# microsoft/fadtk

Measured on AMD Instinct MI355X. Metric: FAD scores/sec + cov-GEMM TFLOP/s (% MFMA peak), N=100k D=512, higher is better.
Workload: dtype f16 in, f16 MFMA with f32 accumulate over <= 8192-row runs, f64 across runs (moments); split-f16 MFMA iterations (f32 accumulate) + exact int8-MFMA products (int32 accumulate) + f64 correction (Frechet)

## Files before the change

fadtk_amd/csrc/frechet.hip:

```cpp
#include "frechet_internal.h"
#include "ns_mean.h"
#include "ns_fast.h"
#include "ns_fast_big.h"
#include "ns_fast_res.h"

#include <algorithm>
#include <atomic>
#include <cmath>
#include <type_traits>

namespace fad {

Pool& thread_pool(int device) {
    static thread_local PerThreadDevice<Pool> set;
    return set.get(device);
}
Workspace* free_slot(int device) {
    Pool& p = thread_pool(device);
    for (Workspace& w : p.slot)
        if (!w.busy) { w.pool = &p; return &w; }
    return nullptr;
}

SongKnobs SongKnobs::from_env() {
    SongKnobs k;
    auto off = [](const char* name) { const char* e = getenv(name); return e && e[0] == '0'; };
    if (const char* e = getenv("FAD_SONG_BIG")) k.big_min = atol(e);
    if (const char* e = getenv("FAD_SONG_RES")) k.res = (e[0] == '0') ? 0 : (e[0] == '1' ? 1 : 2);
    if (const char* e = getenv("FAD_SONG_FAST")) k.fast = (e[0] == '0') ? 0 : (e[0] == '2' ? 2 : 1);
    if (const char* e = getenv("FAD_FAST_TRACE")) k.trace = e[0] == '1';
    k.scaled = !off("FAD_SONG_SCALED");
    if (const char* e = getenv("FAD_SONG_L0_SCALE")) { const double v = atof(e); if (v > 0.0) k.l0_scale = v; }
    return k;
}


struct MixedResult {
    int status;
    int iters, decided_at, nonfinite, too_few0, too_few1;
    double tr_scaled, c, tr1, tr2, mean_term, res, est;
    int prepared;
    int pad;
};

__global__ __launch_bounds__(256) void ns32_finish(const double* __restrict__ stats, int d, int nb,
                                                   const NsState* __restrict__ st, Ns32State* __restrict__ s32,
                                                   MixedResult* __restrict__ out, int max_low) {
    __shared__ double red[4];
    __shared__ double red3[12];
    const int tid = threadIdx.x;
    const bool live = s32->ok != 0;
    double mr = 0.0, mc = 0.0, corr = 0.0, r2 = 0.0, tr = 0.0;
    if (live) {
        const double* rowabs = stats;
        const double* colabs = stats + (int64_t)nb * d;
        const double* scal = stats + 2 * (int64_t)nb * d;
        for (int i = tid; i < d; i += 256) {
            double rs, cs;
            sum_partials(rowabs, colabs, nb, d, i, rs, cs);
            mr = fmax(mr, rs); mc = fmax(mc, cs);
        }
        for (int k = tid; k < nb * nb; k += 256) {
            const double* sc = scal + (int64_t)kStatScal * k;
            corr += sc[0]; r2 += sc[1]; tr += sc[2];
        }
    }
    const double zinf = block_max(mr, red), zone = block_max(mc, red);
    double v3[3] = {corr, r2, tr};
    block_sum_n<3>(v3, red3);
    corr = v3[0]; r2 = v3[1]; tr = v3[2];
    if (tid != 0) return;
    MixedResult o;
    o.status = 0; o.iters = s32->final_iter; o.decided_at = s32->decided_at; o.nonfinite = st->nonfinite;
    o.too_few0 = st->too_few[0]; o.too_few1 = st->too_few[1];
    o.c = st->c; o.tr1 = st->tr1; o.tr2 = st->tr2; o.mean_term = st->mean_term;
    o.tr_scaled = 0.0; o.res = 0.0; o.est = 0.0; o.prepared = 1; o.pad = 0;
    if (st->done || s32->failed) {
        o.status = 2;
    } else if (live) {
        const int f = s32->final_iter;
        const int fm = f < 16 ? f : 15;
        double res = s32->res[fm];
        if (s32->decided_at == f - 1) { const double rp = s32->res[f - 1 < 16 ? f - 1 : 15]; res = 0.75 * rp * rp + 0.25 * rp * rp * rp; if (res < 2e-6) res = 2e-6; }
        const double zn = sqrt(zinf * zone), rn = sqrt(r2);
        const double trs = tr + 0.5 * corr;
        const double est = zn * zn * zn * rn * rn / 8.0 + zn * res * rn / 2.0;
        const bool finite = (trs == trs) && !isinf(trs) && (est == est) && !isinf(est);
        o.tr_scaled = trs; o.res = res; o.est = est;
        o.status = (finite && est <= 1e-9 * fabs(trs)) ? 1 : 2;
        if (o.status == 2 && finite && !s32->strict && s32->decided_at == f - 1 && f + 1 < max_low) {
            o.status = 4;
            s32->done = 0; s32->finished = 0; s32->ok = 0; s32->skip_corr = 1; s32->upd_skip[0] = 0; s32->upd_skip[1] = 0;
            s32->strict = 1;
        }
    }
    *out = o;
}

constexpr int kMaxLow = 14;
constexpr int kMaxLowWide = 22;
constexpr double kWideL0Scale = 3.0, kWideL0Min = 9e-4;
static bool wide_enabled(Pool* p) {
    if (p && p->lp_wide < 0) { const char* e = getenv("FAD_FRECHET_WIDE"); p->lp_wide = (e && e[0] == '0') ? 0 : 1; }
    return !p || p->lp_wide != 0;
}
static int max_low_of(const Workspace& ws) { return (ws.job.fast && wide_enabled(ws.pool)) ? kMaxLowWide : kMaxLow; }

static double pred_threshold(Pool* p, int d) {
    if (p && p->pred_thr == 0.0) { const char* e = getenv("FAD_FRECHET_PRED_THR"); p->pred_thr = (e && atof(e) > 0.0) ? atof(e) : -1.0; }
    if (p && p->pred_thr > 0.0) return p->pred_thr;
    return 2.5e-3 * (double)d / 512.0;
}

struct MixedBufs {
    double* A; float *Y[2], *Z[2], *T;
    NsState* dstate; double* partials; double* tilestats; Ns32State* s32; MixedResult* hres;
    unsigned nb;
};
static MixedBufs mixed_bufs(Workspace& ws, int d) {
    const int64_t dd = (int64_t)d * d;
    MixedBufs m;
    m.A = static_cast<double*>(ws.mats.p);
    m.Y[0] = static_cast<float*>(ws.mats32.p); m.Y[1] = m.Y[0] + dd;
    m.Z[0] = m.Y[1] + dd; m.Z[1] = m.Y[1] + 2 * dd;
    m.T = m.Y[1] + 3 * dd;
    m.dstate = static_cast<NsState*>(ws.small.p);
    m.partials = reinterpret_cast<double*>(m.dstate + 1);
    m.tilestats = m.partials + ns_pstride(d);
    m.s32 = reinterpret_cast<Ns32State*>(m.tilestats + stat_doubles(d));
    m.hres = reinterpret_cast<MixedResult*>(static_cast<char*>(ws.pinned) + sizeof(NsState));
    m.nb = (unsigned)stat_blocks(d);
    return m;
}

static int mixed_enqueue(Workspace& ws, int upto) {
    const int d = ws.job.d;
    hipStream_t stream = ws.job.stream;
    MixedBufs m = mixed_bufs(ws, d);
    int rc;
    for (int& k = ws.job.k; k < upto; ++k) {
        const int cur = k & 1;
        Gemm32Args g;
        memset(&g, 0, sizeof(g));
        if (k == 0) {
            g.C[0] = m.Y[1]; g.C[1] = m.Z[1]; g.alpha[0] = 1.0f; g.ntypes = 1; g.A64 = m.A; g.st64 = m.dstate;
            g.skip = &m.s32->done;
            FAD_TRY(gemm_f32_first_launch(d, g, stream));
            continue;
        }
        g.A[0] = m.Z[cur]; g.B[0] = m.Y[cur]; g.C[0] = m.T; g.alpha[0] = -0.5f; g.beta_eye[0] = 1.5f; g.gamma[0] = 1.0f;
        g.partials[0] = m.partials; g.skip = &m.s32->done; g.ntypes = 1;
        const int nslots = gemm_f32_launch(d, g, stream);
        if (nslots < 0) return nslots;
        memset(&g, 0, sizeof(g));
        g.A[0] = m.Y[cur]; g.B[0] = m.T; g.C[0] = m.Y[cur ^ 1]; g.alpha[0] = 1.0f;
        g.A[1] = m.T; g.B[1] = m.Z[cur]; g.C[1] = m.Z[cur ^ 1]; g.alpha[1] = 1.0f;
        g.ntypes = 2;
        g.skip = &m.s32->upd_skip[k & 1];
        g.check = 1; g.k = k; g.max_low = kMaxLow; g.nslots = nslots; g.chk_partials = m.partials; g.st = m.s32; g.st64 = m.dstate;
        g.thr_pred = pred_threshold(ws.pool, d);
        rc = gemm_f32_launch(d, g, stream);
        if (rc < 0) return rc;
    }
    NsProductExt ext;
    memset(&ext, 0, sizeof(ext));
    ext.stats = m.tilestats; ext.st = m.dstate; ext.A64 = m.A; ext.Z32 = m.Z[0]; ext.Z32_alt = m.Z[1];
    FAD_TRY(gemm_f64_correction_launch(d, m.Y[0], m.Y[1], &m.s32->final_iter, &m.s32->skip_corr, ext, stream));
    hipLaunchKernelGGL(ns32_finish, dim3(1), dim3(256), 0, stream, m.tilestats, d, (int)m.nb, m.dstate, m.s32, m.hres, kMaxLow);
    FAD_HIP_TRY(hipGetLastError());
    if (!ws.done_ev) FAD_HIP_TRY(hipEventCreateWithFlags(&ws.done_ev, hipEventDisableTiming));
    FAD_HIP_TRY(hipEventRecord(ws.done_ev, stream));
    return FAD_OK;
}

static bool mixed_eligible(Workspace& ws, int d, int max_iter, double tol);
static bool fast_dim(int d) { return d == 256 || d == 384 || d == 512 || d == 768 || d == 1024; }
static bool fast_eligible(Workspace& ws, int d, int max_iter, double tol) {
    Pool* p = ws.pool;
    if (p && p->fast < 0) { const char* e = getenv("FAD_FRECHET_FAST"); p->fast = (e && e[0] == '0') ? 0 : 1; }
    return (!p || p->fast) && fast_dim(d) && mixed_eligible(ws, d, max_iter, tol);
}

struct FastBufs {
    nsf::MatHdr* hdr;
    uint4* digC[2];
    nsf::SplitMat P, Y[2], Z[2], T;
    uint4 *digY[2], *digYt[2];
    nsf::SplitMat Rv, Pv, Ev;
    int* host_words; double* host_vals; double* host_stats; double* host_vstats;
};
static size_t fast_bytes(int d) {
    const size_t dd = (size_t)d * d;
    return 256 + 2 * 6 * dd + 6 * 8 * dd + 4 * 6 * dd + 3 * 8 * dd + 256;
}
static size_t fast_pinned_bytes(int d) {
    const size_t nb = (size_t)d / 32;
    return sizeof(NsState) + sizeof(MixedResult) + 64 + nsf::kHostWords * sizeof(int) + nsf::kHostVals * sizeof(double) +
           (nsf::kTileStats + 2 + nsf::kVerStats) * nb * nb * sizeof(double) + 128;
}
static FastBufs fast_bufs(Workspace& ws, int d) {
    const size_t dd = (size_t)d * d;
    char* p = static_cast<char*>(ws.fast.p);
    FastBufs f;
    f.hdr = reinterpret_cast<nsf::MatHdr*>(p); p += 256;
    for (int i = 0; i < 2; ++i) { f.digC[i] = reinterpret_cast<uint4*>(p); p += 6 * dd; }
    nsf::SplitMat* mats[6] = {&f.P, &f.Y[0], &f.Y[1], &f.Z[0], &f.Z[1], &f.T};
    for (nsf::SplitMat* m : mats) {
        m->a = reinterpret_cast<uint4*>(p); p += 4 * dd;
        m->at = reinterpret_cast<uint4*>(p); p += 4 * dd;
    }
    for (int i = 0; i < 2; ++i) { f.digY[i] = reinterpret_cast<uint4*>(p); p += 6 * dd; f.digYt[i] = reinterpret_cast<uint4*>(p); p += 6 * dd; }
    nsf::SplitMat* vmats[3] = {&f.Rv, &f.Pv, &f.Ev};
    for (nsf::SplitMat* m : vmats) {
        m->a = reinterpret_cast<uint4*>(p); p += 4 * dd;
        m->at = reinterpret_cast<uint4*>(p); p += 4 * dd;
    }
    char* h = static_cast<char*>(ws.pinned);
    f.host_words = nullptr; f.host_vals = nullptr; f.host_stats = nullptr; f.host_vstats = nullptr;
    if (h && ws.pinned_cap >= fast_pinned_bytes(d)) {
        const size_t nb2 = ((size_t)d / 32) * ((size_t)d / 32);
        h += ((sizeof(NsState) + sizeof(MixedResult) + 63) / 64) * 64;
        f.host_vals = reinterpret_cast<double*>(h); h += nsf::kHostVals * sizeof(double);
        f.host_stats = reinterpret_cast<double*>(h); h += (nsf::kTileStats + 2) * nb2 * sizeof(double);
        f.host_vstats = reinterpret_cast<double*>(h); h += nsf::kVerStats * nb2 * sizeof(double);
        f.host_words = reinterpret_cast<int*>(h);
    }
    return f;
}

static int fast_prepare(Workspace& ws, int d, int ddof, const double* acc1, const double* acc2, const double* cov1, const double* cov2,
                        const double* mu1, const double* mu2, int mean_dtype, double* mus, double* covs, hipStream_t st,
                        const float* run1 = nullptr, const float* run2 = nullptr) {
    void* const before = ws.fast.p;
    FAD_TRY(ws.fast.reserve(fast_bytes(d)));
    FAD_TRY(ws.small.reserve(ns_small_bytes(d, 1)));
    FastBufs f = fast_bufs(ws, d);
    if (ws.fast.p != before) FAD_HIP_TRY(hipMemsetAsync(f.hdr, 0, 256, st));
    ws.job.gen = ++ws.fast_gen;
    if (ws.fast_gen > (1 << 30)) ws.fast_gen = 1;
    nsf::PrepArgs a;
    memset(&a, 0, sizeof(a));
    a.acc[0] = acc1; a.acc[1] = acc2; a.cov_in[0] = cov1; a.cov_in[1] = cov2; a.mu_in[0] = mu1; a.mu_in[1] = mu2;
    a.run[0] = run1; a.run[1] = run2;
    a.d = d; a.ddof = ddof; a.gen = ws.job.gen; a.mean_dtype = mean_dtype;
    a.mus = mus; a.covs = covs;
    a.dig[0] = f.digC[0]; a.dig[1] = f.digC[1];
    a.st = static_cast<NsState*>(ws.small.p);
    a.hdr[0] = f.hdr; a.hdr[1] = f.hdr + 1;
    hipLaunchKernelGGL(nsf::nsf_prepare, dim3((unsigned)((int64_t)d * d / 2048 + 1), 2), dim3(512), 0, st, a);
    FAD_HIP_TRY(hipGetLastError());
    return FAD_OK;
}

template <int NS> static void fast_launch_split(int mode, unsigned t, unsigned B, const nsf::SplitArgs& g, hipStream_t st) {
    if (mode == nsf::SP_FIRST) hipLaunchKernelGGL((nsf::nsf_split<NS, nsf::SP_FIRST>), dim3(t, t, B), dim3(512), 0, st, g);
    else if (mode == nsf::SP_T) hipLaunchKernelGGL((nsf::nsf_split<NS, nsf::SP_T>), dim3(t, t, B), dim3(512), 0, st, g);
    else if (mode == nsf::SP_V2) hipLaunchKernelGGL((nsf::nsf_split<NS, nsf::SP_V2>), dim3(t, t, 2 * B), dim3(512), 0, st, g);
    else if (mode == nsf::SP_V3) hipLaunchKernelGGL((nsf::nsf_split<NS, nsf::SP_V3>), dim3(t, t, B), dim3(512), 0, st, g);
    else hipLaunchKernelGGL((nsf::nsf_split<NS, nsf::SP_U>), dim3(t, t, 3 * B), dim3(512), 0, st, g);
}
static void fast_split(int d, int mode, const nsf::SplitArgs& g, hipStream_t st, unsigned B);
static void fast_verify_launch(int d, unsigned B, nsf::SplitArgs g, const nsf::SplitMat (&Y)[2], const nsf::SplitMat (&Z)[2], const nsf::SplitMat& Rv,
                               const nsf::SplitMat& Pv, const nsf::SplitMat& Ev, const Ns32State* s32, double* vstats, int* vwords, int64_t hstride,
                               hipStream_t st) {
    g.sel = &s32->final_iter; g.skip = &s32->skip_corr;
    g.Zf[0] = Z[0]; g.Zf[1] = Z[1]; g.Yf[0] = Y[0]; g.Yf[1] = Y[1];
    g.vstats = vstats; g.vwords = vwords; g.hstride = hstride;
    g.B[0] = Rv; g.C[0] = Pv; g.C[1] = Ev;
    fast_split(d, nsf::SP_V2, g, st, B);
    g.B[0] = Pv; g.A[1] = Ev; g.C[0] = nsf::SplitMat{nullptr, nullptr}; g.C[1] = nsf::SplitMat{nullptr, nullptr};
    fast_split(d, nsf::SP_V3, g, st, B);
}
static void fast_split(int d, int mode, const nsf::SplitArgs& g, hipStream_t st, unsigned B) {
    const unsigned t = (unsigned)(d / 32);
    switch (d) {
        case 128: fast_launch_split<1>(mode, t, B, g, st); break;
        case 256: fast_launch_split<2>(mode, t, B, g, st); break;
        case 384: fast_launch_split<3>(mode, t, B, g, st); break;
        case 512: fast_launch_split<4>(mode, t, B, g, st); break;
        case 768: fast_launch_split<6>(mode, t, B, g, st); break;
        default: fast_launch_split<8>(mode, t, B, g, st); break;
    }
}
template <int NJ> static void fast_big_attrs() {
    (void)hipFuncSetAttribute(reinterpret_cast<const void*>(&nsf::nsf_big<nsf::SP_T, NJ>), hipFuncAttributeMaxDynamicSharedMemorySize, (int)nsf::kBigLds);
    (void)hipFuncSetAttribute(reinterpret_cast<const void*>(&nsf::nsf_big<nsf::SP_U, NJ>), hipFuncAttributeMaxDynamicSharedMemorySize, (int)nsf::kBigLds);
    (void)hipFuncSetAttribute(reinterpret_cast<const void*>(&nsf::nsf_big<nsf::SP_FIRST, NJ>), hipFuncAttributeMaxDynamicSharedMemorySize, (int)nsf::kBigLds);
}
template <int NJ> static void fast_big_launch(int d, int mode, const nsf::SplitArgs& g, hipStream_t st, unsigned B) {
    const int tt = nsf::big_tiles(d, NJ);
    const unsigned one = (unsigned)nsf::big_grid((int)B, tt), two = (unsigned)nsf::big_grid((int)B, 2 * tt);
    if (mode == nsf::SP_FIRST) hipLaunchKernelGGL((nsf::nsf_big<nsf::SP_FIRST, NJ>), dim3(one), dim3(256), nsf::kBigLds, st, g);
    else if (mode == nsf::SP_T) hipLaunchKernelGGL((nsf::nsf_big<nsf::SP_T, NJ>), dim3(one), dim3(256), nsf::kBigLds, st, g);
    else hipLaunchKernelGGL((nsf::nsf_big<nsf::SP_U, NJ>), dim3(two + B), dim3(256), nsf::kBigLds, st, g);
}
static int fast_big_t_slots(int d, unsigned B) { return nsf::big_tiles(d, nsf::big_nj(d, 1, (int)B)); }
static int fast_split_big(int d, int mode, nsf::SplitArgs g, hipStream_t st, unsigned B, int device) {
    static std::atomic<unsigned> ready{0};
    if (device >= 0 && device < 32 && !(ready.load(std::memory_order_acquire) & (1u << device))) {
        fast_big_attrs<1>(); fast_big_attrs<2>();
        FAD_HIP_TRY(hipGetLastError());
        ready.fetch_or(1u << device, std::memory_order_release);
    }
    g.nprob = (int)B;
    if (nsf::big_nj(d, mode == nsf::SP_U ? 2 : 1, (int)B) == 1) fast_big_launch<1>(d, mode, g, st, B);
    else fast_big_launch<2>(d, mode, g, st, B);
    return FAD_OK;
}
static int fast_i8_big(int d, int mode, const nsf::I8Args& g, hipStream_t st, unsigned B, int device) {
    static std::atomic<unsigned> ready{0};
    if (device >= 0 && device < 32 && !(ready.load(std::memory_order_acquire) & (1u << device))) {
        FAD_HIP_TRY(hipFuncSetAttribute(reinterpret_cast<const void*>(&nsf::nsf_i8_big<nsf::I8_A>), hipFuncAttributeMaxDynamicSharedMemorySize, (int)nsf::kI8BigLds));
        FAD_HIP_TRY(hipFuncSetAttribute(reinterpret_cast<const void*>(&nsf::nsf_i8_big<nsf::I8_G>), hipFuncAttributeMaxDynamicSharedMemorySize, (int)nsf::kI8BigLds));
        FAD_HIP_TRY(hipFuncSetAttribute(reinterpret_cast<const void*>(&nsf::nsf_i8_big<nsf::I8_G, true>), hipFuncAttributeMaxDynamicSharedMemorySize, (int)nsf::kI8BigLds));
        ready.fetch_or(1u << device, std::memory_order_release);
    }
    const unsigned grid = (unsigned)nsf::big_grid((int)B, (d / 128) * (d / 64));
    if (mode == nsf::I8_A) hipLaunchKernelGGL((nsf::nsf_i8_big<nsf::I8_A>), dim3(grid), dim3(512), nsf::kI8BigLds, st, g, (int)B);
    else if (g.Rv.a) hipLaunchKernelGGL((nsf::nsf_i8_big<nsf::I8_G, true>), dim3(grid), dim3(512), nsf::kI8BigLds, st, g, (int)B);
    else hipLaunchKernelGGL((nsf::nsf_i8_big<nsf::I8_G>), dim3(grid), dim3(512), nsf::kI8BigLds, st, g, (int)B);
    return FAD_OK;
}
template <int NS8> static void fast_launch_i8(int mode, unsigned t, unsigned B, const nsf::I8Args& g, hipStream_t st) {
    if (mode == nsf::I8_A) hipLaunchKernelGGL((nsf::nsf_i8<NS8, nsf::I8_A>), dim3(t, t, B), dim3(512), 0, st, g);
    else hipLaunchKernelGGL((nsf::nsf_i8<NS8, nsf::I8_G>), dim3(t, t, B), dim3(512), 0, st, g);
}
static void fast_i8(int d, int mode, const nsf::I8Args& g, hipStream_t st, unsigned B = 1) {
    const unsigned t = (unsigned)(d / 32);
    switch (d) {
        case 128: case 256: fast_launch_i8<1>(mode, t, B, g, st); break;
        case 384: case 512: fast_launch_i8<2>(mode, t, B, g, st); break;
        case 768: fast_launch_i8<3>(mode, t, B, g, st); break;
        default: fast_launch_i8<4>(mode, t, B, g, st); break;
    }
}

static nsf::SplitArgs fast_split_args(Workspace& ws, const MixedBufs& m, const FastBufs& f, int d) {
    nsf::SplitArgs g;
    memset(&g, 0, sizeof(g));
    g.d = d; g.gen = ws.job.gen; g.hA = f.hdr; g.hB = f.hdr + 1; g.st = m.dstate; g.s32 = m.s32;
    if (wide_enabled(ws.pool)) { g.scaled = 1; g.lp_wide = 1; g.l0_scale = kWideL0Scale; g.l0_min = kWideL0Min; }
    return g;
}
static int fast_verify_enqueue(Workspace& ws) {
    const int d = ws.job.d;
    MixedBufs m = mixed_bufs(ws, d);
    FastBufs f = fast_bufs(ws, d);
    f.host_words[13] = 0;
    fast_verify_launch(d, 1, fast_split_args(ws, m, f, d), f.Y, f.Z, f.Rv, f.Pv, f.Ev, m.s32, f.host_vstats, f.host_words, 0, ws.job.stream);
    FAD_HIP_TRY(hipGetLastError());
    FAD_HIP_TRY(hipEventRecord(ws.done_ev, ws.job.stream));
    return FAD_OK;
}
static int fast_enqueue(Workspace& ws, int upto) {
    const int d = ws.job.d;
    hipStream_t stream = ws.job.stream;
    MixedBufs m = mixed_bufs(ws, d);
    FastBufs f = fast_bufs(ws, d);
    if (!f.host_words) return set_error(FAD_ERR_ALLOC, "pinned result area of the fast Frechet chain is missing");
    const int nslots = (d / 32) * (d / 32);
    const int max_low = max_low_of(ws);
    for (int& k = ws.job.k; k < upto; ++k) {
        nsf::SplitArgs g = fast_split_args(ws, m, f, d);
        if (k == 0) {
            nsf::I8Args a;
            memset(&a, 0, sizeof(a));
            a.Adig = f.digC[0]; a.Bdig = f.digC[1]; a.d = d; a.gen = ws.job.gen; a.hA = f.hdr; a.hB = f.hdr + 1; a.stats = m.tilestats;
            a.A64 = m.A; a.P = f.P; a.st = m.dstate;
            fast_i8(d, nsf::I8_A, a, stream);
            g.A[0] = f.P; g.B[0] = f.P; g.C[0] = f.Y[1]; g.C[1] = f.Z[1]; g.Cdig[0] = f.digY[1]; g.Cdig_t[0] = f.digYt[1];
            g.A64 = m.A; g.statsA = m.tilestats;
            fast_split(d, nsf::SP_FIRST, g, stream, 1);
            continue;
        }
        const int cur = k & 1;
        g.A[0] = f.Z[cur]; g.B[0] = f.Y[cur]; g.C[0] = f.T; g.alpha = -0.5f; g.beta_eye = 1.5f; g.gamma = 1.0f;
        g.partials = m.partials; g.skip = &m.s32->done; g.k = k;
        fast_split(d, nsf::SP_T, g, stream, 1);
        g = fast_split_args(ws, m, f, d);
        g.A[0] = f.Y[cur]; g.B[0] = f.T; g.C[0] = f.Y[cur ^ 1];
        g.A[1] = f.T; g.B[1] = f.Z[cur]; g.C[1] = f.Z[cur ^ 1];
        g.Cdig[0] = f.digY[cur ^ 1]; g.Cdig_t[0] = f.digYt[cur ^ 1];
        g.skip = &m.s32->upd_skip[k & 1];
        g.k = k; g.max_low = max_low; g.nslots = nslots; g.chk_partials = m.partials;
        g.thr_pred = pred_threshold(ws.pool, d);
        fast_split(d, nsf::SP_U, g, stream, 1);
    }
    nsf::I8Args a;
    memset(&a, 0, sizeof(a));
    a.Adig = f.digY[0]; a.Bdig = f.digYt[0]; a.Adig_alt = f.digY[1]; a.Bdig_alt = f.digYt[1]; a.sel = &m.s32->final_iter;
    a.d = d; a.gen = ws.job.gen; a.hA = f.hdr; a.hB = f.hdr + 1; a.skip = &m.s32->skip_corr; a.stats = f.host_stats; a.st = m.dstate; a.A64in = m.A;
    a.Y[0] = f.Y[0]; a.Y[1] = f.Y[1]; a.Z[0] = f.Z[0]; a.Z[1] = f.Z[1];
    a.s32 = m.s32; a.host_words = f.host_words; a.host_vals = f.host_vals;
    const bool wide = wide_enabled(ws.pool);
    if (wide) { a.Rv = f.Rv; a.scaled = 1; }
    f.host_words[12] = 0;
    f.host_words[13] = 0;
    fast_i8(d, nsf::I8_G, a, stream);
    FAD_HIP_TRY(hipGetLastError());
    if (!ws.done_ev) FAD_HIP_TRY(hipEventCreateWithFlags(&ws.done_ev, hipEventDisableTiming));
    if (wide && ws.pool && ws.pool->lp_verify) return fast_verify_enqueue(ws);
    FAD_HIP_TRY(hipEventRecord(ws.done_ev, stream));
    return FAD_OK;
}

static void fast_decide_one(const int* hw, const double* hv, const double* hsx, int nb, MixedResult* out, const double* hvx = nullptr,
                            int gen = 0, int max_low = kMaxLow) {
    MixedResult o;
    memset(&o, 0, sizeof(o));
    const bool bad = hw[0] != 0;
    o.status = 0; o.iters = hw[7]; o.decided_at = hw[8]; o.nonfinite = hw[2]; o.too_few0 = hw[3]; o.too_few1 = hw[4];
    o.c = hv[0]; o.tr1 = hv[1]; o.tr2 = hv[2]; o.mean_term = hv[3];
    o.prepared = 0;
    const bool ok = hw[5] != 0, failed = hw[6] != 0, strict = hw[9] != 0;
    if (bad || hw[1] || failed) {
        o.status = 2;
    } else if (ok && !hw[11]) {
        double corr = 0.0, r2 = 0.0, tr = 0.0, zinf = 0.0, zone = 0.0;
        for (int t = 0; t < nb * nb; ++t) { corr += hsx[nsf::kTileStats * t]; r2 += hsx[nsf::kTileStats * t + 1]; tr += hsx[nsf::kTileStats * t + 2]; }
        const double* zmax = hsx + (size_t)nsf::kTileStats * nb * nb;
        for (int x = 0; x < nb; ++x) {
            double rs = 0.0, cs = 0.0;
            for (int y = 0; y < nb; ++y) { rs += zmax[2 * (y * nb + x)]; cs += zmax[2 * (x * nb + y) + 1]; }
            if (rs > zinf) zinf = rs;
            if (cs > zone) zone = cs;
        }
        const int fi = hw[7];
        double res = hv[4 + ns32_slot(fi)];
        if (hw[8] == fi - 1) { const double rp = hv[4 + ns32_slot(fi - 1)]; res = 0.75 * rp * rp + 0.25 * rp * rp * rp; if (res < 2e-6) res = 2e-6; }
        const double zn = std::sqrt(zinf * zone), rn = std::sqrt(r2);
        double trs = tr + 0.5 * corr;
        double est = zn * zn * zn * rn * rn / 8.0 + zn * res * rn / 2.0;
        bool finite = std::isfinite(trs) && std::isfinite(est);
        double fad = o.mean_term + o.tr1 + o.tr2 - 2.0 * std::sqrt(o.c) * trs;
        bool accept = finite && (est <= 1e-9 * std::fabs(trs) || 2.0 * std::sqrt(o.c) * est <= 1e-5 * std::fabs(fad));
        const bool scaled = hvx && hw[14] != 0;
        const bool predicted = hw[8] == fi - 1 && fi >= 1;
        const double r_pred = predicted ? hv[4 + ns32_slot(fi - 1)] : 0.0;
        const bool can_go_on = predicted && !strict && fi + 1 < max_low && (!scaled || r_pred > 0.1);
        bool need_verify = false;
        if (!accept && finite && hvx && !can_go_on) {
            if (hw[13] == gen) {
                const double inv = 1.0 / ((double)nsf::kVerScale * (double)nsf::kVerScale);
                double qp = 0.0, ep = 0.0, pp = 0.0, ee = 0.0;
                for (int t = 0; t < nb * nb; ++t) { qp += hvx[nsf::kVerStats * t]; ep += hvx[nsf::kVerStats * t + 1]; pp += hvx[nsf::kVerStats * t + 2]; ee += hvx[nsf::kVerStats * t + 3]; }
                qp *= inv; ep *= inv; pp *= inv; ee *= inv;
                const double trs_v = trs + 0.5 * ep;
                const double est_v = 4.0 * std::fabs(qp) / 8.0 + ee * std::sqrt(pp);
                const double fad_v = o.mean_term + o.tr1 + o.tr2 - 2.0 * std::sqrt(o.c) * trs_v;
                const bool fin_v = std::isfinite(trs_v) && std::isfinite(est_v);
                if (fin_v && (est_v <= 1e-9 * std::fabs(trs_v) || 2.0 * std::sqrt(o.c) * est_v <= 4e-6 * std::fabs(fad_v))) {
                    accept = true; trs = trs_v; est = est_v; fad = fad_v; o.pad = 1;
                }
            } else {
                need_verify = true;
            }
        }
        o.tr_scaled = trs; o.res = res; o.est = est;
        o.status = accept ? 1 : 2;
        if (!accept && finite && can_go_on) o.status = 4;
        else if (!accept && need_verify) o.status = 5;
    }
    *out = o;
}

static int fast_decide(Workspace& ws) {
    const int d = ws.job.d, nb = d / 32;
    MixedBufs m = mixed_bufs(ws, d);
    FastBufs f = fast_bufs(ws, d);
    if (f.host_words[12] != ws.job.gen) return set_error(FAD_ERR_HIP, "the correction kernel of the fast Frechet chain left no result");
    const bool wide = wide_enabled(ws.pool);
    fast_decide_one(f.host_words, f.host_vals, f.host_stats, nb, m.hres, wide ? f.host_vstats : nullptr, ws.job.gen, max_low_of(ws));
    if (m.hres->status == 4) {
        hipLaunchKernelGGL(nsf::nsf_rearm, dim3(1), dim3(64), 0, ws.job.stream, m.s32);
        FAD_HIP_TRY(hipGetLastError());
    }
    return FAD_OK;
}

bool fast_song_dim(int d) { return d == 128 || d == 256 || d == 384 || d == 512 || d == 768 || d == 1024; }

struct SongBlock {
    size_t hdr, st, s32, partials, stats, A64, P, Y[2], Z[2], T, digS, digY[2], digYt[2], stride;
};
static SongBlock song_block(int d) {
    const size_t dd = (size_t)d * d, nb = (size_t)d / 32;
    SongBlock b; size_t o = 0;
    auto take = [&](size_t bytes) { const size_t at = o; o += (bytes + 255) & ~(size_t)255; return at; };
    b.hdr = take(sizeof(nsf::MatHdr)); b.st = take(sizeof(NsState)); b.s32 = take(sizeof(Ns32State));
    b.partials = take(nb * nb * sizeof(double)); b.stats = take(nsf::kTileStats * nb * nb * sizeof(double));
    b.A64 = take(8 * dd); b.P = take(8 * dd);
    b.Y[0] = take(8 * dd); b.Y[1] = take(8 * dd); b.Z[0] = take(8 * dd); b.Z[1] = take(8 * dd); b.T = take(8 * dd);
    b.digS = take(6 * dd);
    b.digY[0] = take(6 * dd); b.digYt[0] = take(6 * dd); b.digY[1] = take(6 * dd); b.digYt[1] = take(6 * dd);
    b.stride = o;
    return b;
}
static size_t host_vstats_off(int d) {
    const size_t nb = (size_t)d / 32;
    return (nsf::kHostVals + (nsf::kTileStats + 2) * nb * nb) * sizeof(double) + ((nsf::kHostWords * sizeof(int) + 7) & ~(size_t)7);
}
static size_t song_host_stride(int d) {
    const size_t nb = (size_t)d / 32;
    return (host_vstats_off(d) + nsf::kVerStats * nb * nb * sizeof(double) + 63) & ~(size_t)63;
}
int64_t fast_songs_capacity(int d, size_t budget_bytes) {
    const int64_t n = (int64_t)(budget_bytes / song_block(d).stride);
    return n < 1 ? 1 : (n > 16384 ? 16384 : n);
}

int fast_songs(int d, int64_t B, const double* dcov_b, const double* covs, hipStream_t st, Workspace& ws,
               std::vector<double>& tr_sqrt, std::vector<char>& ok, int device, const SongKnobs& knobs) {
    const bool big = knobs.big_min > 0 && B >= knobs.big_min;
    const bool resident = d == 128 && knobs.res != 0;
    const bool res_full = resident && knobs.res != 1;
    const bool scaled_steps = knobs.scaled && big && d >= 256;
    const bool scaled_res = knobs.scaled && resident;
    const size_t dd = (size_t)d * d;
    const int nb = d / 32;
    const SongBlock L = song_block(d);
    const size_t hs = song_host_stride(d);
    FAD_TRY(ws.fast_songs.reserve(512 + 6 * dd + (size_t)B * L.stride));
    if (!ws.fast_songs_pin || ws.fast_songs_pin_cap < (size_t)B * hs) {
        if (ws.fast_songs_pin) (void)hipHostFree(ws.fast_songs_pin);
        ws.fast_songs_pin = nullptr; ws.fast_songs_pin_cap = 0;
        FAD_HIP_TRY(hipHostMalloc(&ws.fast_songs_pin, (size_t)B * hs + 4096, hipHostMallocDefault));
        ws.fast_songs_pin_cap = (size_t)B * hs + 4096;
    }
    char* base = static_cast<char*>(ws.fast_songs.p);
    nsf::MatHdr* hdr_b = reinterpret_cast<nsf::MatHdr*>(base);
    uint4* dig_b = reinterpret_cast<uint4*>(base + 512);
    char* blk = base + 512 + ((6 * dd + 255) & ~(size_t)255);
    char* hpin = static_cast<char*>(ws.fast_songs_pin);
    double* h_vals = reinterpret_cast<double*>(hpin);
    double* h_stats = h_vals + nsf::kHostVals;
    int* h_words = reinterpret_cast<int*>(h_stats + (size_t)(nsf::kTileStats + 2) * nb * nb);
    auto at = [&](size_t off) { return blk + off; };
    auto mat = [&](size_t off) { nsf::SplitMat m; m.a = reinterpret_cast<uint4*>(at(off)); m.at = reinterpret_cast<uint4*>(at(off + 4 * dd)); return m; };
    const int gen = ++ws.fast_gen;
    if (ws.fast_gen > (1 << 30)) ws.fast_gen = 1;
    FAD_HIP_TRY(hipMemsetAsync(hdr_b, 0, sizeof(nsf::MatHdr), st));
    FAD_HIP_TRY(hipMemset2DAsync(at(L.hdr), L.stride, 0, sizeof(nsf::MatHdr), (size_t)B, st));

    nsf::PrepArgs pa;
    memset(&pa, 0, sizeof(pa));
    pa.cov_in[0] = dcov_b; pa.cov_in[1] = covs; pa.d = d; pa.ddof = 1; pa.gen = gen; pa.mean_dtype = -1;
    pa.dig[0] = dig_b; pa.dig[1] = reinterpret_cast<uint4*>(at(L.digS));
    pa.st = reinterpret_cast<NsState*>(at(L.st)); pa.hdr[0] = hdr_b; pa.hdr[1] = reinterpret_cast<nsf::MatHdr*>(at(L.hdr));
    pa.batch = 1; pa.pstride = (int64_t)L.stride;
    hipLaunchKernelGGL(nsf::nsf_prepare, dim3((unsigned)(dd / 2048), (unsigned)(1 + B)), dim3(512), 0, st, pa);

    NsState* st0 = reinterpret_cast<NsState*>(at(L.st));
    Ns32State* s32_0 = reinterpret_cast<Ns32State*>(at(L.s32));
    double* partials = reinterpret_cast<double*>(at(L.partials));
    double* stats = reinterpret_cast<double*>(at(L.stats));
    double* A64 = reinterpret_cast<double*>(at(L.A64));
    const nsf::SplitMat P = mat(L.P), Y[2] = {mat(L.Y[0]), mat(L.Y[1])}, Z[2] = {mat(L.Z[0]), mat(L.Z[1])}, T = mat(L.T);
    uint4* digY[2] = {reinterpret_cast<uint4*>(at(L.digY[0])), reinterpret_cast<uint4*>(at(L.digY[1]))};
    uint4* digYt[2] = {reinterpret_cast<uint4*>(at(L.digYt[0])), reinterpret_cast<uint4*>(at(L.digYt[1]))};
    auto split_args = [&]() {
        nsf::SplitArgs g;
        memset(&g, 0, sizeof(g));
        g.d = d; g.gen = gen; g.hA = hdr_b; g.hB = reinterpret_cast<nsf::MatHdr*>(at(L.hdr)); g.pstride = (int64_t)L.stride;
        g.st = st0; g.s32 = s32_0;
        g.scaled = scaled_steps ? 1 : 0; g.l0_scale = knobs.l0_scale;
        return g;
    };
    {
        nsf::I8Args a;
        memset(&a, 0, sizeof(a));
        a.Adig = dig_b; a.Bdig = reinterpret_cast<uint4*>(at(L.digS)); a.d = d; a.gen = gen; a.hA = hdr_b;
        a.hB = reinterpret_cast<nsf::MatHdr*>(at(L.hdr)); a.pstride = (int64_t)L.stride; a.stats = stats; a.A64 = A64; a.P = P; a.st = st0;
        if (res_full) {  }
        else if (big && d >= 256) FAD_TRY(fast_i8_big(d, nsf::I8_A, a, st, (unsigned)B, device));
        else fast_i8(d, nsf::I8_A, a, st, (unsigned)B);
        if (resident) {
            static std::atomic<unsigned> ready{0};
            if (device >= 0 && device < 32 && !(ready.load(std::memory_order_acquire) & (1u << device))) {
                FAD_HIP_TRY(hipFuncSetAttribute(reinterpret_cast<const void*>(&nsf::nsf_res128<false>), hipFuncAttributeMaxDynamicSharedMemorySize, (int)nsf::kResLds));
                FAD_HIP_TRY(hipFuncSetAttribute(reinterpret_cast<const void*>(&nsf::nsf_res128<true>), hipFuncAttributeMaxDynamicSharedMemorySize, (int)nsf::kResLdsFull));
                ready.fetch_or(1u << device, std::memory_order_release);
            }
            nsf::ResArgs r;
            memset(&r, 0, sizeof(r));
            r.gen = gen; r.max_low = kMaxLow; r.thr_pred = pred_threshold(ws.pool, d); r.hA = hdr_b; r.hB = reinterpret_cast<nsf::MatHdr*>(at(L.hdr));
            r.pstride = (int64_t)L.stride; r.A64 = A64; r.statsA = stats; r.st = st0; r.s32 = s32_0;
            r.Y[0] = Y[0]; r.Y[1] = Y[1]; r.Z[0] = Z[0]; r.Z[1] = Z[1];
            r.scaled = scaled_res ? 1 : 0; r.l0_scale = 2.0 * knobs.l0_scale;
            if (res_full) {
                r.Adig = dig_b; r.Bdig = reinterpret_cast<uint4*>(at(L.digS)); r.hstride = (int64_t)hs;
                r.stats = h_stats; r.host_words = h_words; r.host_vals = h_vals;
                for (int64_t b = 0; b < B; ++b) reinterpret_cast<int*>(reinterpret_cast<char*>(h_words) + b * hs)[12] = 0;
                hipLaunchKernelGGL(nsf::nsf_res128<true>, dim3((unsigned)B), dim3(256), nsf::kResLdsFull, st, r);
            } else {
                hipLaunchKernelGGL(nsf::nsf_res128<false>, dim3((unsigned)B), dim3(256), nsf::kResLds, st, r);
            }
        } else {
            nsf::SplitArgs g = split_args();
            g.A[0] = P; g.B[0] = P; g.C[0] = Y[1]; g.C[1] = Z[1]; g.A64 = A64; g.statsA = stats;
            if (big && d >= 256) FAD_TRY(fast_split_big(d, nsf::SP_FIRST, g, st, (unsigned)B, device));
            else fast_split(d, nsf::SP_FIRST, g, st, (unsigned)B);
        }
    }
    tr_sqrt.assign((size_t)B, 0.0); ok.assign((size_t)B, 0);
    std::vector<char> settled((size_t)B, 0);
    const bool trace = knobs.trace;
    int k = 1, upto = resident ? 1 : 9;
    for (;;) {
        for (; k < upto; ++k) {
            const int cur = k & 1;
            nsf::SplitArgs g = split_args();
            g.A[0] = Z[cur]; g.B[0] = Y[cur]; g.C[0] = T; g.alpha = -0.5f; g.beta_eye = 1.5f; g.gamma = 1.0f;
            g.partials = partials; g.skip = &s32_0->done; g.k = k;
            if (big) FAD_TRY(fast_split_big(d, nsf::SP_T, g, st, (unsigned)B, device));
            else fast_split(d, nsf::SP_T, g, st, (unsigned)B);
            g = split_args();
            g.A[0] = Y[cur]; g.B[0] = T; g.C[0] = Y[cur ^ 1]; g.A[1] = T; g.B[1] = Z[cur]; g.C[1] = Z[cur ^ 1];
            g.skip = &s32_0->upd_skip[k & 1];
            g.k = k; g.max_low = kMaxLow; g.nslots = big ? fast_big_t_slots(d, (unsigned)B) : nb * nb; g.chk_partials = partials; g.thr_pred = pred_threshold(ws.pool, d);
            if (big) FAD_TRY(fast_split_big(d, nsf::SP_U, g, st, (unsigned)B, device));
            else fast_split(d, nsf::SP_U, g, st, (unsigned)B);
        }
        if (!res_full) {
            nsf::DigArgs dg;
            memset(&dg, 0, sizeof(dg));
            dg.d = d; dg.gen = gen; dg.hA = hdr_b; dg.hB = reinterpret_cast<nsf::MatHdr*>(at(L.hdr)); dg.pstride = (int64_t)L.stride; dg.s32 = s32_0;
            dg.Y[0] = Y[0]; dg.Y[1] = Y[1]; dg.dig[0] = digY[0]; dg.dig[1] = digY[1]; dg.dig_t[0] = digYt[0]; dg.dig_t[1] = digYt[1];
            hipLaunchKernelGGL(nsf::nsf_digitize, dim3((unsigned)((dd / 16 + 255) / 256), 2, (unsigned)B), dim3(256), 0, st, dg);
        }
        if (!res_full) {
            nsf::I8Args a;
            memset(&a, 0, sizeof(a));
            a.Adig = digY[0]; a.Bdig = digYt[0]; a.Adig_alt = digY[1]; a.Bdig_alt = digYt[1]; a.sel = &s32_0->final_iter;
            a.d = d; a.gen = gen; a.hA = hdr_b; a.hB = reinterpret_cast<nsf::MatHdr*>(at(L.hdr)); a.pstride = (int64_t)L.stride; a.hstride = (int64_t)hs;
            a.skip = &s32_0->skip_corr; a.stats = h_stats; a.st = st0; a.A64in = A64;
            a.Y[0] = Y[0]; a.Y[1] = Y[1]; a.Z[0] = Z[0]; a.Z[1] = Z[1]; a.s32 = s32_0; a.host_words = h_words; a.host_vals = h_vals;
            for (int64_t b = 0; b < B; ++b) reinterpret_cast<int*>(reinterpret_cast<char*>(h_words) + b * hs)[12] = 0;
            if (big && d >= 256) FAD_TRY(fast_i8_big(d, nsf::I8_G, a, st, (unsigned)B, device));
            else fast_i8(d, nsf::I8_G, a, st, (unsigned)B);
        }
        FAD_HIP_TRY(hipGetLastError());
        FAD_HIP_TRY(hipStreamSynchronize(st));
        bool pending = false;
        for (int64_t b = 0; b < B; ++b) {
            if (settled[b]) continue;
            const int* hw = reinterpret_cast<const int*>(reinterpret_cast<const char*>(h_words) + b * hs);
            const double* hv = reinterpret_cast<const double*>(reinterpret_cast<const char*>(h_vals) + b * hs);
            const double* hx = reinterpret_cast<const double*>(reinterpret_cast<const char*>(h_stats) + b * hs);
            if (hw[12] != gen) return set_error(FAD_ERR_HIP, "the correction kernel of the batched fast chain left no result for song %lld", (long long)b);
            MixedResult r;
            fast_decide_one(hw, hv, hx, nb, &r);
            if (r.status == 0 && k < kMaxLow && !resident) { pending = true; continue; }
            settled[b] = 1;
            if (r.status == 1) { ok[b] = 1; tr_sqrt[b] = std::sqrt(r.c) * r.tr_scaled; }
            if (trace)
                fprintf(stderr, "[fad fast songs] song %lld: status %d iters %d decided_at %d res %.3e est %.3e tr %.6e c %.3e (words bad %d done %d ok %d failed %d skipped %d)\n",
                        (long long)b, r.status, r.iters, r.decided_at, r.res, r.est, r.tr_scaled, r.c, hw[0], hw[1], hw[5], hw[6], hw[11]);
            if (trace && b == 0) {
                fprintf(stderr, "[fad fast songs] song 0 residuals:");
                for (int q = 1; q < 16 && q <= r.iters; ++q) fprintf(stderr, " %.3e", hv[4 + q]);
                fprintf(stderr, "\n");
            }
        }
        if (!pending) break;
        upto = kMaxLow;
    }
    return FAD_OK;
}


struct PairBlock {
    size_t hdrA, hdrB, st, s32, partials, stats, A64, P, Y[2], Z[2], T, digA, digB, digY[2], digYt[2], mus, covs, Rv, Pv, Ev, stride;
};
static PairBlock pair_block(int d) {
    const size_t dd = (size_t)d * d, nb = (size_t)d / 32;
    PairBlock b; size_t o = 0;
    auto take = [&](size_t bytes) { const size_t at = o; o += (bytes + 255) & ~(size_t)255; return at; };
    b.hdrA = take(sizeof(nsf::MatHdr)); b.hdrB = take(sizeof(nsf::MatHdr)); b.st = take(sizeof(NsState)); b.s32 = take(sizeof(Ns32State));
    b.partials = take(nb * nb * sizeof(double)); b.stats = take(nsf::kTileStats * nb * nb * sizeof(double));
    b.A64 = take(8 * dd); b.P = take(8 * dd);
    b.Y[0] = take(8 * dd); b.Y[1] = take(8 * dd); b.Z[0] = take(8 * dd); b.Z[1] = take(8 * dd); b.T = take(8 * dd);
    b.digA = take(6 * dd); b.digB = take(6 * dd);
    b.digY[0] = take(6 * dd); b.digYt[0] = take(6 * dd); b.digY[1] = take(6 * dd); b.digYt[1] = take(6 * dd);
    b.mus = take(2 * (size_t)d * sizeof(double)); b.covs = take(2 * dd * sizeof(double));
    b.Rv = take(8 * dd); b.Pv = take(8 * dd); b.Ev = take(8 * dd);
    b.stride = o;
    return b;
}

static int pairs_verify_enqueue(Workspace& ws, int d, int B, hipStream_t st) {
    const size_t dd = (size_t)d * d;
    const PairBlock L = pair_block(d);
    const size_t hs = song_host_stride(d);
    char* blk = static_cast<char*>(ws.fast_pairs.p);
    char* hpin = static_cast<char*>(ws.fast_pairs_pin);
    auto at = [&](size_t off) { return blk + off; };
    auto mat = [&](size_t off) { nsf::SplitMat m; m.a = reinterpret_cast<uint4*>(at(off)); m.at = reinterpret_cast<uint4*>(at(off + 4 * dd)); return m; };
    nsf::SplitArgs g;
    memset(&g, 0, sizeof(g));
    g.d = d; g.gen = ws.multi.gen; g.hA = reinterpret_cast<nsf::MatHdr*>(at(L.hdrA)); g.hB = reinterpret_cast<nsf::MatHdr*>(at(L.hdrB));
    g.pstride = (int64_t)L.stride; g.astride = (int64_t)L.stride;
    g.st = reinterpret_cast<NsState*>(at(L.st)); g.s32 = reinterpret_cast<Ns32State*>(at(L.s32));
    const nsf::SplitMat Y[2] = {mat(L.Y[0]), mat(L.Y[1])}, Z[2] = {mat(L.Z[0]), mat(L.Z[1])};
    const int nb = d / 32;
    int* h_words = reinterpret_cast<int*>(hpin + (nsf::kHostVals + (size_t)(nsf::kTileStats + 2) * nb * nb) * sizeof(double));
    double* h_vstats = reinterpret_cast<double*>(hpin + host_vstats_off(d));
    for (int b = 0; b < B; ++b) reinterpret_cast<int*>(reinterpret_cast<char*>(h_words) + (size_t)b * hs)[13] = 0;
    fast_verify_launch(d, (unsigned)B, g, Y, Z, mat(L.Rv), mat(L.Pv), mat(L.Ev), g.s32, h_vstats, h_words, (int64_t)hs, st);
    FAD_HIP_TRY(hipGetLastError());
    FAD_HIP_TRY(hipEventRecord(ws.done_ev, st));
    return FAD_OK;
}

static int pairs_enqueue(Workspace& ws, int d, int B, const fad_moments_t* const* h1, const fad_moments_t* const* h2, int ddof,
                         int mean_dtype, hipStream_t st) {
    const size_t dd = (size_t)d * d;
    const int nb = d / 32;
    constexpr int kPairsBigMin = 3;
    const bool big = B >= kPairsBigMin && d >= 256;
    const bool wide = wide_enabled(ws.pool);
    const int max_low = wide ? kMaxLowWide : kMaxLow;
    const int device = ws.job.device;
    const PairBlock L = pair_block(d);
    const size_t hs = song_host_stride(d);
    void* const before = ws.fast_pairs.p;
    FAD_TRY(ws.fast_pairs.reserve((size_t)(B > 16 ? kMaxMultiPairs : B > 8 ? 16 : B > 4 ? 8 : 4) * L.stride + 256));
    if (!ws.fast_pairs_pin || ws.fast_pairs_pin_cap < (size_t)B * hs) {
        if (ws.fast_pairs_pin) (void)hipHostFree(ws.fast_pairs_pin);
        ws.fast_pairs_pin = nullptr; ws.fast_pairs_pin_cap = 0;
        FAD_HIP_TRY(hipHostMalloc(&ws.fast_pairs_pin, (size_t)kMaxMultiPairs * hs + 4096, hipHostMallocDefault));
        ws.fast_pairs_pin_cap = (size_t)kMaxMultiPairs * hs + 4096;
    }
    char* blk = static_cast<char*>(ws.fast_pairs.p);
    char* hpin = static_cast<char*>(ws.fast_pairs_pin);
    double* h_vals = reinterpret_cast<double*>(hpin);
    double* h_stats = h_vals + nsf::kHostVals;
    int* h_words = reinterpret_cast<int*>(h_stats + (size_t)(nsf::kTileStats + 2) * nb * nb);
    auto at = [&](size_t off) { return blk + off; };
    auto mat = [&](size_t off) { nsf::SplitMat m; m.a = reinterpret_cast<uint4*>(at(off)); m.at = reinterpret_cast<uint4*>(at(off + 4 * dd)); return m; };
    const int gen = ++ws.fast_gen;
    if (ws.fast_gen > (1 << 30)) ws.fast_gen = 1;
    ws.multi.gen = gen;
    if (ws.fast_pairs.p != before) {
        FAD_HIP_TRY(hipMemset2DAsync(at(L.hdrA), L.stride, 0, sizeof(nsf::MatHdr), (size_t)B, st));
        FAD_HIP_TRY(hipMemset2DAsync(at(L.hdrB), L.stride, 0, sizeof(nsf::MatHdr), (size_t)B, st));
    }
    nsf::MatHdr* hA = reinterpret_cast<nsf::MatHdr*>(at(L.hdrA));
    nsf::MatHdr* hB = reinterpret_cast<nsf::MatHdr*>(at(L.hdrB));
    NsState* st0 = reinterpret_cast<NsState*>(at(L.st));
    Ns32State* s32_0 = reinterpret_cast<Ns32State*>(at(L.s32));
    double* partials = reinterpret_cast<double*>(at(L.partials));
    double* stats = reinterpret_cast<double*>(at(L.stats));
    double* A64 = reinterpret_cast<double*>(at(L.A64));
    const nsf::SplitMat P = mat(L.P), Y[2] = {mat(L.Y[0]), mat(L.Y[1])}, Z[2] = {mat(L.Z[0]), mat(L.Z[1])}, T = mat(L.T);
    uint4* digY[2] = {reinterpret_cast<uint4*>(at(L.digY[0])), reinterpret_cast<uint4*>(at(L.digY[1]))};
    uint4* digYt[2] = {reinterpret_cast<uint4*>(at(L.digYt[0])), reinterpret_cast<uint4*>(at(L.digYt[1]))};

    static_assert(2 * kMaxMultiPairs <= nsf::kPrepMaxSets, "PrepArgs holds two sets per pair of a batch");
    nsf::PrepArgs pa;
    memset(&pa, 0, sizeof(pa));
    for (int b = 0; b < B; ++b) {
        pa.accs[2 * b] = moments_packed(h1[b]); pa.accs[2 * b + 1] = moments_packed(h2[b]);
        pa.runs[2 * b] = moments_runsum(h1[b]); pa.runs[2 * b + 1] = moments_runsum(h2[b]);
    }
    pa.acc[0] = pa.accs[0]; pa.acc[1] = pa.accs[1];
    pa.d = d; pa.ddof = ddof; pa.gen = gen; pa.mean_dtype = mean_dtype;
    pa.mus = reinterpret_cast<double*>(at(L.mus)); pa.covs = reinterpret_cast<double*>(at(L.covs));
    pa.dig[0] = reinterpret_cast<uint4*>(at(L.digA)); pa.dig[1] = reinterpret_cast<uint4*>(at(L.digB));
    pa.st = st0; pa.hdr[0] = hA; pa.hdr[1] = hB;
    pa.batch = 2; pa.pstride = (int64_t)L.stride; pa.no_covs = 1;
    pa.per = ((dd / 2048) % 4 == 0) ? 4 : 2;
    hipLaunchKernelGGL(nsf::nsf_prepare, dim3((unsigned)(dd / 2048 / pa.per + 1), (unsigned)(2 * B)), dim3(512), 0, st, pa);

    auto split_args = [&]() {
        nsf::SplitArgs g;
        memset(&g, 0, sizeof(g));
        g.d = d; g.gen = gen; g.hA = hA; g.hB = hB; g.pstride = (int64_t)L.stride; g.astride = (int64_t)L.stride;
        g.st = st0; g.s32 = s32_0;
        if (wide) { g.scaled = 1; g.lp_wide = 1; g.l0_scale = kWideL0Scale; g.l0_min = kWideL0Min; }
        return g;
    };
    {
        nsf::I8Args a;
        memset(&a, 0, sizeof(a));
        a.Adig = reinterpret_cast<uint4*>(at(L.digA)); a.Bdig = reinterpret_cast<uint4*>(at(L.digB)); a.d = d; a.gen = gen; a.hA = hA; a.hB = hB;
        a.pstride = (int64_t)L.stride; a.astride = (int64_t)L.stride; a.stats = stats; a.A64 = A64; a.P = P; a.st = st0;
        if (big) FAD_TRY(fast_i8_big(d, nsf::I8_A, a, st, (unsigned)B, device));
        else fast_i8(d, nsf::I8_A, a, st, (unsigned)B);
        nsf::SplitArgs g = split_args();
        g.A[0] = P; g.B[0] = P; g.C[0] = Y[1]; g.C[1] = Z[1]; g.A64 = A64; g.statsA = stats;
        if (big) FAD_TRY(fast_split_big(d, nsf::SP_FIRST, g, st, (unsigned)B, device));
        else { g.Cdig[0] = digY[1]; g.Cdig_t[0] = digYt[1]; fast_split(d, nsf::SP_FIRST, g, st, (unsigned)B); }
    }
    int want = ws.pool ? ws.pool->lp_iters : 5;
    if (want < 2) want = 2;
    if (want > max_low) want = max_low;
    for (int k = 1; k < want; ++k) {
        const int cur = k & 1;
        nsf::SplitArgs g = split_args();
        g.A[0] = Z[cur]; g.B[0] = Y[cur]; g.C[0] = T; g.alpha = -0.5f; g.beta_eye = 1.5f; g.gamma = 1.0f;
        g.partials = partials; g.skip = &s32_0->done; g.k = k;
        if (big) FAD_TRY(fast_split_big(d, nsf::SP_T, g, st, (unsigned)B, device));
        else fast_split(d, nsf::SP_T, g, st, (unsigned)B);
        g = split_args();
        g.A[0] = Y[cur]; g.B[0] = T; g.C[0] = Y[cur ^ 1]; g.A[1] = T; g.B[1] = Z[cur]; g.C[1] = Z[cur ^ 1];
        if (!big) { g.Cdig[0] = digY[cur ^ 1]; g.Cdig_t[0] = digYt[cur ^ 1]; }
        g.skip = &s32_0->upd_skip[k & 1];
        g.k = k; g.max_low = max_low; g.nslots = big ? fast_big_t_slots(d, (unsigned)B) : nb * nb; g.chk_partials = partials; g.thr_pred = pred_threshold(ws.pool, d);
        if (big) FAD_TRY(fast_split_big(d, nsf::SP_U, g, st, (unsigned)B, device));
        else fast_split(d, nsf::SP_U, g, st, (unsigned)B);
    }
    if (big) {
        nsf::DigArgs dg;
        memset(&dg, 0, sizeof(dg));
        dg.d = d; dg.gen = gen; dg.hA = hA; dg.hB = hB; dg.pstride = (int64_t)L.stride; dg.astride = (int64_t)L.stride; dg.s32 = s32_0;
        dg.Y[0] = Y[0]; dg.Y[1] = Y[1]; dg.dig[0] = digY[0]; dg.dig[1] = digY[1]; dg.dig_t[0] = digYt[0]; dg.dig_t[1] = digYt[1];
        hipLaunchKernelGGL(nsf::nsf_digitize, dim3((unsigned)((dd / 16 + 255) / 256), 2, (unsigned)B), dim3(256), 0, st, dg);
    }
    {
        nsf::I8Args a;
        memset(&a, 0, sizeof(a));
        a.Adig = digY[0]; a.Bdig = digYt[0]; a.Adig_alt = digY[1]; a.Bdig_alt = digYt[1]; a.sel = &s32_0->final_iter;
        a.d = d; a.gen = gen; a.hA = hA; a.hB = hB; a.pstride = (int64_t)L.stride; a.astride = (int64_t)L.stride; a.hstride = (int64_t)hs;
        a.skip = &s32_0->skip_corr; a.stats = h_stats; a.st = st0; a.A64in = A64;
        a.Y[0] = Y[0]; a.Y[1] = Y[1]; a.Z[0] = Z[0]; a.Z[1] = Z[1]; a.s32 = s32_0; a.host_words = h_words; a.host_vals = h_vals;
        if (wide) { a.Rv = mat(L.Rv); a.scaled = 1; }
        for (int b = 0; b < B; ++b) { int* w = reinterpret_cast<int*>(reinterpret_cast<char*>(h_words) + (size_t)b * hs); w[12] = 0; w[13] = 0; }
        if (big) FAD_TRY(fast_i8_big(d, nsf::I8_G, a, st, (unsigned)B, device));
        else fast_i8(d, nsf::I8_G, a, st, (unsigned)B);
    }
    FAD_HIP_TRY(hipGetLastError());
    if (!ws.done_ev) FAD_HIP_TRY(hipEventCreateWithFlags(&ws.done_ev, hipEventDisableTiming));
    if (wide && ws.pool && ws.pool->lp_verify) return pairs_verify_enqueue(ws, d, B, st);
    FAD_HIP_TRY(hipEventRecord(ws.done_ev, st));
    return FAD_OK;
}

static int mixed_begin(const NsProblem& pb, int device, hipStream_t stream, Workspace& ws) {
    const int d = pb.d;
    const int64_t dd = (int64_t)d * d;
    FAD_TRY(ws.mats.reserve((size_t)(6 * dd) * sizeof(double)));
    FAD_TRY(ws.mats32.reserve((size_t)(5 * dd) * sizeof(float)));
    const size_t hbytes = ws.job.fast ? fast_pinned_bytes(d) : sizeof(NsState) + sizeof(MixedResult);
    if (!ws.pinned || ws.pinned_cap < hbytes) {
        if (ws.pinned) (void)hipHostFree(ws.pinned);
        ws.pinned = nullptr; ws.pinned_cap = 0;
        FAD_HIP_TRY(hipHostMalloc(&ws.pinned, hbytes + 4096, hipHostMallocDefault));
        ws.pinned_cap = hbytes + 4096;
    }
    MixedBufs m = mixed_bufs(ws, d);
    m.hres->status = -1;
    ws.job.d = d; ws.job.device = device; ws.job.stream = stream; ws.job.k = 0;
    if (ws.job.fast) {
        ws.job.mu1 = pb.mu1; ws.job.mu2 = pb.mu2; ws.job.mean_dtype = pb.mean_dtype;
        int want = ws.pool ? ws.pool->lp_iters : 5;
        if (want < 2) want = 2;
        if (want > max_low_of(ws)) want = max_low_of(ws);
        if (ws.pool && ws.pool->lp_hopeless) want = 1;
        return fast_enqueue(ws, want);
    }
    NsProductExt ext;
    memset(&ext, 0, sizeof(ext));
    ext.stats = m.tilestats; ext.mu1 = pb.mu1; ext.mu2 = pb.mu2; ext.mean_dtype = pb.mean_dtype; ext.st = m.dstate;
    FAD_TRY(gemm_f64_product_stats_launch(d, pb.cov1, pb.cov2, m.A, &m.dstate->done, ext, stream));
    enqueue_ns_prepare(m.tilestats, d, (int)m.nb, pb.mu1, 0, pb.mu2, 0, pb.mean_dtype, m.dstate, 1, m.s32, 1, stream);
    int want = ws.pool ? ws.pool->lp_iters : 5;
    if (want < 2) want = 2;
    if (want > kMaxLow) want = kMaxLow;
    return mixed_enqueue(ws, want);
}

static int mixed_finish(Workspace& ws, MixedResult* res) {
    MixedBufs m = mixed_bufs(ws, ws.job.d);
    const int max_low = max_low_of(ws);
    bool asked = false;
    for (;;) {
        FAD_HIP_TRY(hipEventSynchronize(ws.done_ev));
        if (ws.job.fast) FAD_TRY(fast_decide(ws));
        if (m.hres->status == 5) {
            if (asked) { m.hres->status = 2; break; }
            asked = true;
            FAD_TRY(fast_verify_enqueue(ws));
            continue;
        }
        if (m.hres->status == 4) {
            ws.job.k = m.hres->iters;
            m.hres->status = 0;
        } else if (m.hres->status != 0 || ws.job.k >= max_low) {
            break;
        }
        if (ws.job.k >= max_low) break;
        const int step = (ws.job.fast && max_low > kMaxLow) ? 4 : 2;
        const int upto = (ws.job.k + step < max_low) ? ws.job.k + step : max_low;
        FAD_TRY(ws.job.fast ? fast_enqueue(ws, upto) : mixed_enqueue(ws, upto));
    }
    *res = *m.hres;
    if (res->status == 0) res->status = 2;
    if (res->status == 1 && res->decided_at >= 0 && ws.pool) ws.pool->lp_iters = res->decided_at + 1;
    if (ws.pool && ws.job.fast) {
        ws.pool->lp_hopeless = res->status == 2 && res->iters < 0;
        ws.pool->lp_verify = res->status == 1 && res->pad == 1;
    }
    return FAD_OK;
}

static bool mixed_eligible(Workspace& ws, int d, int max_iter, double tol) {
    Pool* p = ws.pool;
    if (p && p->mixed < 0) { const char* e = getenv("FAD_FRECHET_MIXED"); p->mixed = (e && e[0] == '0') ? 0 : 1; }
    return (!p || p->mixed) && d % 64 == 0 && max_iter <= 0 && tol <= 0.0;
}

static int frechet_single(int d, const double* cov1, const double* cov2, const double* mu1, const double* mu2,
                          double eps, int max_iter, double tol, int mean_dtype, int device, hipStream_t stream,
                          Workspace& ws, double* out_fad, fad_diag_t* diag, bool check_few) {
    const int64_t dd = (int64_t)d * d;
    NsState* hs = nullptr;
    bool reuse = false;
    NsProblem pb{d, 1, cov1, 0, cov2, 0, mu1, 0, mu2, 0, mean_dtype};
    if (mixed_eligible(ws, d, max_iter, tol)) {
        MixedResult r;
        if (!ws.job.mixed) FAD_TRY(mixed_begin(pb, device, stream, ws));
        ws.job.mixed = false;
        FAD_TRY(mixed_finish(ws, &r));
        if (check_few && (r.too_few0 || r.too_few1))
            return set_error(FAD_ERR_TOO_FEW_ROWS, "FAD requires at least two embedding window frames in each set");
        if (r.status == 1) {
            const double tr_sqrt = sqrt(r.c) * r.tr_scaled;
            if (out_fad) *out_fad = r.mean_term + r.tr1 + r.tr2 - 2.0 * tr_sqrt;
            if (diag) {
                diag->iters = r.iters + 1; diag->converged = 3; diag->used_eps = 0; diag->route = ws.job.fast ? 2 : 1;
                diag->residual = r.res; diag->scale = r.c; diag->mean_term = r.mean_term; diag->tr1 = r.tr1; diag->tr2 = r.tr2;
                diag->tr_sqrt = tr_sqrt; diag->verified = (ws.job.fast && r.pad == 1) ? 1 : 0; diag->reserved = 0;
            }
            return FAD_OK;
        }
        reuse = r.prepared != 0;
    }
    FAD_TRY(run_ns(pb, max_iter, tol, device, stream, ws, &hs, reuse));
    if (check_few && (hs->too_few[0] || hs->too_few[1]))
        return set_error(FAD_ERR_TOO_FEW_ROWS, "FAD requires at least two embedding window frames in each set");
    bool used_eps = false;
    if (hs->nonfinite && eps > 0.0) {
        FAD_TRY(ws.stage.reserve((size_t)(4 * dd + 2 * d) * sizeof(double)));
        double* E1 = static_cast<double*>(ws.stage.p) + 2 * dd + 2 * d;
        double* E2 = E1 + dd;
        FAD_HIP_TRY(hipMemcpyAsync(E1, cov1, dd * sizeof(double), hipMemcpyDeviceToDevice, stream));
        FAD_HIP_TRY(hipMemcpyAsync(E2, cov2, dd * sizeof(double), hipMemcpyDeviceToDevice, stream));
        enqueue_add_diag(E1, d, eps, stream);
        enqueue_add_diag(E2, d, eps, stream);
        enqueue_clear_states(static_cast<NsState*>(ws.small.p), 1, stream);
        NsProblem pe{d, 1, E1, 0, E2, 0, mu1, 0, mu2, 0, mean_dtype};
        FAD_TRY(run_ns(pe, max_iter, tol, device, stream, ws, &hs));
        used_eps = true;
    }
    if (hs->nonfinite) {
        if (diag) { memset(diag, 0, sizeof(*diag)); diag->used_eps = used_eps; diag->residual = hs->res_last; }
        return set_error(FAD_ERR_NOT_FINITE,
                         "sqrt(C1 C2) did not stay finite (NaN/Inf input or a product with negative eigenvalues)");
    }
    const double tr_sqrt = sqrt(hs->c) * hs->tr_last;
    double tr1 = hs->tr1, tr2 = hs->tr2;
    if (used_eps) { tr1 -= eps * d; tr2 -= eps * d; }
    if (out_fad) *out_fad = hs->mean_term + tr1 + tr2 - 2.0 * tr_sqrt;
    if (diag) {
        diag->iters = hs->final_iter + 1; diag->converged = hs->conv; diag->used_eps = used_eps ? 1 : 0;
        diag->route = 0; diag->residual = hs->res_last; diag->scale = hs->c;
        diag->mean_term = hs->mean_term; diag->tr1 = tr1; diag->tr2 = tr2; diag->tr_sqrt = tr_sqrt; diag->verified = 0; diag->reserved = 0;
    }
    if (hs->conv == 0)
        return set_error(FAD_ERR_NOT_CONVERGED, "Newton-Schulz stopped at max_iter with residual %.3e", hs->res_last);
    return FAD_OK;
}

const void* code_object_anchor_frechet() { return reinterpret_cast<const void*>(&ns32_finish); }
}

using namespace fad;

extern "C" {

int fad_frechet(int d, const double* mu1, const double* cov1, const double* mu2, const double* cov2,
                double eps, int max_iter, double tol, int on_device, int device, void* stream,
                double* out_fad, fad_diag_t* diag) {
    if (d < 1 || d > 16384) return set_error(FAD_ERR_INVALID, "d=%d out of range", d);
    if (!mu1 || !mu2 || !cov1 || !cov2 || !out_fad) return set_error(FAD_ERR_INVALID, "NULL argument");
    FAD_TRY(check_device(device));
    DeviceGuard g(device);
    if (!g.ok) return set_error(FAD_ERR_HIP, "cannot select device %d", device);
    hipStream_t st = static_cast<hipStream_t>(stream);
    Workspace* wsp = free_slot(device);
    if (!wsp) return set_error(FAD_ERR_INVALID, "all %d Frechet slots of this thread are in flight: collect one with fad_frechet_end", Pool::kSlots);
    Workspace& ws = *wsp;
    ws.job = Workspace::Job();
    FAD_TRY(ws.small.reserve(ns_small_bytes(d, 1)));
    const bool fast = fast_eligible(ws, d, max_iter, tol);
    if (!fast) enqueue_clear_states(static_cast<NsState*>(ws.small.p), 1, st);
    const int64_t dd = (int64_t)d * d;
    const double *dc1 = cov1, *dc2 = cov2, *dm1 = mu1, *dm2 = mu2;
    if (!on_device) {
        FAD_TRY(ws.stage.reserve((size_t)(4 * dd + 2 * d) * sizeof(double)));
        double* s = static_cast<double*>(ws.stage.p);
        FAD_HIP_TRY(hipMemcpyAsync(s, cov1, dd * sizeof(double), hipMemcpyHostToDevice, st));
        FAD_HIP_TRY(hipMemcpyAsync(s + dd, cov2, dd * sizeof(double), hipMemcpyHostToDevice, st));
        FAD_HIP_TRY(hipMemcpyAsync(s + 2 * dd, mu1, d * sizeof(double), hipMemcpyHostToDevice, st));
        FAD_HIP_TRY(hipMemcpyAsync(s + 2 * dd + d, mu2, d * sizeof(double), hipMemcpyHostToDevice, st));
        dc1 = s; dc2 = s + dd; dm1 = s + 2 * dd; dm2 = s + 2 * dd + d;
    }
    if (fast) {
        ws.job.fast = true;
        FAD_TRY(fast_prepare(ws, d, 1, nullptr, nullptr, dc1, dc2, dm1, dm2, -1, nullptr, nullptr, st));
    }
    return frechet_single(d, dc1, dc2, dm1, dm2, eps, max_iter, tol, -1, device, st, ws, out_fad, diag, false);
}

static int stage_from_moments(const fad_moments_t* h1, const fad_moments_t* h2, int ddof, double eps, int mean_dtype,
                              hipStream_t st, Workspace& ws, int max_iter = 0, double tol = 0.0) {
    if (!h1 || !h2) return set_error(FAD_ERR_INVALID, "NULL argument");
    const int d = moments_dim(h1), device = moments_device(h1);
    if (moments_dim(h2) != d)
        return set_error(FAD_ERR_SHAPE, "Training and test covariances have different dimensions (%d vs %d)", d, moments_dim(h2));
    if (moments_device(h2) != device) return set_error(FAD_ERR_INVALID, "handles live on different devices");
    FAD_TRY(moments_settle(h1, st));
    FAD_TRY(moments_settle(h2, st));
    FAD_TRY(ws.small.reserve(ns_small_bytes(d, 1)));
    const int64_t dd = (int64_t)d * d;
    FAD_TRY(ws.stage.reserve((size_t)(4 * dd + 2 * d) * sizeof(double)));
    double* s = static_cast<double*>(ws.stage.p);
    ws.job = Workspace::Job();
    ws.job.d = d; ws.job.device = device; ws.job.stream = st; ws.job.eps = eps; ws.job.mean_dtype = mean_dtype; ws.job.ddof = ddof;
    ws.job.cov1 = s; ws.job.cov2 = s + dd; ws.job.mu1 = s + 2 * dd; ws.job.mu2 = s + 2 * dd + d;
    if (fast_eligible(ws, d, max_iter, tol)) {
        ws.job.fast = true;
        FAD_TRY(fast_prepare(ws, d, ddof, moments_packed(h1), moments_packed(h2), nullptr, nullptr, nullptr, nullptr, mean_dtype, s + 2 * dd, s, st,
                             moments_runsum(h1), moments_runsum(h2)));
        FAD_TRY(moments_mark_read(h1, st));
        return moments_mark_read(h2, st);
    }
    enqueue_finalize_for_frechet(moments_packed(h1), moments_packed(h2), d, ddof, s + 2 * dd, s, static_cast<NsState*>(ws.small.p), st,
                                 moments_runsum(h1), moments_runsum(h2));
    FAD_HIP_TRY(hipGetLastError());
    FAD_TRY(moments_mark_read(h1, st));
    return moments_mark_read(h2, st);
}

int fad_frechet_from_moments(const fad_moments_t* h1, const fad_moments_t* h2, int ddof, double eps,
                             int max_iter, double tol, int mean_dtype, void* stream, double* out_fad, fad_diag_t* diag) {
    if (!h1 || !h2 || !out_fad) return set_error(FAD_ERR_INVALID, "NULL argument");
    const int device = moments_device(h1);
    DeviceGuard g(device);
    hipStream_t st = static_cast<hipStream_t>(stream);
    Workspace* wsp = free_slot(device);
    if (!wsp) return set_error(FAD_ERR_INVALID, "all %d Frechet slots of this thread are in flight: collect one with fad_frechet_end", Pool::kSlots);
    Workspace& ws = *wsp;
    ws.pool = &thread_pool(device);
    FAD_TRY(stage_from_moments(h1, h2, ddof, eps, mean_dtype, st, ws, max_iter, tol));
    const Workspace::Job j = ws.job;
    return frechet_single(j.d, j.cov1, j.cov2, j.mu1, j.mu2, eps, max_iter, tol, mean_dtype, device, st, ws, out_fad, diag, true);
}

int fad_frechet_from_moments_begin(const fad_moments_t* h1, const fad_moments_t* h2, int ddof, double eps, int mean_dtype,
                                   void* stream, fad_frechet_job_t** job) {
    if (!h1 || !h2 || !job) return set_error(FAD_ERR_INVALID, "NULL argument");
    *job = nullptr;
    const int device = moments_device(h1);
    DeviceGuard g(device);
    hipStream_t st = static_cast<hipStream_t>(stream);
    Workspace* wsp = free_slot(device);
    if (!wsp) return set_error(FAD_ERR_INVALID, "all %d Frechet slots of this thread are in flight: collect one with fad_frechet_end", Pool::kSlots);
    Workspace& ws = *wsp;
    ws.pool = &thread_pool(device);
    const bool mixed = mixed_eligible(ws, moments_dim(h1), 0, 0.0);
    FAD_TRY(stage_from_moments(h1, h2, ddof, eps, mean_dtype, st, ws));
    if (mixed) {
        const Workspace::Job& j = ws.job;
        NsProblem pb{j.d, 1, j.cov1, 0, j.cov2, 0, j.mu1, 0, j.mu2, 0, mean_dtype};
        FAD_TRY(mixed_begin(pb, device, st, ws));
        ws.job.mixed = true;
    }
    ws.busy = true;
    *job = reinterpret_cast<fad_frechet_job_t*>(wsp);
    return FAD_OK;
}

int fad_frechet_end(fad_frechet_job_t* job, double* out_fad, fad_diag_t* diag) {
    if (!job || !out_fad) return set_error(FAD_ERR_INVALID, "NULL argument");
    Workspace& ws = *reinterpret_cast<Workspace*>(job);
    if (!ws.busy) return set_error(FAD_ERR_INVALID, "this job was collected already");
    DeviceGuard g(ws.job.device);
    ws.busy = false;
    const Workspace::Job j = ws.job;
    return frechet_single(j.d, j.cov1, j.cov2, j.mu1, j.mu2, j.eps, 0, 0.0, j.mean_dtype, j.device, j.stream, ws, out_fad, diag, true);
}

int fad_frechet_from_moments_multi_begin(int count, const fad_moments_t* const* h1, const fad_moments_t* const* h2, int ddof, double eps,
                                         int mean_dtype, void* stream, fad_frechet_job_t** job) {
    if (!h1 || !h2 || !job) return set_error(FAD_ERR_INVALID, "NULL argument");
    *job = nullptr;
    if (count < 1 || count > kMaxMultiPairs) return set_error(FAD_ERR_INVALID, "count=%d out of range [1, %d]", count, kMaxMultiPairs);
    for (int b = 0; b < count; ++b) if (!h1[b] || !h2[b]) return set_error(FAD_ERR_INVALID, "pair %d: NULL handle", b);
    const int device = moments_device(h1[0]), d = moments_dim(h1[0]);
    for (int b = 0; b < count; ++b) {
        if (moments_dim(h1[b]) != d || moments_dim(h2[b]) != d)
            return set_error(FAD_ERR_SHAPE, "Training and test covariances have different dimensions (pair %d: %d vs %d, pair 0: %d)", b,
                             moments_dim(h1[b]), moments_dim(h2[b]), d);
        if (moments_device(h1[b]) != device || moments_device(h2[b]) != device) return set_error(FAD_ERR_INVALID, "handles live on different devices");
    }
    DeviceGuard g(device);
    hipStream_t st = static_cast<hipStream_t>(stream);
    Workspace* wsp = free_slot(device);
    if (!wsp) return set_error(FAD_ERR_INVALID, "all %d Frechet slots of this thread are in flight: collect one with fad_frechet_end", Pool::kSlots);
    Workspace& ws = *wsp;
    ws.pool = &thread_pool(device);
    ws.job = Workspace::Job();
    ws.job.d = d; ws.job.device = device; ws.job.stream = st; ws.job.eps = eps; ws.job.mean_dtype = mean_dtype; ws.job.ddof = ddof;
    ws.multi = Workspace::Multi();
    ws.multi.count = count;
    for (int b = 0; b < count; ++b) { ws.multi.h1[b] = h1[b]; ws.multi.h2[b] = h2[b]; }
    if (fast_eligible(ws, d, 0, 0.0)) {
        for (int b = 0; b < count; ++b) { FAD_TRY(moments_settle(h1[b], st)); FAD_TRY(moments_settle(h2[b], st)); }
        FAD_TRY(pairs_enqueue(ws, d, count, h1, h2, ddof, mean_dtype, st));
        for (int b = 0; b < count; ++b) { FAD_TRY(moments_mark_read(h1[b], st)); FAD_TRY(moments_mark_read(h2[b], st)); }
        ws.multi.enqueued = true;
    }
    ws.busy = true;
    *job = reinterpret_cast<fad_frechet_job_t*>(wsp);
    return FAD_OK;
}

int fad_frechet_multi_end(fad_frechet_job_t* job, int count, double* out_fad, fad_diag_t* diag) {
    if (!job || !out_fad) return set_error(FAD_ERR_INVALID, "NULL argument");
    Workspace& ws = *reinterpret_cast<Workspace*>(job);
    if (!ws.busy) return set_error(FAD_ERR_INVALID, "this job was collected already");
    if (count != ws.multi.count) return set_error(FAD_ERR_INVALID, "this job holds %d pairs, not %d", ws.multi.count, count);
    const Workspace::Job j = ws.job;
    const Workspace::Multi m = ws.multi;
    DeviceGuard g(j.device);
    const int d = j.d, nb = d / 32;
    bool done[kMaxMultiPairs] = {false};
    int chain_status[kMaxMultiPairs];
    for (int b = 0; b < kMaxMultiPairs; ++b) chain_status[b] = -1;
    int rc = FAD_OK;
    if (m.enqueued) {
        const hipError_t e = hipEventSynchronize(ws.done_ev);
        if (e != hipSuccess) { ws.busy = false; return set_error(FAD_ERR_HIP, "hipEventSynchronize failed: %s", hipGetErrorString(e)); }
        const size_t hs = song_host_stride(d);
        const char* hpin = static_cast<const char*>(ws.fast_pairs_pin);
        const size_t off_stats = nsf::kHostVals * sizeof(double), off_words = off_stats + (size_t)(nsf::kTileStats + 2) * nb * nb * sizeof(double);
        const size_t off_vstats = host_vstats_off(d);
        const bool wide = wide_enabled(ws.pool);
        int learnt = -1;
        bool any_verified = false;
        for (int round = 0; round < 2; ++round) {
            bool ask = false;
            for (int b = 0; b < count; ++b) {
                if (done[b]) continue;
                const double* hv = reinterpret_cast<const double*>(hpin + (size_t)b * hs);
                const double* hx = reinterpret_cast<const double*>(hpin + (size_t)b * hs + off_stats);
                const int* hw = reinterpret_cast<const int*>(hpin + (size_t)b * hs + off_words);
                const double* hvx = reinterpret_cast<const double*>(hpin + (size_t)b * hs + off_vstats);
                if (hw[12] != m.gen) continue;
                MixedResult r;
                fast_decide_one(hw, hv, hx, nb, &r, wide ? hvx : nullptr, m.gen, wide ? kMaxLowWide : kMaxLow);
                chain_status[b] = r.status;
                if (r.too_few0 || r.too_few1) {
                    if (rc == FAD_OK) rc = set_error(FAD_ERR_TOO_FEW_ROWS, "FAD requires at least two embedding window frames in each set");
                    out_fad[b] = NAN; done[b] = true;
                    continue;
                }
                if (r.status == 5 && round == 0) { ask = true; continue; }
                if (r.status != 1) continue;
                const double tr_sqrt = sqrt(r.c) * r.tr_scaled;
                out_fad[b] = r.mean_term + r.tr1 + r.tr2 - 2.0 * tr_sqrt;
                if (diag) {
                    fad_diag_t& q = diag[b];
                    memset(&q, 0, sizeof(q));
                    q.iters = r.iters + 1; q.converged = 3; q.used_eps = 0; q.route = 2;
                    q.residual = r.res; q.scale = r.c; q.mean_term = r.mean_term; q.tr1 = r.tr1; q.tr2 = r.tr2; q.tr_sqrt = tr_sqrt;
                    q.verified = r.pad == 1 ? 1 : 0;
                }
                if (r.decided_at + 1 > learnt) learnt = r.decided_at + 1;
                if (r.pad == 1) any_verified = true;
                done[b] = true;
            }
            if (!ask) break;
            const int rv = pairs_verify_enqueue(ws, d, count, j.stream);
            if (rv != FAD_OK) { if (rc == FAD_OK) rc = rv; break; }
            const hipError_t e2 = hipEventSynchronize(ws.done_ev);
            if (e2 != hipSuccess) { ws.busy = false; return set_error(FAD_ERR_HIP, "hipEventSynchronize failed: %s", hipGetErrorString(e2)); }
        }
        if (learnt > 0 && ws.pool) ws.pool->lp_iters = learnt;
        if (ws.pool && wide) ws.pool->lp_verify = any_verified;

        int declined = 0;
        for (int b = 0; b < count; ++b) if (!done[b] && chain_status[b] == 2) ++declined;
        if (rc == FAD_OK && declined >= 2) {
            const PairBlock L = pair_block(d);
            const size_t dd = (size_t)d * d;
            char* blk = static_cast<char*>(ws.fast_pairs.p);
            const int64_t stride = (int64_t)(L.stride / sizeof(double));
            const double* mus = reinterpret_cast<const double*>(blk + L.mus);
            const double* covs = reinterpret_cast<const double*>(blk + L.covs);
            int r2 = ws.small.reserve(ns_small_bytes(d, count));
            NsState* hst = nullptr;
            if (r2 == FAD_OK) {
                NsState* dstates = static_cast<NsState*>(ws.small.p);
                enqueue_clear_states(dstates, count, j.stream);
                uint32_t mask = 0;
                for (int b = 0; b < count; ++b) if (done[b] || chain_status[b] != 2) mask |= (1u << b);
                if (mask) enqueue_mark_states_done(dstates, mask, count, j.stream);
                nsf::PrepArgs pc;
                memset(&pc, 0, sizeof(pc));
                for (int b = 0; b < count; ++b) { pc.accs[2 * b] = moments_packed(m.h1[b]); pc.accs[2 * b + 1] = moments_packed(m.h2[b]); }
                pc.d = d; pc.ddof = j.ddof; pc.batch = 2; pc.pstride = (int64_t)L.stride;
                pc.covs = reinterpret_cast<double*>(blk + L.covs);
                hipLaunchKernelGGL(nsf::nsf_pairs_covs, dim3((unsigned)(dd / 2048), (unsigned)(2 * count)), dim3(512), 0, j.stream, pc);
                NsProblem pb{d, count, covs, stride, covs + dd, stride, mus, stride, mus + d, stride, j.mean_dtype};
                r2 = run_ns(pb, 0, 0.0, j.device, j.stream, ws, &hst, false, nullptr, (ws.pool && ws.pool->f64_iters_multi > 0) ? ws.pool->f64_iters_multi + 1 : 0);
            }
            if (r2 == FAD_OK && hst) {
                int most = 0;
                for (int b = 0; b < count; ++b) {
                    if (done[b] || chain_status[b] != 2) continue;
                    const NsState& q = hst[b];
                    if (q.nonfinite || q.conv == 0 || !q.finished || q.final_iter < 0) continue;
                    const double tr_sqrt = sqrt(q.c) * q.tr_last;
                    out_fad[b] = q.mean_term + q.tr1 + q.tr2 - 2.0 * tr_sqrt;
                    if (diag) {
                        fad_diag_t& g2 = diag[b];
                        memset(&g2, 0, sizeof(g2));
                        g2.iters = q.final_iter + 1; g2.converged = q.conv; g2.used_eps = 0; g2.route = 0; g2.residual = q.res_last;
                        g2.scale = q.c; g2.mean_term = q.mean_term; g2.tr1 = q.tr1; g2.tr2 = q.tr2; g2.tr_sqrt = tr_sqrt;
                    }
                    if (q.final_iter + 1 > most) most = q.final_iter + 1;
                    done[b] = true;
                }
                if (most > 0 && ws.pool) ws.pool->f64_iters_multi = most;
            }
        }
    }
    ws.busy = false;
    ws.multi = Workspace::Multi();
    for (int b = 0; b < count; ++b) {
        if (done[b]) continue;
        const int r1 = fad_frechet_from_moments(m.h1[b], m.h2[b], j.ddof, j.eps, 0, 0.0, j.mean_dtype, j.stream, &out_fad[b], diag ? &diag[b] : nullptr);
        if (r1 != FAD_OK && rc == FAD_OK) rc = r1;
    }
    return rc;
}

int fad_frechet_cancel(fad_frechet_job_t* job) {
    if (!job) return set_error(FAD_ERR_INVALID, "NULL argument");
    Workspace& ws = *reinterpret_cast<Workspace*>(job);
    if (!ws.busy) return FAD_OK;
    DeviceGuard g(ws.job.device);
    if ((ws.job.mixed || ws.multi.enqueued) && ws.done_ev) FAD_HIP_TRY(hipEventSynchronize(ws.done_ev));
    else FAD_HIP_TRY(hipStreamSynchronize(ws.job.stream));
    ws.busy = false;
    ws.job = Workspace::Job();
    ws.multi = Workspace::Multi();
    return FAD_OK;
}

}
```

fadtk_amd/csrc/ns_fast.h:

```cpp
#pragma once
#include "fad_common.h"
#include "ns_check.h"
#include "ns32.h"
#include "ns_mean.h"

namespace fad {
namespace nsf {

typedef int i32x4 __attribute__((ext_vector_type(4)));
typedef int i32x16 __attribute__((ext_vector_type(16)));
typedef _Float16 f16x8 __attribute__((ext_vector_type(8)));
typedef _Float16 f16x2 __attribute__((ext_vector_type(2)));

constexpr int kDigits = 6;
constexpr int kUminA = 3, kUminG = 4;
constexpr float kLoScale = 2048.f, kLoInv = 1.f / 2048.f;
constexpr int kTileStats = 4;

__device__ __host__ __forceinline__ size_t fa_idx(int rb, int ks, int plane, int lane, int d) {
    return (((size_t)rb * (size_t)(d >> 4) + (size_t)ks) * 2 + (size_t)plane) * 64 + (size_t)lane;
}
__device__ __host__ __forceinline__ size_t dg_idx(int rb, int ks, int p, int lane, int d) {
    return (((size_t)rb * (size_t)(d >> 5) + (size_t)ks) * kDigits + (size_t)p) * 64 + (size_t)lane;
}
__device__ __host__ __forceinline__ size_t fa_elem(int row, int k, int plane, int d, int& half) {
    half = k & 7;
    return fa_idx(row >> 5, k >> 4, plane, 32 * ((k >> 3) & 1) + (row & 31), d);
}
__device__ __host__ __forceinline__ size_t dg_elem(int row, int k, int p, int d, int& byte) {
    byte = k & 15;
    return dg_idx(row >> 5, k >> 5, p, 32 * ((k >> 4) & 1) + (row & 31), d);
}

template <typename F> __device__ __forceinline__ void digits_of(F v, int (&dg)[kDigits]) {
    F t = v * (F)32;
#pragma unroll
    for (int p = kDigits - 1; p >= 0; --p) {
        const F r = (sizeof(F) == 4) ? (F)__builtin_rintf((float)t) : (F)__builtin_rint((double)t);
        dg[p] = (int)r;
        t = (t - r) * (F)128;
    }
}

__device__ __forceinline__ void split16(float v, _Float16& hi, _Float16& lo) {
    hi = (_Float16)v;
    lo = (_Float16)((v - (float)hi) * kLoScale);
}
__device__ __forceinline__ float used16(_Float16 hi, _Float16 lo) { return (float)hi + (float)lo * kLoInv; }

template <int N, int NW = 8> __device__ __forceinline__ void wg8_sum(double (&v)[N], double* red) {
#pragma unroll
    for (int q = 0; q < N; ++q)
#pragma unroll
        for (int off = 32; off > 0; off >>= 1) v[q] += __shfl_xor(v[q], off);
    __syncthreads();
    if ((threadIdx.x & 63) == 0) {
#pragma unroll
        for (int q = 0; q < N; ++q) red[(threadIdx.x >> 6) * N + q] = v[q];
    }
    __syncthreads();
#pragma unroll
    for (int q = 0; q < N; ++q) {
        double t = 0.0;
#pragma unroll
        for (int w = 0; w < NW; ++w) t += red[w * N + q];
        v[q] = t;
    }
}
template <int NW = 8> __device__ __forceinline__ double wg8_max(double v, double* red) {
#pragma unroll
    for (int off = 32; off > 0; off >>= 1) v = fmax(v, __shfl_xor(v, off));
    __syncthreads();
    if ((threadIdx.x & 63) == 0) red[threadIdx.x >> 6] = v;
    __syncthreads();
    double t = red[0];
#pragma unroll
    for (int w = 1; w < NW; ++w) t = fmax(t, red[w]);
    return t;
}

__device__ __forceinline__ void tile_of_block(int& ty, int& tx) {
    ty = blockIdx.y; tx = blockIdx.x;
    const int t = gridDim.x;
    if ((t & 3) == 0) {
        const int b = blockIdx.y * t + blockIdx.x;
        const int xcd = b & 7, idx = b >> 3;
        const int R = t >> 1, Cc = t >> 2;
        ty = (xcd >> 2) * R + idx / Cc;
        tx = (xcd & 3) * Cc + idx % Cc;
    }
}

struct MatHdr {
    double s;
    double tr;
    int bad;
    int flag_gen;
    int pad[2];
};
__device__ __forceinline__ bool hdr_bad(const MatHdr* a, const MatHdr* b, int gen) {
    return (a->bad | b->bad) != 0 || a->flag_gen == gen || b->flag_gen == gen;
}
__device__ __forceinline__ double hdr_inv_s12(const MatHdr* a, const MatHdr* b) { return 1.0 / (a->s * b->s); }

template <class T> __device__ __forceinline__ T* adv(T* p, int64_t bytes) {
    return reinterpret_cast<T*>(reinterpret_cast<uintptr_t>(p) + (uintptr_t)bytes);
}

struct SplitMat { uint4* a; uint4* at; };
__device__ __forceinline__ SplitMat adv(const SplitMat& m, int64_t bytes) { return SplitMat{adv(m.a, bytes), adv(m.at, bytes)}; }

constexpr int kPrepMaxSets = 64;
struct PrepArgs {
    const double* acc[2];
    const double* cov_in[2];
    const double* mu_in[2];
    int d, ddof, gen, mean_dtype;
    double* mus;
    double* covs;
    uint4* dig[2];
    NsState* st; MatHdr* hdr[2];
    int batch; int64_t pstride;
    const double* accs[kPrepMaxSets];
    const float* run[2]; const float* runs[kPrepMaxSets];
    int no_covs;
    int per;
};

__device__ __forceinline__ double prep_cov(double m, double sr, double sk, double inv_n, double inv_nd) { return (m - (sr * sk) * inv_n) * inv_nd; }

__global__ __launch_bounds__(512) void nsf_prepare(PrepArgs a) {
    __shared__ double red[8 * 2];
    __shared__ double mu_lds[2 * 1024];
    __shared__ float gaps[1024];
    const int tid = threadIdx.x, d = a.d;
    const bool pairs = a.batch == 2, songs = a.batch == 1;
    const int set = songs ? (blockIdx.y ? 1 : 0) : (pairs ? (int)(blockIdx.y & 1) : (int)blockIdx.y);
    const int64_t po = songs ? (blockIdx.y ? (int64_t)(blockIdx.y - 1) * a.pstride : 0) : (pairs ? (int64_t)(blockIdx.y >> 1) * a.pstride : 0);
    if (!songs && blockIdx.x == gridDim.x - 1) {
        if (set != 0 || tid >= 256) return;
        double* mus = adv(a.mus, po);
        for (int q = 0; q < 2; ++q) {
            const double* acq = pairs ? a.accs[(blockIdx.y & ~1u) + q] : a.acc[q];
            const float* rq = pairs ? a.runs[(blockIdx.y & ~1u) + q] : a.run[q];
            for (int i = tid; i < d; i += 256) {
                const double m = acq ? ((rq ? numpy_mean_of_f32_sum(rq[i], acq[0]) : acq[1 + i] / acq[0])) : a.mu_in[q][i];
                mu_lds[q * 1024 + i] = m;
                if (acq) mus[(int64_t)q * d + i] = m;
            }
        }
        __syncthreads();
        const double mt = mean_term_block(mu_lds, mu_lds + 1024, d, a.mean_dtype, gaps, red);
        if (tid == 0) adv(a.st, po)->mean_term = mt;
        return;
    }
    const double* acc = pairs ? a.accs[blockIdx.y] : a.acc[set];
    const double n = acc ? acc[0] : 2.0;
    const double* sum = acc ? acc + 1 : nullptr;
    const double* M = acc ? acc + 1 + d : a.cov_in[set] + ((songs && blockIdx.y) ? (int64_t)(blockIdx.y - 1) * d * d : 0);
    MatHdr* hdr = adv(a.hdr[set], po);
    NsState* st = adv(a.st, po);
    const double inv_n = 1.0 / n, inv_nd = 1.0 / (n - (double)a.ddof);
    const int per = a.per > 1 ? a.per : 1;
    int T = blockIdx.x * per * 512 + tid;
    int qd = T & 3, piece = T >> 2;
    int r = piece & 31, g = (piece >> 5) & 1, ksrb = piece >> 6, ks = ksrb % (d >> 5), rb = ksrb / (d >> 5);
    int row = 32 * rb + r, k0 = 32 * ks + 16 * g + 4 * qd;
    double m[4], sk[4], sr = 0.0;
    const bool transposed = !acc && set == 1;
    auto fetch = [&]() {
        const double* Mrow = M + (int64_t)row * d + k0;
#pragma unroll
        for (int q = 0; q < 4; ++q) m[q] = transposed ? M[(int64_t)(k0 + q) * d + row] : Mrow[q];
        if (acc) {
            sr = sum[row];
#pragma unroll
            for (int q = 0; q < 4; ++q) sk[q] = sum[k0 + q];
        }
    };
    fetch();
    double tr1[1] = {0.0}, mx = 0.0;
    for (int i = tid; i < d; i += 512) {
        const double md = M[(int64_t)i * d + i];
        const double v = acc ? (md - (sum[i] * sum[i]) * inv_n) * inv_nd : md;
        tr1[0] += v; mx = fmax(mx, v);
    }
    mx = wg8_max(mx, red);
    wg8_sum<1>(tr1, red);
    const double tr = tr1[0];
    const bool few = acc && n < 2.0;
    const bool bad = few || !(tr == tr) || isinf(tr) || !(mx > 0.0) || isinf(mx);
    int ex = 0;
    if (!bad) (void)frexp(mx, &ex);
    const double s = bad ? 1.0 : ldexp(1.0, -ex);
    if (blockIdx.x == 0 && tid == 0) {
        hdr->s = s; hdr->tr = tr; hdr->bad = bad ? 1 : 0;
        if (!songs) st->too_few[set] = few ? 1 : 0;
        if (songs ? set == 1 : set == 0) {
            st->done = 0; st->finished = 0; st->nonfinite = 0; st->conv = 0; st->final_iter = -1;
            st->upd_skip[0] = 0; st->upd_skip[1] = 0;
            if (songs) { st->too_few[0] = 0; st->too_few[1] = 0; st->mean_term = 0.0; }
        }
    }
    bool off_grid = false;
    uint4* out = adv(a.dig[set], po);
    for (int it = 0; it < per; ++it) {
        if (it > 0) {
            T += 512;
            qd = T & 3; piece = T >> 2;
            r = piece & 31; g = (piece >> 5) & 1; ksrb = piece >> 6; ks = ksrb % (d >> 5); rb = ksrb / (d >> 5);
            row = 32 * rb + r; k0 = 32 * ks + 16 * g + 4 * qd;
            fetch();
        }
        uint32_t w[kDigits];
#pragma unroll
        for (int p = 0; p < kDigits; ++p) w[p] = 0u;
        double* cov_out = acc ? adv(a.covs, po) + (int64_t)set * d * d + (int64_t)row * d + k0 : nullptr;
#pragma unroll
        for (int q = 0; q < 4; ++q) {
            const double c0 = acc ? prep_cov(m[q], sr, sk[q], inv_n, inv_nd) : m[q];
            if (acc && !a.no_covs) cov_out[q] = c0;
            const double v = c0 * s;
            const bool fits = fabs(v) <= 1.9375;
            off_grid = off_grid || !fits;
            int dg[kDigits];
            digits_of<double>((bad || !fits) ? 0.0 : v, dg);
#pragma unroll
            for (int p = 0; p < kDigits; ++p) w[p] |= ((uint32_t)dg[p] & 0xffu) << (8 * q);
        }
#pragma unroll
        for (int p = 0; p < kDigits; ++p) reinterpret_cast<uint32_t*>(out + dg_idx(rb, ks, p, 32 * g + r, d))[qd] = w[p];
    }
    if (off_grid) hdr->flag_gen = a.gen;
}

__global__ __launch_bounds__(512) void nsf_pairs_covs(PrepArgs a) {
    const int d = a.d, set = (int)(blockIdx.y & 1);
    const int64_t po = (int64_t)(blockIdx.y >> 1) * a.pstride;
    const double* acc = a.accs[blockIdx.y];
    const double n = acc[0];
    const double* sum = acc + 1;
    const double* M = acc + 1 + d;
    const double inv_n = 1.0 / n, inv_nd = 1.0 / (n - (double)a.ddof);
    const int64_t e = ((int64_t)blockIdx.x * 512 + threadIdx.x) * 4;
    const int row = (int)(e / d), k0 = (int)(e - (int64_t)row * d);
    const double sr = sum[row];
    double* cov_out = adv(a.covs, po) + (int64_t)set * d * d + (int64_t)row * d + k0;
#pragma unroll
    for (int q = 0; q < 4; ++q) cov_out[q] = prep_cov(M[(int64_t)row * d + k0 + q], sr, sum[k0 + q], inv_n, inv_nd);
}

__device__ __forceinline__ void store_tile_planes(const float* fin, const SplitMat& X, int ty, int tx, int d, int tid) {
    {
        const bool tr = tid >= 128;
        const int ln = tid & 31, q = (tid >> 5) & 3;
        f16x8 hi, lo;
#pragma unroll
        for (int j = 0; j < 8; ++j) {
            const float v = tr ? fin[(8 * q + j) * 33 + ln] : fin[ln * 33 + 8 * q + j];
            _Float16 h, l; split16(v, h, l); hi[j] = h; lo[j] = l;
        }
        uint4* base = tr ? X.at : X.a;
        const int rb = tr ? tx : ty, ks = 2 * (tr ? ty : tx) + (q >> 1), lane = 32 * (q & 1) + ln;
        uint4 uh, ul; __builtin_memcpy(&uh, &hi, 16); __builtin_memcpy(&ul, &lo, 16);
        base[fa_idx(rb, ks, 0, lane, d)] = uh;
        base[fa_idx(rb, ks, 1, lane, d)] = ul;
    }
}
__device__ __forceinline__ void store_tile_digits(const float* fin, uint4* dig, uint4* dig_t, int ty, int tx, int d, int tid) {
    {
        const bool tr = tid < 256;
        const int u = tid & 255, ln = u & 31, q = u >> 5;
        uint32_t w[kDigits];
#pragma unroll
        for (int p = 0; p < kDigits; ++p) w[p] = 0u;
#pragma unroll
        for (int j = 0; j < 4; ++j) {
            const float v = tr ? fin[(4 * q + j) * 33 + ln] : fin[ln * 33 + 4 * q + j];
            _Float16 h, l; split16(v, h, l);
            int dg[kDigits];
            digits_of<float>(used16(h, l), dg);
#pragma unroll
            for (int p = 0; p < kDigits; ++p) w[p] |= ((uint32_t)dg[p] & 0xffu) << (8 * j);
        }
        uint4* base = tr ? dig_t : dig;
        const int rb = tr ? tx : ty, ks = tr ? ty : tx, lane = 32 * (q >> 2) + ln;
#pragma unroll
        for (int p = 0; p < kDigits; ++p)
            reinterpret_cast<uint32_t*>(base + dg_idx(rb, ks, p, lane, d))[q & 3] = w[p];
    }
}
__device__ __forceinline__ void store_tile(const float* fin, const SplitMat& X, uint4* dig, uint4* dig_t, int ty, int tx, int d, int tid) {
    if (tid < 256) store_tile_planes(fin, X, ty, tx, d, tid);
    if (dig) store_tile_digits(fin, dig, dig_t, ty, tx, d, tid);
}


enum { I8_A = 0, I8_G = 1 };
constexpr int kHostWords = 16, kHostVals = 24;
struct I8Args {
    const uint4* Adig; const uint4* Bdig;
    const uint4* Adig_alt; const uint4* Bdig_alt; const int* sel;
    int d, gen;
    const MatHdr* hA; const MatHdr* hB;
    int64_t pstride, hstride;
    int64_t astride;
    const int* skip;
    double* stats;
    double* A64; SplitMat P;
    NsState* st;
    const double* A64in;
    SplitMat Y[2], Z[2];
    const Ns32State* s32;
    int* host_words;
    double* host_vals;
    SplitMat Rv;
    int scaled;
};
constexpr float kVerScale = 4096.f;
constexpr int kVerStats = 4;

template <int NS8, int MODE>
__global__ __launch_bounds__(512) void nsf_i8(I8Args g) {
    __shared__ __attribute__((aligned(16))) double part[2 * 32 * 33];
    __shared__ float fin[32 * 33];
    __shared__ float finR[(MODE == I8_G) ? 32 * 33 : 1];
    __shared__ double red[8 * 4];
    constexpr int kUmin = (MODE == I8_A) ? kUminA : kUminG;
    constexpr int kGroups = 2 * (kDigits - 1) - kUmin + 1;
    const int d = g.d, tid = threadIdx.x, lane = tid & 63;
    const int64_t po = (int64_t)blockIdx.z * g.pstride, ho = (int64_t)blockIdx.z * g.hstride;
    const MatHdr* hB = adv(g.hB, po);
    const MatHdr* hA = adv(g.hA, (int64_t)blockIdx.z * g.astride);
    NsState* const st_p = adv(g.st, po);
    const bool bad = hdr_bad(hA, hB, g.gen);
    const bool skipped = bad || (g.skip && *adv(g.skip, po) != 0);
    if constexpr (MODE == I8_G) {
        if (blockIdx.x == 0 && blockIdx.y == 0 && tid == 0) {
            const NsState* st = st_p; const Ns32State* s = adv(g.s32, po);
            int* hw = adv(g.host_words, ho); double* hv = adv(g.host_vals, ho);
            hw[0] = bad ? 1 : 0; hw[1] = st->done; hw[2] = st->nonfinite; hw[3] = st->too_few[0]; hw[4] = st->too_few[1];
            hw[5] = s->ok; hw[6] = s->failed; hw[7] = s->final_iter; hw[8] = s->decided_at; hw[9] = s->strict; hw[10] = s->finished;
            hw[11] = skipped ? 1 : 0;
            hv[0] = st->c; hv[1] = st->tr1; hv[2] = st->tr2; hv[3] = st->mean_term;
#pragma unroll
            for (int q = 0; q < 16; ++q) hv[4 + q] = s->res[q];
            hw[14] = (g.scaled && st->mu[0] != 1.0) ? 1 : 0;
            hw[12] = g.gen;
        }
    }
    if (skipped) return;
    int ty, tx; tile_of_block(ty, tx);
    const int wave = __builtin_amdgcn_readfirstlane(tid >> 6);
    const int kg = lane >> 5, r = lane & 31;
    const int row0 = ty * 32, col0 = tx * 32;
    const bool alt = (MODE == I8_G) && g.sel && (*adv(g.sel, po) & 1);
    const uint4* Ad = (MODE == I8_A) ? adv(g.Adig, (int64_t)blockIdx.z * g.astride) : adv(alt ? g.Adig_alt : g.Adig, po);
    const uint4* Bd = adv(alt ? g.Bdig_alt : g.Bdig, po);
    const bool idle = wave * NS8 >= (d >> 5);

    constexpr int NBUF = (NS8 <= 2) ? NS8 : 2;
    i32x4 a[NBUF][kDigits], b[NBUF][kDigits];
    auto fetch = [&](int buf, int s) {
        const i32x4* pa = reinterpret_cast<const i32x4*>(Ad + dg_idx(ty, wave * NS8 + s, 0, lane, d));
        const i32x4* pb = reinterpret_cast<const i32x4*>(Bd + dg_idx(tx, wave * NS8 + s, 0, lane, d));
#pragma unroll
        for (int m = kDigits - 1; m >= 0; --m) { a[buf][m] = pa[64 * m]; b[buf][m] = pb[64 * m]; }
    };
    i32x16 acc[kGroups];
#pragma unroll
    for (int u = 0; u < kGroups; ++u)
#pragma unroll
        for (int q = 0; q < 16; ++q) acc[u][q] = 0;
    auto mma = [&](int buf) {
#pragma unroll
        for (int m = kDigits - 1; m >= 0; --m) {
#pragma unroll
            for (int q = kDigits - 1; q >= m; --q)
                if (m + q >= kUmin) acc[m + q - kUmin] = __builtin_amdgcn_mfma_i32_32x32x32_i8(a[buf][m], b[buf][q], acc[m + q - kUmin], 0, 0, 0);
#pragma unroll
            for (int p = kDigits - 1; p > m; --p)
                if (p + m >= kUmin) acc[p + m - kUmin] = __builtin_amdgcn_mfma_i32_32x32x32_i8(a[buf][p], b[buf][m], acc[p + m - kUmin], 0, 0, 0);
        }
    };
    if (idle) {
    } else if constexpr (NS8 <= 2) {
#pragma unroll
        for (int s = 0; s < NS8; ++s) fetch(s, s);
#pragma unroll
        for (int s = 0; s < NS8; ++s) mma(s);
    } else {
        fetch(0, 0);
#pragma unroll
        for (int s = 0; s < NS8; ++s) {
            if (s + 1 < NS8) fetch((s + 1) & 1, s + 1);
            mma(s & 1);
        }
    }
    double gp[16];
#pragma unroll
    for (int q = 0; q < 16; ++q) gp[q] = 0.0;
#pragma unroll
    for (int u = 0; u < kGroups; ++u) {
        const double wgt = __builtin_ldexp(1.0, 7 * (u + kUmin) - 80);
#pragma unroll
        for (int q = 0; q < 16; ++q) gp[q] = __builtin_fma((double)acc[u][q], wgt, gp[q]);
    }
    {
        auto put = [&](int slot) {
#pragma unroll
            for (int reg = 0; reg < 16; ++reg) part[slot * (32 * 33) + ((reg & 3) + 8 * (reg >> 2) + 4 * kg) * 33 + r] = gp[reg];
        };
        auto add = [&](int slot) {
#pragma unroll
            for (int reg = 0; reg < 16; ++reg) gp[reg] += part[slot * (32 * 33) + ((reg & 3) + 8 * (reg >> 2) + 4 * kg) * 33 + r];
        };
        if (wave >= 6) put(wave - 6);
        __syncthreads();
        if (wave == 4 || wave == 5) add(wave - 4);
        __syncthreads();
        if (wave == 4 || wave == 5) put(wave - 4);
        __syncthreads();
        if (wave == 2 || wave == 3) add(wave - 2);
        __syncthreads();
        if (wave == 2 || wave == 3) put(wave - 2);
        __syncthreads();
        if (wave < 2) add(wave);
        __syncthreads();
        if (wave < 2) put(wave);
        __syncthreads();
    }
    const int rr = tid >> 4, cp = tid & 15;
    double G2[2];
#pragma unroll
    for (int q = 0; q < 2; ++q) {
        const int o = rr * 33 + 2 * cp + q;
        G2[q] = part[o] + part[(32 * 33) + o];
    }
    const int nb = gridDim.x;
    const int gr = row0 + rr, gc = col0 + 2 * cp;
    double* const stats = adv(g.stats, (MODE == I8_A) ? po : ho);
    double* scal = stats + (size_t)kTileStats * (ty * nb + tx);
    double m = 0.0, v3[3] = {0.0, 0.0, 0.0};
    if constexpr (MODE == I8_A) {
        const double inv = hdr_inv_s12(hA, hB);
        *reinterpret_cast<double2*>(adv(g.A64, po) + (int64_t)gr * d + gc) = make_double2(G2[0] * inv, G2[1] * inv);
        fin[rr * 33 + 2 * cp] = (float)G2[0]; fin[rr * 33 + 2 * cp + 1] = (float)G2[1];
        v3[0] = G2[0] * G2[0] + G2[1] * G2[1];
        v3[1] = (gr == gc ? G2[0] : 0.0) + (gr == gc + 1 ? G2[1] : 0.0);
        __syncthreads();
        store_tile(fin, adv(g.P, po), nullptr, nullptr, ty, tx, d, tid);
        if (tid < 32) { for (int c = 0; c < 32; ++c) m += fabsf(fin[tid * 33 + c]); }
        else if (tid < 64) { for (int q = 0; q < 32; ++q) m += fabsf(fin[q * 33 + tid - 32]); }
    } else {
        const SplitMat Zm = adv(g.Z[alt ? 1 : 0], po);
        const SplitMat Ym = adv(g.Y[alt ? 1 : 0], po);
        const double inv_c = 1.0 / st_p->c;
        const double2 a2 = *reinterpret_cast<const double2*>(adv(g.A64in, po) + (int64_t)gr * d + gc);
        int half;
        const size_t zi0 = fa_elem(gr, gc, 0, d, half);
        const f16x2 zh = *reinterpret_cast<const f16x2*>(reinterpret_cast<const _Float16*>(Zm.at + zi0) + half);
        const f16x2 zl = *reinterpret_cast<const f16x2*>(reinterpret_cast<const _Float16*>(Zm.at + zi0 + 64) + half);
        const double z0 = (double)used16(zh[0], zl[0]), z1 = (double)used16(zh[1], zl[1]);
        const double R0 = a2.x * inv_c - G2[0], R1 = a2.y * inv_c - G2[1];
        v3[0] = z0 * R0 + z1 * R1; v3[1] = R0 * R0 + R1 * R1;
        if (gr == gc || gr == gc + 1) {
            int hy;
            const size_t yi = fa_elem(gr, gr, 0, d, hy);
            v3[2] = (double)used16(reinterpret_cast<const _Float16*>(Ym.a + yi)[hy], reinterpret_cast<const _Float16*>(Ym.a + yi + 64)[hy]);
        }
        fin[rr * 33 + 2 * cp] = fabsf((float)z0); fin[rr * 33 + 2 * cp + 1] = fabsf((float)z1);
        finR[rr * 33 + 2 * cp] = (float)(R0 * (double)kVerScale); finR[rr * 33 + 2 * cp + 1] = (float)(R1 * (double)kVerScale);
        __syncthreads();
        if (g.Rv.a && tid < 256) store_tile_planes(finR, adv(g.Rv, po), ty, tx, d, tid);
        if (tid < 32) { for (int q = 0; q < 32; ++q) m += fin[q * 33 + tid]; }
        else if (tid < 64) { for (int c = 0; c < 32; ++c) m += fin[(tid - 32) * 33 + c]; }
    }
    double mrow = (tid < 32) ? m : 0.0, mcol = (tid >= 32 && tid < 64) ? m : 0.0;
#pragma unroll
    for (int off = 32; off > 0; off >>= 1) { mrow = fmax(mrow, __shfl_xor(mrow, off)); mcol = fmax(mcol, __shfl_xor(mcol, off)); }
    wg8_sum<3>(v3, red);
    if (tid == 0) {
        if constexpr (MODE == I8_A) {
            scal[0] = v3[0]; scal[1] = v3[1]; scal[2] = mrow; scal[3] = mcol;
        } else {
            scal[0] = v3[0]; scal[1] = v3[1]; scal[2] = v3[2]; scal[3] = 0.0;
            double* zmax = stats + (size_t)kTileStats * nb * nb + 2 * (size_t)(ty * nb + tx);
            zmax[0] = mrow; zmax[1] = mcol;
        }
    }
}

enum { SP_FIRST = 0, SP_T = 1, SP_U = 2, SP_V2 = 3, SP_V3 = 4 };
struct SplitArgs {
    int d, gen;
    const MatHdr* hA; const MatHdr* hB;
    int64_t pstride;
    int64_t astride;
    const int* skip;
    SplitMat A[2], B[2], C[2];
    uint4* Cdig[2]; uint4* Cdig_t[2];
    float alpha, beta_eye, gamma;
    double* partials;
    const double* A64; const double* statsA;
    NsState* st; Ns32State* s32;
    int k, max_low, nslots;
    int nprob;
    double l0_scale;
    int scaled;
    double thr_pred;
    const double* chk_partials;
    int lp_wide; double l0_min;
    const int* sel; SplitMat Zf[2], Yf[2];
    double* vstats; int* vwords; int64_t hstride;
};

template <int NT = 512> __device__ __forceinline__ void nsf_check(const SplitArgs& g, int64_t po, double* red) {
    Ns32State* st = adv(g.s32, po);
    NsState* st64 = adv(g.st, po);
    const double* chk_partials = adv(g.chk_partials, po);
    const int k = g.k;
    if (st->finished || st64->done) {
        if (threadIdx.x == 0) { st->upd_skip[(k + 1) & 1] = 1; if (st64->done && !st->finished) { st->finished = 1; st->failed = 1; st->done = 1; } }
        return;
    }
    double s[1] = {0.0};
    for (int i = threadIdx.x; i < g.nslots; i += NT) s[0] += chk_partials[i];
    wg8_sum<1, NT / 64>(s, red);
    if (threadIdx.x != 0) return;
    const double mu_k = g.scaled ? st64->mu[k] : 1.0;
    const double res = 2.0 * sqrt(s[0]) / (mu_k * mu_k * mu_k);
    st->res[ns32_slot(k)] = res;
    if (g.scaled && k + 1 < kMaxIter) {
        double l = st64->l_cur;
        if (res == res && res < 1.0) { const double lr = sqrt(1.0 - res); if (lr > l) l = lr; }
        (void)ns_step_scale_with(mu_k, l);
        double ln = l, mn = ns_step_scale(ln);
        const double cap = ns_scale_cap(res, g.d);
        st64->mu[k + 1] = mn < cap ? mn : cap;
        st64->l_cur = l;
    }
    const double prev = (k > 0) ? st->res[ns32_slot(k - 1)] : 1e300;
    const bool finite = (res == res) && !isinf(res);
    const bool grows = k >= 4 && res > prev && res > 1e-3;
    const bool give_up = grows && (!g.scaled || st->grew);
    st->grew = grows ? 1 : 0;
    if (!finite || k + 1 >= g.max_low || give_up) {
        st->failed = 1; st->finished = 1; st->done = 1; st->final_iter = k; st->decided_at = k; st->upd_skip[(k + 1) & 1] = 1;
        return;
    }
    if (k >= 1 && res <= 1e-3 && (res > 0.3 * prev || res <= 1e-6)) {
        st->ok = 1; st->skip_corr = 0; st->finished = 1; st->done = 1; st->final_iter = k; st->decided_at = k; st->upd_skip[(k + 1) & 1] = 1;
        return;
    }
    const double bound = 0.75 * res * res + 0.25 * res * res * res;
    if (bound <= (st->strict ? 2e-6 : g.thr_pred) && mu_k == 1.0) {
        st->ok = 1; st->skip_corr = 0; st->finished = 1; st->done = 1; st->final_iter = k + 1; st->decided_at = k; st->upd_skip[(k + 1) & 1] = 1;
    }
}

template <int NS, int MODE>
__global__ __launch_bounds__(512) void nsf_split(SplitArgs g) {
    __shared__ __attribute__((aligned(16))) float part[4 * 32 * 33];
    __shared__ float fin[32 * 33];
    __shared__ float fin2[32 * 33];
    __shared__ double red[8 * 4];
    const int d = g.d, tid = threadIdx.x, lane = tid & 63;
    constexpr int ZPER = (MODE == SP_U) ? 3 : ((MODE == SP_V2) ? 2 : 1);
    const int64_t po = (int64_t)(blockIdx.z / ZPER) * g.pstride;
    const int zs = (int)(blockIdx.z % ZPER);
    if constexpr (MODE == SP_U) {
        if (zs == 2) {
            if (blockIdx.x == 0 && blockIdx.y == 0) nsf_check<512>(g, po, red);
            return;
        }
    }
    const MatHdr* hB = adv(g.hB, po);
    const MatHdr* hA = adv(g.hA, (int64_t)(blockIdx.z / ZPER) * g.astride);
    if (hdr_bad(hA, hB, g.gen)) return;
    const int zi = (MODE == SP_U || MODE == SP_V2) ? zs : 0;
    int ty, tx; tile_of_block(ty, tx);
    const int wave = __builtin_amdgcn_readfirstlane(tid >> 6);
    const int kg = lane >> 5, r = lane & 31;
    const int row0 = ty * 32, col0 = tx * 32;
    constexpr bool VER = (MODE == SP_V2 || MODE == SP_V3);
    if constexpr (VER) {
        if (g.skip && *adv(g.skip, po) != 0) return;
        if (MODE == SP_V3 && blockIdx.x == 0 && blockIdx.y == 0 && tid == 0)
            adv(g.vwords, (int64_t)blockIdx.z * g.hstride)[13] = g.gen;
    }
    const int par = VER ? (*adv(g.sel, po) & 1) : 0;

    f16x8 ah[NS], al[NS], bh[NS], bl[NS];
    {
        const SplitMat Am = adv(VER ? g.Zf[par] : g.A[zi], po);
        const SplitMat Bm = adv((MODE == SP_V2 && zs == 1) ? g.Yf[par] : g.B[VER ? 0 : zi], po);
        const f16x8* pa = reinterpret_cast<const f16x8*>(Am.a + fa_idx(ty, wave * NS, 0, lane, d));
        const f16x8* pb = reinterpret_cast<const f16x8*>(Bm.at + fa_idx(tx, wave * NS, 0, lane, d));
#pragma unroll
        for (int s = 0; s < NS; ++s) { ah[s] = pa[128 * s]; al[s] = pa[128 * s + 64]; bh[s] = pb[128 * s]; bl[s] = pb[128 * s + 64]; }
    }
    const int rr = tid >> 4, cp = tid & 15;
    double inv_c = 0.0, inv_cn = 0.0;
    float m1 = 1.5f, m3 = 0.5f;
    double2 a2 = make_double2(0.0, 0.0);
    if constexpr (MODE == SP_FIRST) {
        a2 = *reinterpret_cast<const double2*>(adv(g.A64, po) + (int64_t)(row0 + rr) * d + col0 + 2 * cp);
        const int nb = gridDim.x;
        const double* scal = adv(g.statsA, po);
        double* tmax = reinterpret_cast<double*>(part);
        double v2[2] = {0.0, 0.0};
        for (int k = tid; k < nb * nb; k += 512) {
            const double2 r0 = *reinterpret_cast<const double2*>(scal + kTileStats * k), r1 = *reinterpret_cast<const double2*>(scal + kTileStats * k + 2);
            v2[0] += r0.x; v2[1] += r0.y;
            tmax[k] = (r1.x == r1.x) ? r1.x : 1e300; tmax[nb * nb + k] = (r1.y == r1.y) ? r1.y : 1e300;
        }
        __syncthreads();
        double bnd = 0.0;
        if (tid < 2 * nb) {
            const int line = tid % nb; const bool col = tid >= nb;
            for (int q = 0; q < nb; ++q) bnd += col ? tmax[nb * nb + q * nb + line] : tmax[line * nb + q];
        }
        const double inf_b = wg8_max((tid < nb) ? bnd : 0.0, red);
        const double one_b = wg8_max((tid >= nb && tid < 2 * nb) ? bnd : 0.0, red);
        wg8_sum<2>(v2, red);
        const double fro2 = v2[0], trA = v2[1];
        double u = sqrt(fro2);
        if (inf_b < u) u = inf_b;
        if (one_b < u) u = one_b;
        double c = u / 2.9;
        const double wmean = (trA > 0.0) ? fro2 / trA : 0.0;
        if (wmean > c && wmean <= u) c = wmean;
        NsState* const st_p = adv(g.st, po);
        const double mean_term = st_p->mean_term, tr1 = hA->tr, tr2 = hB->tr;
        const bool bad = !(fro2 == fro2) || isinf(fro2) || !(trA == trA) || isinf(trA) || !(mean_term == mean_term) || isinf(mean_term);
        const bool zero = !bad && !(c > 0.0);
        const bool flat = trA * trA >= 0.25 * (double)d * fro2;
        const bool scaled = g.scaled && !bad && !zero && u > 0.0 && trA * trA < 0.8 * (double)d * fro2;
        double l0 = 1.0;
        if (scaled) { l0 = ns_l0_from_participation((float)(trA * trA / fro2), d) * g.l0_scale; if (l0 > 0.5) l0 = 0.5; }
        const bool hopeless = !bad && !zero && (c < 0.0078125 || (g.lp_wide ? (scaled && l0 < g.l0_min) || (!scaled && !flat) : !flat));
        double mu0 = 1.0;
        if (scaled && !hopeless) {
            c = u;
            double l = l0;
            mu0 = ns_step_scale(l);
            if (blockIdx.x == 0 && blockIdx.y == 0 && tid == 0) { double ln = l; st_p->mu[0] = mu0; st_p->mu[1] = ns_step_scale(ln); st_p->l_cur = l; }
        } else if (g.scaled && blockIdx.x == 0 && blockIdx.y == 0 && tid == 0) {
            st_p->mu[0] = 1.0; st_p->mu[1] = 1.0; st_p->l_cur = 1.0;
        }
        if (blockIdx.x == 0 && blockIdx.y == 0 && tid == 0) {
            NsState* st = st_p; Ns32State* s32 = adv(g.s32, po);
            st->c = zero ? 1.0 : c * hdr_inv_s12(hA, hB);
            st->tr1 = tr1; st->tr2 = tr2;
            st->res_last = 0.0; st->tr_last = 0.0; st->res_min = 1e300; st->tr_safe = 0.0; st->has_safe = 0;
            st->final_iter = zero ? 0 : -1; st->conv = zero ? 1 : 0;
            st->nonfinite = bad ? 1 : 0; st->done = (bad || zero) ? 1 : 0; st->finished = (bad || zero) ? 1 : 0;
            s32->done = 0; s32->finished = 0; s32->ok = 0; s32->final_iter = -1; s32->failed = 0;
            s32->upd_skip[0] = 0; s32->upd_skip[1] = 0; s32->skip_corr = 1; s32->decided_at = -1; s32->strict = 0; s32->grew = 0;
            s32->res[0] = 1e300;
            if (bad || zero || hopeless) { s32->done = 1; s32->finished = 1; s32->failed = 1; s32->upd_skip[0] = 1; s32->upd_skip[1] = 1; }
        }
        if (bad || zero || hopeless) return;
        inv_cn = 1.0 / c;
        inv_c = inv_cn / hdr_inv_s12(hA, hB);
        m1 = (float)(1.5 * mu0); m3 = (float)(0.5 * mu0 * mu0 * mu0);
    } else if constexpr (!VER) {
        if (g.skip && *adv(g.skip, po) != 0) return;
    }
    f32x16 acc0, acc1;
#pragma unroll
    for (int q = 0; q < 16; ++q) { acc0[q] = 0.f; acc1[q] = 0.f; }
#pragma unroll
    for (int s = 0; s < NS; ++s) {
        acc0 = __builtin_amdgcn_mfma_f32_32x32x16_f16(ah[s], bh[s], acc0, 0, 0, 0);
        acc1 = __builtin_amdgcn_mfma_f32_32x32x16_f16(ah[s], bl[s], acc1, 0, 0, 0);
        acc1 = __builtin_amdgcn_mfma_f32_32x32x16_f16(al[s], bh[s], acc1, 0, 0, 0);
    }
    if (wave >= 4) {
#pragma unroll
        for (int reg = 0; reg < 16; ++reg) part[(wave - 4) * (32 * 33) + ((reg & 3) + 8 * (reg >> 2) + 4 * kg) * 33 + r] = acc0[reg] + acc1[reg] * kLoInv;
    }
    __syncthreads();
    if (wave < 4) {
#pragma unroll
        for (int reg = 0; reg < 16; ++reg) part[wave * (32 * 33) + ((reg & 3) + 8 * (reg >> 2) + 4 * kg) * 33 + r] += acc0[reg] + acc1[reg] * kLoInv;
    }
    __syncthreads();
    float alpha = (MODE == SP_T) ? g.alpha : 1.f, beta = (MODE == SP_T) ? g.beta_eye : 0.f, gamma = g.gamma;
    if (MODE == SP_T && g.scaled) {
        const double m = adv(g.st, po)->mu[g.k];
        alpha = (float)(-0.5 * m * m * m); beta = (float)(1.5 * m); gamma = beta + alpha;
    }
    double ss = 0.0;
    double v4[4] = {0.0, 0.0, 0.0, 0.0};
#pragma unroll
    for (int q = 0; q < 2; ++q) {
        const int o = rr * 33 + 2 * cp + q;
        const float sum = (part[o] + part[(32 * 33) + o]) + (part[2 * (32 * 33) + o] + part[3 * (32 * 33) + o]);
        const bool dg = (row0 + rr) == (col0 + 2 * cp + q);
        if constexpr (MODE == SP_FIRST) {
            const float y0 = (float)((q ? a2.y : a2.x) * inv_c);
            const float y2 = (float)((double)sum * (inv_cn * inv_cn));
            fin[o] = m1 * y0 - m3 * y2;
            fin2[o] = (dg ? m1 : 0.f) - m3 * y0;
        } else if constexpr (MODE == SP_V2) {
            fin[o] = zs ? ((dg ? 1.f : 0.f) - sum) * kVerScale : sum;
        } else if constexpr (MODE == SP_V3) {
            const int gr = row0 + rr, gc = col0 + 2 * cp;
            int half;
            const size_t pi = fa_elem(gr, gc, 0, d, half);
            const SplitMat Pm = adv(g.B[0], po), Em = adv(g.A[1], po);
            const float pt = used16(reinterpret_cast<const _Float16*>(Pm.at + pi)[half + q], reinterpret_cast<const _Float16*>(Pm.at + pi + 64)[half + q]);
            const float pij = used16(reinterpret_cast<const _Float16*>(Pm.a + pi)[half + q], reinterpret_cast<const _Float16*>(Pm.a + pi + 64)[half + q]);
            const float eij = used16(reinterpret_cast<const _Float16*>(Em.a + pi)[half + q], reinterpret_cast<const _Float16*>(Em.a + pi + 64)[half + q]);
            v4[0] += (double)sum * (double)pt; v4[1] += (double)eij * (double)pt; v4[2] += (double)pij * (double)pij; v4[3] += (double)eij * (double)eij;
        } else {
            const float v = alpha * sum + (dg ? beta : 0.f);
            fin[o] = v;
            if constexpr (MODE == SP_T) { const double e = (double)v - (dg ? (double)gamma : 0.0); ss += e * e; }
        }
    }
    if constexpr (MODE == SP_V3) {
        wg8_sum<4>(v4, red);
        if (tid == 0) {
            double* o = adv(g.vstats, (int64_t)blockIdx.z * g.hstride) + (size_t)kVerStats * (ty * gridDim.x + tx);
            o[0] = v4[0]; o[1] = v4[1]; o[2] = v4[2]; o[3] = v4[3];
        }
        return;
    }
    __syncthreads();
    const bool with_digits = ((MODE == SP_FIRST) || (MODE == SP_U && zi == 0)) && g.Cdig[0] != nullptr;
    store_tile(fin, adv(g.C[zi], po), with_digits ? adv(g.Cdig[0], po) : nullptr, with_digits ? adv(g.Cdig_t[0], po) : nullptr, ty, tx, d, tid);
    if constexpr (MODE == SP_FIRST) store_tile(fin2, adv(g.C[1], po), nullptr, nullptr, ty, tx, d, tid);
    if constexpr (MODE == SP_T) {
        double s1[1] = {ss};
        wg8_sum<1>(s1, red);
        if (tid == 0) adv(g.partials, po)[ty * gridDim.x + tx] = s1[0];
    }
}

struct DigArgs {
    int d, gen;
    const MatHdr* hA; const MatHdr* hB; int64_t pstride;
    const Ns32State* s32;
    SplitMat Y[2]; uint4* dig[2]; uint4* dig_t[2];
    int64_t astride;
};
__global__ __launch_bounds__(256) void nsf_digitize(DigArgs g) {
    const int64_t po = (int64_t)blockIdx.z * g.pstride;
    if (hdr_bad(adv(g.hA, (int64_t)blockIdx.z * g.astride), adv(g.hB, po), g.gen)) return;
    const Ns32State* s = adv(g.s32, po);
    if (s->skip_corr) return;
    const int d = g.d, par = s->final_iter & 1;
    const int t = blockIdx.x * 256 + threadIdx.x;
    if (t >= (d * d) >> 4) return;
    const SplitMat Ym = adv(g.Y[par], po);
    const uint4* src = blockIdx.y ? Ym.at : Ym.a;
    uint4* dst = adv(blockIdx.y ? g.dig_t[par] : g.dig[par], po);
    const int lane = t & 63, ksrb = t >> 6, ks = ksrb % (d >> 5), rb = ksrb / (d >> 5);
    const int m = lane & 31, g2 = lane >> 5;
    uint32_t w[kDigits][4];
#pragma unroll
    for (int p = 0; p < kDigits; ++p) { w[p][0] = 0u; w[p][1] = 0u; w[p][2] = 0u; w[p][3] = 0u; }
#pragma unroll
    for (int h = 0; h < 2; ++h) {
        const uint4 uh = src[fa_idx(rb, 2 * ks + g2, 0, 32 * h + m, d)], ul = src[fa_idx(rb, 2 * ks + g2, 1, 32 * h + m, d)];
        f16x8 hi, lo; __builtin_memcpy(&hi, &uh, 16); __builtin_memcpy(&lo, &ul, 16);
#pragma unroll
        for (int j = 0; j < 8; ++j) {
            int dg[kDigits];
            digits_of<float>(used16(hi[j], lo[j]), dg);
            const int byte = 8 * h + j;
#pragma unroll
            for (int p = 0; p < kDigits; ++p) w[p][byte >> 2] |= ((uint32_t)dg[p] & 0xffu) << (8 * (byte & 3));
        }
    }
#pragma unroll
    for (int p = 0; p < kDigits; ++p) dst[dg_idx(rb, ks, p, lane, d)] = make_uint4(w[p][0], w[p][1], w[p][2], w[p][3]);
}

__global__ void nsf_rearm(Ns32State* s32) {
    if (threadIdx.x == 0 && blockIdx.x == 0) {
        s32->done = 0; s32->finished = 0; s32->ok = 0; s32->skip_corr = 1; s32->upd_skip[0] = 0; s32->upd_skip[1] = 0;
        s32->strict = 1;
    }
}

}
}
```

fadtk_amd/csrc/ns_fast_big.h:

```cpp
#pragma once
#include "ns_fast.h"
#include "big_slots.h"

namespace fad {
namespace nsf {

#ifndef FAD_BIG_STAGES
#define FAD_BIG_STAGES 3
#endif
constexpr int kBigStages = FAD_BIG_STAGES;
constexpr int kBigStage = 1024;
constexpr size_t kBigLds = (size_t)kBigStages * kBigStage * 16 + 256;

template <int MODE, int NJ = 2>
__global__ __launch_bounds__(256, (FAD_BIG_STAGES <= 3) ? 3 : ((FAD_BIG_STAGES <= 4) ? 2 : 1)) void nsf_big(SplitArgs g) {
    static_assert(MODE == SP_T || MODE == SP_U || MODE == SP_FIRST, "SP_FIRST: iteration 0 (scale from nsf_i8<A>'s statistics, Y1, Z1)");
    extern __shared__ __attribute__((aligned(16))) uint4 ring[];
    double* red = reinterpret_cast<double*>(ring + kBigStages * kBigStage);
    const int d = g.d, tid = threadIdx.x, lane = tid & 63;
    constexpr int ZP = (MODE == SP_U) ? 2 : 1;
    const int t = d >> 7, tx_n = (NJ == 2) ? t : 2 * t, tt = t * tx_n;
    const int L = blockIdx.x;
    const int nprod = big_grid(g.nprob, tt * ZP);
    if constexpr (MODE == SP_U) {
        if (L >= nprod) { nsf_check<256>(g, (int64_t)(L - nprod) * g.pstride, red); return; }
    }
    const BigSlot slot = big_slot(L, g.nprob, tt * ZP);
    if (!slot.live) return;
    const int song = slot.song, zi = slot.item / tt, tile = slot.item - zi * tt;
    const int TY = tile / tx_n, TX = tile - TY * tx_n;
    const int64_t po = (int64_t)song * g.pstride;
    const MatHdr* hB = adv(g.hB, po);
    const MatHdr* hA = adv(g.hA, (int64_t)song * g.astride);
    if (hdr_bad(hA, hB, g.gen)) return;
    double inv_c = 0.0, inv_cn = 0.0;
    float m1 = 1.5f, m3 = 0.5f;
    if constexpr (MODE == SP_FIRST) {
        const int nb = d >> 5;
        const double* scal = adv(g.statsA, po);
        double* tmax = reinterpret_cast<double*>(ring);
        double v2[2] = {0.0, 0.0};
        for (int k = tid; k < nb * nb; k += 256) {
            const double2 r0 = *reinterpret_cast<const double2*>(scal + kTileStats * k), r1 = *reinterpret_cast<const double2*>(scal + kTileStats * k + 2);
            v2[0] += r0.x; v2[1] += r0.y;
            tmax[k] = (r1.x == r1.x) ? r1.x : 1e300; tmax[nb * nb + k] = (r1.y == r1.y) ? r1.y : 1e300;
        }
        __syncthreads();
        double bnd = 0.0;
        if (tid < 2 * nb) {
            const int line = tid % nb; const bool col = tid >= nb;
            for (int q = 0; q < nb; ++q) bnd += col ? tmax[nb * nb + q * nb + line] : tmax[line * nb + q];
        }
        const double inf_b = wg8_max<4>((tid < nb) ? bnd : 0.0, red);
        const double one_b = wg8_max<4>((tid >= nb && tid < 2 * nb) ? bnd : 0.0, red);
        wg8_sum<2, 4>(v2, red);
        const double fro2 = v2[0], trA = v2[1];
        double u = sqrt(fro2);
        if (inf_b < u) u = inf_b;
        if (one_b < u) u = one_b;
        double c = u / 2.9;
        const double wmean = (trA > 0.0) ? fro2 / trA : 0.0;
        if (wmean > c && wmean <= u) c = wmean;
        NsState* const st_p = adv(g.st, po);
        const double mean_term = st_p->mean_term, tr1 = hA->tr, tr2 = hB->tr;
        const bool bad = !(fro2 == fro2) || isinf(fro2) || !(trA == trA) || isinf(trA) || !(mean_term == mean_term) || isinf(mean_term);
        const bool zero = !bad && !(c > 0.0);
        const bool flat = trA * trA >= 0.25 * (double)d * fro2;
        const bool want_scaled = g.scaled && !bad && !zero && u > 0.0 && trA * trA < 0.8 * (double)d * fro2;
        double l0 = 1.0;
        if (want_scaled) { l0 = ns_l0_from_participation((float)(trA * trA / fro2), d) * g.l0_scale; if (l0 > 0.5) l0 = 0.5; }
        const bool hopeless = !bad && !zero && (c < 0.0078125 || (g.lp_wide ? (want_scaled && l0 < g.l0_min) || (!want_scaled && !flat) : !flat));
        const bool scaled = want_scaled && !hopeless;
        double mu0 = 1.0;
        if (scaled) {
            c = u;
            double l = l0;
            mu0 = ns_step_scale(l);
            if (tile == 0 && tid == 0) { double ln = l; st_p->mu[0] = mu0; st_p->mu[1] = ns_step_scale(ln); st_p->l_cur = l; }
        } else if (g.scaled && tile == 0 && tid == 0) {
            st_p->mu[0] = 1.0; st_p->mu[1] = 1.0; st_p->l_cur = 1.0;
        }
        if (tile == 0 && tid == 0) {
            NsState* st = st_p; Ns32State* s32 = adv(g.s32, po);
            st->c = zero ? 1.0 : c * hdr_inv_s12(hA, hB);
            st->tr1 = tr1; st->tr2 = tr2;
            st->res_last = 0.0; st->tr_last = 0.0; st->res_min = 1e300; st->tr_safe = 0.0; st->has_safe = 0;
            st->final_iter = zero ? 0 : -1; st->conv = zero ? 1 : 0;
            st->nonfinite = bad ? 1 : 0; st->done = (bad || zero) ? 1 : 0; st->finished = (bad || zero) ? 1 : 0;
            s32->done = 0; s32->finished = 0; s32->ok = 0; s32->final_iter = -1; s32->failed = 0;
            s32->upd_skip[0] = 0; s32->upd_skip[1] = 0; s32->skip_corr = 1; s32->decided_at = -1; s32->strict = 0; s32->grew = 0;
            s32->res[0] = 1e300;
            if (bad || zero || hopeless) { s32->done = 1; s32->finished = 1; s32->failed = 1; s32->upd_skip[0] = 1; s32->upd_skip[1] = 1; }
        }
        if (bad || zero || hopeless) return;
        inv_cn = 1.0 / c;
        inv_c = inv_cn / hdr_inv_s12(hA, hB);
        m1 = (float)(1.5 * mu0); m3 = (float)(0.5 * mu0 * mu0 * mu0);
        __syncthreads();
    } else {
        if (g.skip && *adv(g.skip, po) != 0) return;
    }
    const int wave = __builtin_amdgcn_readfirstlane(tid >> 6);
    const int wr = wave >> 1, wc = wave & 1;
#ifdef FAD_BIG_ABL_NOLOOP
    const int nks = 0;
#else
    const int nks = d >> 4;
#endif

    const SplitMat Am = adv(g.A[zi], po), Bm = adv(g.B[zi], po);
    constexpr int PP = 2 + NJ;
    constexpr int STG = kBigStage, NST = kBigStages;
    const uint32_t voff = (uint32_t)lane * 16u;
    const uint32_t ring_lds = (uint32_t)(size_t)(__attribute__((address_space(3))) void*)ring;
    auto issue = [&](int ks) {
        const int kk = ks;
#pragma unroll
        for (int q = 0; q < PP; ++q) {
            const int piece = wave * PP + q;
            const bool bside = piece >= 8;
            const int blk = (bside ? piece - 8 : piece) >> 1, plane = piece & 1;
            const uint4* src_mat = bside ? Bm.at : Am.a;
            const int blk_global = bside ? 2 * NJ * TX + blk : 4 * TY + blk;
            const uint64_t sb = (uint64_t)(src_mat + fa_idx(blk_global, kk, plane, 0, d));
            const uint32_t lo = __builtin_amdgcn_readfirstlane((uint32_t)sb);
            const uint32_t hi = __builtin_amdgcn_readfirstlane((uint32_t)(sb >> 32));
            const uint64_t ub = ((uint64_t)hi << 32) | lo;
            const uint32_t dst = ring_lds + (uint32_t)(((ks % NST) * STG + piece * 64) * 16);
            const uint32_t m0v = __builtin_amdgcn_readfirstlane(dst);
            asm volatile("s_mov_b32 m0, %2\n\ts_nop 0\n\tglobal_load_lds_dwordx4 %0, %1" ::"v"(voff), "s"(ub), "s"(m0v) : "memory", "m0");
        }
    };
    f32x16 acc0[2][NJ], acc1[2][NJ];
#pragma unroll
    for (int i = 0; i < 2; ++i)
#pragma unroll
        for (int j = 0; j < NJ; ++j)
#pragma unroll
            for (int q = 0; q < 16; ++q) { acc0[i][j][q] = 0.f; acc1[i][j][q] = 0.f; }

    for (int ks = 0; ks < NST - 1 && ks < nks; ++ks) issue(ks);
    for (int ks = 0; ks < nks; ++ks) {
        const int ahead = (nks - 1 - ks < NST - 2) ? (nks - 1 - ks) : (NST - 2);
        switch (ahead * PP) {
            case 24: asm volatile("s_waitcnt vmcnt(24)" ::: "memory"); break;
            case 20: asm volatile("s_waitcnt vmcnt(20)" ::: "memory"); break;
            case 18: asm volatile("s_waitcnt vmcnt(18)" ::: "memory"); break;
            case 16: asm volatile("s_waitcnt vmcnt(16)" ::: "memory"); break;
            case 15: asm volatile("s_waitcnt vmcnt(15)" ::: "memory"); break;
            case 12: asm volatile("s_waitcnt vmcnt(12)" ::: "memory"); break;
            case 9: asm volatile("s_waitcnt vmcnt(9)" ::: "memory"); break;
            case 8: asm volatile("s_waitcnt vmcnt(8)" ::: "memory"); break;
            case 6: asm volatile("s_waitcnt vmcnt(6)" ::: "memory"); break;
            case 4: asm volatile("s_waitcnt vmcnt(4)" ::: "memory"); break;
            case 3: asm volatile("s_waitcnt vmcnt(3)" ::: "memory"); break;
            default: asm volatile("s_waitcnt vmcnt(0)" ::: "memory"); break;
        }
        __builtin_amdgcn_s_barrier();
        if (ks + NST - 1 < nks) issue(ks + NST - 1);
        const f16x8* st = reinterpret_cast<const f16x8*>(ring + (ks % NST) * STG) + lane;
        f16x8 ah[2], al[2], bh[NJ], bl[NJ];
#pragma unroll
        for (int i = 0; i < 2; ++i) { ah[i] = st[((2 * wr + i) * 2) * 64]; al[i] = st[((2 * wr + i) * 2 + 1) * 64]; }
#pragma unroll
        for (int j = 0; j < NJ; ++j) { bh[j] = st[(8 + (NJ * wc + j) * 2) * 64]; bl[j] = st[(8 + (NJ * wc + j) * 2 + 1) * 64]; }
#pragma unroll
        for (int i = 0; i < 2; ++i)
#pragma unroll
            for (int j = 0; j < NJ; ++j) {
                acc0[i][j] = __builtin_amdgcn_mfma_f32_32x32x16_f16(ah[i], bh[j], acc0[i][j], 0, 0, 0);
                acc1[i][j] = __builtin_amdgcn_mfma_f32_32x32x16_f16(ah[i], bl[j], acc1[i][j], 0, 0, 0);
                acc1[i][j] = __builtin_amdgcn_mfma_f32_32x32x16_f16(al[i], bh[j], acc1[i][j], 0, 0, 0);
            }
    }
    __syncthreads();
#ifdef FAD_BIG_ABL_NOEPI
    if (acc0[0][0][0] != 12345.678f) return;
#endif

    float* fin = reinterpret_cast<float*>(ring) + wave * (32 * 33 + 32);
    const int kg = lane >> 5, r = lane & 31;
    float alpha = (MODE == SP_T) ? g.alpha : 1.f, beta = (MODE == SP_T) ? g.beta_eye : 0.f, gamma = g.gamma;
    if (MODE == SP_T && g.scaled) {
        const double m = adv(g.st, po)->mu[g.k];
        alpha = (float)(-0.5 * m * m * m); beta = (float)(1.5 * m); gamma = beta + alpha;
    }
    const SplitMat Cm = adv(g.C[zi], po);
    const bool with_digits = (MODE == SP_U) && zi == 0 && g.Cdig[0];
    uint4* dig = with_digits ? adv(g.Cdig[0], po) : nullptr;
    uint4* dig_t = with_digits ? adv(g.Cdig_t[0], po) : nullptr;
    double ss = 0.0;
#pragma unroll
    for (int i = 0; i < 2; ++i)
#pragma unroll
        for (int j = 0; j < NJ; ++j) {
            const int by = 4 * TY + 2 * wr + i, bx = 2 * NJ * TX + NJ * wc + j;
            if constexpr (MODE == SP_FIRST) {
                const double* A64 = adv(g.A64, po) + (int64_t)(32 * by + 4 * kg) * d + 32 * bx + r;
                float z1[16];
#pragma unroll
                for (int reg = 0; reg < 16; ++reg) {
                    const int q = (reg & 3) + 8 * (reg >> 2);
                    const float y0 = (float)(A64[(int64_t)q * d] * inv_c);
                    const float y2 = (float)((double)(acc0[i][j][reg] + acc1[i][j][reg] * kLoInv) * (inv_cn * inv_cn));
                    fin[(q + 4 * kg) * 33 + r] = m1 * y0 - m3 * y2;
                    z1[reg] = ((by == bx && q + 4 * kg == r) ? m1 : 0.f) - m3 * y0;
                }
                __builtin_amdgcn_wave_barrier();
#pragma unroll
                for (int pass = 0; pass < 4; ++pass) store_tile_planes(fin, Cm, by, bx, d, pass * 64 + lane);
                __builtin_amdgcn_wave_barrier();
#pragma unroll
                for (int reg = 0; reg < 16; ++reg) fin[((reg & 3) + 8 * (reg >> 2) + 4 * kg) * 33 + r] = z1[reg];
                __builtin_amdgcn_wave_barrier();
                const SplitMat Zm1 = adv(g.C[1], po);
#pragma unroll
                for (int pass = 0; pass < 4; ++pass) store_tile_planes(fin, Zm1, by, bx, d, pass * 64 + lane);
                __builtin_amdgcn_wave_barrier();
                continue;
            }
            float ssf = 0.f;
#pragma unroll
            for (int reg = 0; reg < 16; ++reg) {
                const int q = (reg & 3) + 8 * (reg >> 2) + 4 * kg;
                const bool dg = (by == bx) && (q == r);
                const float v = alpha * (acc0[i][j][reg] + acc1[i][j][reg] * kLoInv) + (dg ? beta : 0.f);
                if constexpr (MODE == SP_T) { const float e = v - (dg ? gamma : 0.f); ssf = __builtin_fmaf(e, e, ssf); }
                fin[q * 33 + r] = v;
            }
            ss += (double)ssf;
            __builtin_amdgcn_wave_barrier();
#pragma unroll
            for (int pass = 0; pass < 4; ++pass) store_tile_planes(fin, Cm, by, bx, d, pass * 64 + lane);
            if (with_digits) {
#pragma unroll 2
                for (int pass = 0; pass < 8; ++pass) store_tile_digits(fin, dig, dig_t, by, bx, d, pass * 64 + lane);
            }
            __builtin_amdgcn_wave_barrier();
        }
    if constexpr (MODE == SP_T) {
        double s1[1] = {ss};
        wg8_sum<1, 4>(s1, red);
        if (tid == 0) adv(g.partials, po)[tile] = s1[0];
    }
}

constexpr int kI8BigStage = 36 * 64;
#ifndef FAD_I8_BIG_STAGES
#define FAD_I8_BIG_STAGES 2
#endif
constexpr int kI8BigStages = FAD_I8_BIG_STAGES;
constexpr size_t kI8BigLds = (size_t)kI8BigStages * kI8BigStage * 16 + 256;

template <int MODE, bool WITHR = false>
__global__ __launch_bounds__(512) void nsf_i8_big(I8Args g, int nprob) {
    extern __shared__ __attribute__((aligned(16))) uint4 ring[];
    double* red = reinterpret_cast<double*>(ring + kI8BigStages * kI8BigStage);
    constexpr int kUmin = (MODE == I8_A) ? kUminA : kUminG;
    constexpr int kGroups = 2 * (kDigits - 1) - kUmin + 1;
    const int d = g.d, tid = threadIdx.x, lane = tid & 63;
    const int tr_ = d >> 7, tc_ = d >> 6, tt = tr_ * tc_;
    const BigSlot slot = big_slot(blockIdx.x, nprob, tt);
    if (!slot.live) return;
    const int song = slot.song, tile = slot.item;
    const int TY = tile / tc_, TX = tile - TY * tc_;
    const int64_t po = (int64_t)song * g.pstride, ho = (int64_t)song * g.hstride;
    const MatHdr* hB = adv(g.hB, po);
    const MatHdr* hA = adv(g.hA, (int64_t)song * g.astride);
    NsState* const st_p = adv(g.st, po);
    const bool bad = hdr_bad(hA, hB, g.gen);
    const bool skipped = bad || (g.skip && *adv(g.skip, po) != 0);
    if constexpr (MODE == I8_G) {
        if (tile == 0 && tid == 0) {
            const NsState* st = st_p; const Ns32State* s = adv(g.s32, po);
            int* hw = adv(g.host_words, ho); double* hv = adv(g.host_vals, ho);
            hw[0] = bad ? 1 : 0; hw[1] = st->done; hw[2] = st->nonfinite; hw[3] = st->too_few[0]; hw[4] = st->too_few[1];
            hw[5] = s->ok; hw[6] = s->failed; hw[7] = s->final_iter; hw[8] = s->decided_at; hw[9] = s->strict; hw[10] = s->finished;
            hw[11] = skipped ? 1 : 0;
            hv[0] = st->c; hv[1] = st->tr1; hv[2] = st->tr2; hv[3] = st->mean_term;
#pragma unroll
            for (int q = 0; q < 16; ++q) hv[4 + q] = s->res[q];
            hw[14] = (g.scaled && st->mu[0] != 1.0) ? 1 : 0;
            hw[12] = g.gen;
        }
    }
    if (skipped) return;
    const int wave = __builtin_amdgcn_readfirstlane(tid >> 6);
    const int wr = wave >> 1, wc = wave & 1;
    const bool alt = (MODE == I8_G) && g.sel && (*adv(g.sel, po) & 1);
    const uint4* Ad = (MODE == I8_A) ? adv(g.Adig, (int64_t)song * g.astride) : adv(alt ? g.Adig_alt : g.Adig, po);
    const uint4* Bd = adv(alt ? g.Bdig_alt : g.Bdig, po);
#ifdef FAD_I8_ABL_G_NOLOOP
    const int nks = (MODE == I8_G) ? 0 : (d >> 5);
#else
    const int nks = d >> 5;
#endif

    const uint32_t voff = (uint32_t)lane * 16u;
    const uint32_t ring_lds = (uint32_t)(size_t)(__attribute__((address_space(3))) void*)ring;
    auto issue = [&](int ks) {
#pragma unroll
        for (int i = 0; i < 5; ++i) {
            const int q = wave + 8 * i;
            if (q < 36) {
                const bool bs = q >= 24;
                const int blk = bs ? (q - 24) / 6 : q / 6, p = bs ? (q - 24) % 6 : q % 6;
                const uint64_t sb = (uint64_t)((bs ? Bd : Ad) + dg_idx((bs ? 2 * TX : 4 * TY) + blk, ks, p, 0, d));
                const uint32_t lo = __builtin_amdgcn_readfirstlane((uint32_t)sb);
                const uint32_t hi = __builtin_amdgcn_readfirstlane((uint32_t)(sb >> 32));
                const uint64_t ub = ((uint64_t)hi << 32) | lo;
                const uint32_t m0v = __builtin_amdgcn_readfirstlane(ring_lds + (uint32_t)(((ks % kI8BigStages) * kI8BigStage + q * 64) * 16));
                asm volatile("s_mov_b32 m0, %2\n\ts_nop 0\n\tglobal_load_lds_dwordx4 %0, %1" ::"v"(voff), "s"(ub), "s"(m0v) : "memory", "m0");
            }
        }
    };
    i32x16 acc[kGroups];
#pragma unroll
    for (int u = 0; u < kGroups; ++u)
#pragma unroll
        for (int q = 0; q < 16; ++q) acc[u][q] = 0;
    static_assert(kI8BigStages >= 2 && kI8BigStages <= 4, "the counted waits below cover two younger stages at most");
    for (int ks = 0; ks < kI8BigStages - 1 && ks < nks; ++ks) issue(ks);
    const bool five = wave < 4;
    for (int ks = 0; ks < nks; ++ks) {
        const int ahead = (nks - 1 - ks < kI8BigStages - 2) ? (nks - 1 - ks) : (kI8BigStages - 2);
        if (ahead == 2) { if (five) asm volatile("s_waitcnt vmcnt(10)" ::: "memory"); else asm volatile("s_waitcnt vmcnt(8)" ::: "memory"); }
        else if (ahead == 1) { if (five) asm volatile("s_waitcnt vmcnt(5)" ::: "memory"); else asm volatile("s_waitcnt vmcnt(4)" ::: "memory"); }
        else asm volatile("s_waitcnt vmcnt(0)" ::: "memory");
        __builtin_amdgcn_s_barrier();
#ifndef FAD_I8_ABL_NODMA
        if (ks + kI8BigStages - 1 < nks) issue(ks + kI8BigStages - 1);
#endif
        const i32x4* st = reinterpret_cast<const i32x4*>(ring + (ks % kI8BigStages) * kI8BigStage) + lane;
        i32x4 a[kDigits], b[kDigits];
#pragma unroll
        for (int p = 0; p < kDigits; ++p) { a[p] = st[(wr * 6 + p) * 64]; b[p] = st[(24 + wc * 6 + p) * 64]; }
#ifdef FAD_I8_ABL_NOMMA
#pragma unroll
        for (int p = 0; p < kDigits; ++p) { acc[0][p] += a[p][0] ^ b[p][1]; acc[1][p] += a[p][2] ^ b[p][3]; }
#else
#pragma unroll
        for (int p = kDigits - 1; p >= 0; --p)
#pragma unroll
            for (int q = kDigits - 1; q >= 0; --q)
                if (p + q >= kUmin) acc[p + q - kUmin] = __builtin_amdgcn_mfma_i32_32x32x32_i8(a[p], b[q], acc[p + q - kUmin], 0, 0, 0);
#endif
    }
    __syncthreads();
    double gp[16];
#pragma unroll
    for (int q = 0; q < 16; ++q) gp[q] = 0.0;
#pragma unroll
    for (int u = 0; u < kGroups; ++u) {
        const double wgt = __builtin_ldexp(1.0, 7 * (u + kUmin) - 80);
#pragma unroll
        for (int q = 0; q < 16; ++q) gp[q] = __builtin_fma((double)acc[u][q], wgt, gp[q]);
    }
    float* fin = reinterpret_cast<float*>(ring) + wave * (32 * 33 + 32);
    const int kg = lane >> 5, n = lane & 31;
    const int by = 4 * TY + wr, bx = 2 * TX + wc, nb = d >> 5;
    const int row0 = 32 * by, col0 = 32 * bx;
    double* const stats = adv(g.stats, (MODE == I8_A) ? po : ho);
    double* scal = stats + (size_t)kTileStats * (by * nb + bx);
    double v3[3] = {0.0, 0.0, 0.0};
    if constexpr (MODE == I8_A) {
        const double inv = hdr_inv_s12(hA, hB);
        double* A64 = adv(g.A64, po) + (int64_t)(row0 + 4 * kg) * d + col0 + n;
#pragma unroll
        for (int reg = 0; reg < 16; ++reg) {
            const int q = (reg & 3) + 8 * (reg >> 2);
            A64[(int64_t)q * d] = gp[reg] * inv;
            fin[(q + 4 * kg) * 33 + n] = (float)gp[reg];
            v3[0] += gp[reg] * gp[reg];
            if (by == bx && q + 4 * kg == n) v3[1] += gp[reg];
        }
        __builtin_amdgcn_wave_barrier();
        const SplitMat Pm = adv(g.P, po);
#pragma unroll
        for (int pass = 0; pass < 4; ++pass) store_tile_planes(fin, Pm, by, bx, d, pass * 64 + lane);
    } else {
        const SplitMat Zm = adv(g.Z[alt ? 1 : 0], po);
        const SplitMat Ym = adv(g.Y[alt ? 1 : 0], po);
        const double inv_c = 1.0 / st_p->c;
        const double* A64 = adv(g.A64in, po) + (int64_t)(row0 + 4 * kg) * d + col0 + n;
        typedef _Float16 f16x4 __attribute__((ext_vector_type(4)));
        f16x4 zh[4], zl[4];
#pragma unroll
        for (int j = 0; j < 4; ++j) {
            int half;
            const size_t zi = fa_elem(col0 + n, row0 + 8 * j + 4 * kg, 0, d, half);
            zh[j] = *reinterpret_cast<const f16x4*>(reinterpret_cast<const _Float16*>(Zm.a + zi) + half);
            zl[j] = *reinterpret_cast<const f16x4*>(reinterpret_cast<const _Float16*>(Zm.a + zi + 64) + half);
        }
#pragma unroll
        for (int reg = 0; reg < 16; ++reg) {
            const int q = (reg & 3) + 8 * (reg >> 2), gr = row0 + q + 4 * kg, gc = col0 + n;
            const double R = A64[(int64_t)q * d] * inv_c - gp[reg];
            if constexpr (WITHR) gp[reg] = R;
            const double z = (double)used16(zh[reg >> 2][reg & 3], zl[reg >> 2][reg & 3]);
            v3[0] += z * R; v3[1] += R * R;
            if (by == bx && gr == gc) {
                int hy;
                const size_t yi = fa_elem(gr, gr, 0, d, hy);
                v3[2] += (double)used16(reinterpret_cast<const _Float16*>(Ym.a + yi)[hy], reinterpret_cast<const _Float16*>(Ym.a + yi + 64)[hy]);
            }
            fin[(q + 4 * kg) * 33 + n] = fabsf((float)z);
        }
        __builtin_amdgcn_wave_barrier();
    }
    double m = 0.0;
    if constexpr (MODE == I8_A) {
        if (lane < 32) { for (int c = 0; c < 32; ++c) m += fabsf(fin[lane * 33 + c]); }
        else { for (int q = 0; q < 32; ++q) m += fabsf(fin[q * 33 + lane - 32]); }
    } else {
        if (lane < 32) { for (int q = 0; q < 32; ++q) m += fin[q * 33 + lane]; }
        else { for (int c = 0; c < 32; ++c) m += fin[(lane - 32) * 33 + c]; }
    }
    double mrow = (lane < 32) ? m : 0.0, mcol = (lane >= 32) ? m : 0.0;
#pragma unroll
    for (int off = 32; off > 0; off >>= 1) {
        mrow = fmax(mrow, __shfl_xor(mrow, off)); mcol = fmax(mcol, __shfl_xor(mcol, off));
#pragma unroll
        for (int q = 0; q < 3; ++q) v3[q] += __shfl_xor(v3[q], off);
    }
    if (lane == 0) {
        if constexpr (MODE == I8_A) {
            scal[0] = v3[0]; scal[1] = v3[1]; scal[2] = mrow; scal[3] = mcol;
        } else {
            scal[0] = v3[0]; scal[1] = v3[1]; scal[2] = v3[2]; scal[3] = 0.0;
            double* zmax = stats + (size_t)kTileStats * nb * nb + 2 * (size_t)(by * nb + bx);
            zmax[0] = mrow; zmax[1] = mcol;
        }
    }
    if constexpr (MODE == I8_G && WITHR) {
        if (g.Rv.a) {
            __builtin_amdgcn_wave_barrier();
#pragma unroll
            for (int reg = 0; reg < 16; ++reg) fin[((reg & 3) + 8 * (reg >> 2) + 4 * kg) * 33 + n] = (float)(gp[reg] * (double)kVerScale);
            __builtin_amdgcn_wave_barrier();
            const SplitMat Rm = adv(g.Rv, po);
#pragma unroll
            for (int pass = 0; pass < 4; ++pass) store_tile_planes(fin, Rm, by, bx, d, pass * 64 + lane);
        }
    }
    (void)red;
}

}
}
```

fadtk_amd/csrc/ns_fast_res.h:

```cpp
#pragma once
#include "ns_fast.h"

namespace fad {
namespace nsf {

constexpr size_t kResLds = 2 * 65536 + 1024;
constexpr size_t kResLdsFull = kResLds + 6 * 4 * 1024;

struct ResArgs {
    int gen, max_low;
    double thr_pred;
    const MatHdr* hA; const MatHdr* hB; int64_t pstride;
    double* A64; const double* statsA;
    NsState* st; Ns32State* s32;
    SplitMat Y[2], Z[2];
    const uint4* Adig; const uint4* Bdig;
    int64_t hstride; double* stats; int* host_words; double* host_vals;
    int scaled; double l0_scale;
};

__device__ __forceinline__ int res_lds_off(int row, int col) {
    const int c = col & 15;
    return (((row >> 5) * 8 + (col >> 4)) * 2) * 1024 + (32 * ((c >> 2) & 1) + (row & 31)) * 16 + 2 * ((c & 3) + 4 * (c >> 3));
}

template <bool FULL>
__global__ __launch_bounds__(256) void nsf_res128(ResArgs g) {
    extern __shared__ __attribute__((aligned(16))) char lds[];
    char* const P = lds;
    char* const Q = lds + 65536;
    double* const red = reinterpret_cast<double*>(lds + 131072);
    constexpr int d = 128, nb = 4;
    const int tid = threadIdx.x, lane = tid & 63;
    const int j = __builtin_amdgcn_readfirstlane(tid >> 6);
    const int n = lane & 31, kg = lane >> 5;
    const int64_t po = (int64_t)blockIdx.x * g.pstride, ho = (int64_t)blockIdx.x * g.hstride;
    const MatHdr* hB = adv(g.hB, po);
    NsState* const st = adv(g.st, po);
    Ns32State* const s32 = adv(g.s32, po);
    auto rowc = [](int reg) { return (reg & 3) + 8 * (reg >> 2); };
    auto snapshot = [&](bool bad, bool skipped) {
        if constexpr (FULL) {
            int* hw = adv(g.host_words, ho); double* hv = adv(g.host_vals, ho);
            hw[0] = bad ? 1 : 0; hw[1] = st->done; hw[2] = st->nonfinite; hw[3] = st->too_few[0]; hw[4] = st->too_few[1];
            hw[5] = s32->ok; hw[6] = s32->failed; hw[7] = s32->final_iter; hw[8] = s32->decided_at; hw[9] = s32->strict; hw[10] = s32->finished;
            hw[11] = skipped ? 1 : 0;
            hv[0] = st->c; hv[1] = st->tr1; hv[2] = st->tr2; hv[3] = st->mean_term;
            for (int q = 0; q < 16; ++q) hv[4 + q] = s32->res[q];
            hw[12] = g.gen;
        }
    };
    if (hdr_bad(g.hA, hB, g.gen)) { if (tid == 0) snapshot(true, true); return; }

    double fro2_l = 0.0, tr_l = 0.0, colsum_max = 0.0;
    if constexpr (FULL) {
        constexpr int kGroups = 2 * (kDigits - 1) - kUminA + 1;
        i32x4 bd[4][kDigits];
        {
            const i32x4* pb = reinterpret_cast<const i32x4*>(adv(g.Bdig, po) + dg_idx(j, 0, 0, lane, d));
#pragma unroll
            for (int ks = 0; ks < 4; ++ks)
#pragma unroll
                for (int p = 0; p < kDigits; ++p) bd[ks][p] = pb[(ks * kDigits + p) * 64];
        }
        const double inv12 = hdr_inv_s12(g.hA, hB);
        double* A64 = adv(g.A64, po) + (int64_t)(4 * kg) * d + 32 * j + n;
        double cs = 0.0;
#pragma unroll 1
        for (int rbo = 0; rbo < 4; ++rbo) {
            i32x16 acc[kGroups];
#pragma unroll
            for (int u = 0; u < kGroups; ++u)
#pragma unroll
                for (int q = 0; q < 16; ++q) acc[u][q] = 0;
            const i32x4* pa = reinterpret_cast<const i32x4*>(g.Adig + dg_idx(rbo, 0, 0, lane, d));
#pragma unroll
            for (int ks = 0; ks < 4; ++ks) {
                i32x4 a[kDigits];
#pragma unroll
                for (int p = 0; p < kDigits; ++p) a[p] = pa[(ks * kDigits + p) * 64];
#pragma unroll
                for (int p = kDigits - 1; p >= 0; --p)
#pragma unroll
                    for (int q = kDigits - 1; q >= 0; --q)
                        if (p + q >= kUminA) acc[p + q - kUminA] = __builtin_amdgcn_mfma_i32_32x32x32_i8(a[p], bd[ks][q], acc[p + q - kUminA], 0, 0, 0);
            }
#pragma unroll
            for (int q = 0; q < 16; ++q) {
                double v = 0.0;
#pragma unroll
                for (int u = 0; u < kGroups; ++u) v = __builtin_fma((double)acc[u][q], __builtin_ldexp(1.0, 7 * (u + kUminA) - 80), v);
                A64[(int64_t)(32 * rbo + rowc(q)) * d] = v * inv12;
                fro2_l += v * v; cs += fabs(v);
                if (rbo == j && rowc(q) + 4 * kg == n) tr_l += v;
            }
        }
        cs += __shfl_xor(cs, 32);
        colsum_max = cs;
    }

    double c, inv_c;
    double mu = 1.0, l_cur = 1.0;
    {
        double inf_b = 1e300, one_b = 1e300;
        double v2[2] = {0.0, 0.0};
        if constexpr (FULL) {
            one_b = wg8_max<4>(colsum_max, red);
            v2[0] = fro2_l; v2[1] = tr_l;
            __syncthreads();
            wg8_sum<2, 4>(v2, red + 32);
        } else {
            const double* scal = adv(g.statsA, po);
            double* tmax = red;
            if (tid < nb * nb) {
                v2[0] = scal[kTileStats * tid]; v2[1] = scal[kTileStats * tid + 1];
                const double r0 = scal[kTileStats * tid + 2], r1 = scal[kTileStats * tid + 3];
                tmax[tid] = (r0 == r0) ? r0 : 1e300; tmax[16 + tid] = (r1 == r1) ? r1 : 1e300;
            }
            __syncthreads();
            inf_b = 0.0; one_b = 0.0;
            for (int line = 0; line < nb; ++line) {
                double rs = 0.0, cs = 0.0;
                for (int q = 0; q < nb; ++q) { rs += tmax[line * nb + q]; cs += tmax[16 + q * nb + line]; }
                inf_b = fmax(inf_b, rs); one_b = fmax(one_b, cs);
            }
            __syncthreads();
            wg8_sum<2, 4>(v2, red + 32);
        }
        const double fro2 = v2[0], trA = v2[1];
        double u = sqrt(fro2);
        if (inf_b < u) u = inf_b;
        if (one_b < u) u = one_b;
        c = u / 2.9;
        const double wmean = (trA > 0.0) ? fro2 / trA : 0.0;
        if (wmean > c && wmean <= u) c = wmean;
        const double mean_term = st->mean_term, tr1 = g.hA->tr, tr2 = hB->tr;
        const bool bad = !(fro2 == fro2) || isinf(fro2) || !(trA == trA) || isinf(trA) || !(mean_term == mean_term) || isinf(mean_term);
        const bool zero = !bad && !(c > 0.0);
        const bool hopeless = !bad && !zero && (trA * trA < 0.25 * (double)d * fro2 || c < 0.0078125);
        if (g.scaled && !bad && !zero && !hopeless && u > 0.0 && trA * trA < 0.8 * (double)d * fro2) {
            c = u;
            l_cur = ns_l0_from_participation((float)(trA * trA / fro2), d) * g.l0_scale;
            if (l_cur > 0.5) l_cur = 0.5;
            mu = ns_step_scale(l_cur);
        }
        if (tid == 0) {
            st->c = zero ? 1.0 : c * hdr_inv_s12(g.hA, hB);
            st->tr1 = tr1; st->tr2 = tr2;
            st->res_last = 0.0; st->tr_last = 0.0; st->res_min = 1e300; st->tr_safe = 0.0; st->has_safe = 0;
            st->final_iter = zero ? 0 : -1; st->conv = zero ? 1 : 0;
            st->nonfinite = bad ? 1 : 0; st->done = (bad || zero) ? 1 : 0; st->finished = (bad || zero) ? 1 : 0;
            s32->done = 0; s32->finished = 0; s32->ok = 0; s32->final_iter = -1; s32->failed = 0;
            s32->upd_skip[0] = 0; s32->upd_skip[1] = 0; s32->skip_corr = 1; s32->decided_at = -1; s32->strict = 0; s32->grew = 0;
            s32->res[0] = 1e300;
            if (bad || zero || hopeless) { s32->done = 1; s32->finished = 1; s32->failed = 1; s32->upd_skip[0] = 1; s32->upd_skip[1] = 1; snapshot(false, true); }
        }
        if (bad || zero || hopeless) return;
        inv_c = 1.0 / (c * hdr_inv_s12(g.hA, hB));
    }

    const int scat_base = res_lds_off(4 * kg, 32 * j + n);
    auto scatter = [&](char* buf, const f16x8 (&Bh)[8], const f16x8 (&Bl)[8]) {
        char* p = buf + scat_base;
#pragma unroll
        for (int rbo = 0; rbo < 4; ++rbo)
#pragma unroll
            for (int reg = 0; reg < 16; ++reg) {
                const int off = rbo * 16384 + rowc(reg) * 16;
                *reinterpret_cast<_Float16*>(p + off) = Bh[2 * rbo + (reg >> 3)][reg & 7];
                *reinterpret_cast<_Float16*>(p + off + 1024) = Bl[2 * rbo + (reg >> 3)][reg & 7];
            }
    };
    auto product = [&](const char* buf, const f16x8 (&Bh)[8], const f16x8 (&Bl)[8], f16x8 (&Oh)[8], f16x8 (&Ol)[8], auto f) {
        const f16x8* a = reinterpret_cast<const f16x8*>(buf) + lane;
        f32x16 p0, p1;
        auto convert = [&](int rbo, const f32x16& c0, const f32x16& c1) {
#pragma unroll
            for (int q = 0; q < 16; ++q) {
                const float t = f(rbo, q, c0[q] + c1[q] * kLoInv);
                _Float16 h, l; split16(t, h, l);
                Oh[2 * rbo + (q >> 3)][q & 7] = h; Ol[2 * rbo + (q >> 3)][q & 7] = l;
            }
        };
#pragma unroll
        for (int rbo = 0; rbo < 4; ++rbo) {
            f32x16 a0, a1;
#pragma unroll
            for (int q = 0; q < 16; ++q) { a0[q] = 0.f; a1[q] = 0.f; }
#pragma unroll
            for (int ks = 0; ks < 8; ++ks) {
                const f16x8 ah = a[((rbo * 8 + ks) * 2) * 64], al = a[((rbo * 8 + ks) * 2 + 1) * 64];
                a0 = __builtin_amdgcn_mfma_f32_32x32x16_f16(ah, Bh[ks], a0, 0, 0, 0);
                a1 = __builtin_amdgcn_mfma_f32_32x32x16_f16(ah, Bl[ks], a1, 0, 0, 0);
                a1 = __builtin_amdgcn_mfma_f32_32x32x16_f16(al, Bh[ks], a1, 0, 0, 0);
            }
            if (rbo > 0) convert(rbo - 1, p0, p1);
            p0 = a0; p1 = a1;
            __builtin_amdgcn_sched_barrier(0x2 | 0x4 | 0x8);
        }
        convert(3, p0, p1);
    };
    auto ident = [](int, int, float x) { return x; };

    f16x8 Yh[8], Yl[8], Zh[8], Zl[8], Th[8], Tl[8];
    {
        const double* A64 = adv(g.A64, po) + (int64_t)(4 * kg) * d + 32 * j + n;
        const float a0 = (float)(0.5 * mu * mu * mu), b0 = (float)(1.5 * mu);
#pragma unroll
        for (int rbo = 0; rbo < 4; ++rbo)
#pragma unroll
            for (int reg = 0; reg < 16; ++reg) {
                float y0 = (float)(A64[(int64_t)(32 * rbo + rowc(reg)) * d] * inv_c);
                asm volatile("" : "+v"(y0));
                const float t0 = ((rbo == j && rowc(reg) + 4 * kg == n) ? b0 : 0.f) - a0 * y0;
                _Float16 h, l;
                split16(y0, h, l); Yh[2 * rbo + (reg >> 3)][reg & 7] = h; Yl[2 * rbo + (reg >> 3)][reg & 7] = l;
                split16(t0, h, l); Th[2 * rbo + (reg >> 3)][reg & 7] = h; Tl[2 * rbo + (reg >> 3)][reg & 7] = l;
            }
        scatter(Q, Yh, Yl);
        scatter(P, Th, Tl);
#pragma unroll
        for (int ks = 0; ks < 8; ++ks) { Zh[ks] = Th[ks]; Zl[ks] = Tl[ks]; }
        __syncthreads();
        product(Q, Th, Tl, Yh, Yl, ident);
        __syncthreads();
        scatter(Q, Yh, Yl);
        __syncthreads();
    }

    int final_iter = -1, decided_at = -1, ok = 0, failed = 0;
    double prev = 1e300;
    bool grew = false;
    for (int k = 1;; ++k) {
        float ss = 0.f;
        {
            double lk = l_cur;
            mu = g.scaled ? ns_step_scale(lk) : 1.0;
            if (g.scaled && k > 1) { const double cap = ns_scale_cap(prev, d); if (cap < mu) mu = cap; }
        }
        const float ak = (float)(0.5 * mu * mu * mu), gk = (float)(1.5 * mu - 0.5 * mu * mu * mu);
        product(P, Yh, Yl, Th, Tl, [&](int rbo, int reg, float m) {
            const bool dg = rbo == j && rowc(reg) + 4 * kg == n;
            const float e = (dg ? ak : 0.f) - ak * m;
            ss += e * e;
            return dg ? e + gk : e;
        });
        double s1[1] = {(double)ss};
        wg8_sum<1, 4>(s1, red);
        const double res = sqrt(s1[0]) / (0.5 * mu * mu * mu);
        if (g.scaled) {
            if (res == res && res < 1.0) { const double lr = sqrt(1.0 - res); if (lr > l_cur) l_cur = lr; }
            (void)ns_step_scale_with(mu, l_cur);
        }
        if (tid == 0 && k < 16) s32->res[k] = res;
        const bool finite = (res == res) && !isinf(res);
        const bool grows = k >= 4 && res > prev && res > 1e-3;
        const bool give_up = grows && (!g.scaled || grew);
        grew = grows;
        if (!finite || k + 1 >= g.max_low || give_up) { failed = 1; final_iter = k; decided_at = k; break; }
        if (res <= 1e-3 && (res > 0.3 * prev || res <= 1e-6)) { ok = 1; final_iter = k; decided_at = k; break; }
        const double bound = 0.75 * res * res + 0.25 * res * res * res;
        const bool last = bound <= g.thr_pred && mu == 1.0;
        prev = res;
        scatter(P, Th, Tl);
        product(Q, Th, Tl, Yh, Yl, ident);
        __syncthreads();
        scatter(Q, Yh, Yl);
        product(P, Zh, Zl, Th, Tl, ident);
        __syncthreads();
#pragma unroll
        for (int ks = 0; ks < 8; ++ks) { Zh[ks] = Th[ks]; Zl[ks] = Tl[ks]; }
        scatter(P, Zh, Zl);
        __syncthreads();
        if (last) { ok = 1; final_iter = k + 1; decided_at = k; break; }
    }
    if (tid == 0) {
        s32->finished = 1; s32->done = 1; s32->final_iter = final_iter; s32->decided_at = decided_at;
        s32->ok = ok; s32->failed = failed; s32->skip_corr = ok ? 0 : 1;
        s32->upd_skip[0] = 1; s32->upd_skip[1] = 1;
        if (!ok) snapshot(false, true);
    }
    if (!ok) return;
    __syncthreads();

    if constexpr (FULL) {
        char* const DG = lds + 131072 + 1024;
        constexpr int kGroups = 2 * (kDigits - 1) - kUminG + 1;
        double try_l = 0.0, zcol = 0.0;
#pragma unroll
        for (int ks = 0; ks < 8; ++ks)
#pragma unroll
            for (int i = 0; i < 8; ++i) zcol += (double)fabsf(used16(Zh[ks][i], Zl[ks][i]));
        zcol += __shfl_xor(zcol, 32);
#pragma unroll
        for (int rbo = 0; rbo < 4; ++rbo)
#pragma unroll
            for (int reg = 0; reg < 16; ++reg)
                if (rbo == j && rowc(reg) + 4 * kg == n) try_l += (double)used16(Yh[2 * rbo + (reg >> 3)][reg & 7], Yl[2 * rbo + (reg >> 3)][reg & 7]);
        i32x4 yd[4][kDigits];
#pragma unroll
        for (int ks = 0; ks < 4; ++ks) {
            uint32_t w[kDigits][4];
#pragma unroll
            for (int p = 0; p < kDigits; ++p) { w[p][0] = 0u; w[p][1] = 0u; w[p][2] = 0u; w[p][3] = 0u; }
#pragma unroll
            for (int sl = 0; sl < 16; ++sl) {
                int dg[kDigits];
                digits_of<float>(used16(Yh[2 * ks + (sl >> 3)][sl & 7], Yl[2 * ks + (sl >> 3)][sl & 7]), dg);
#pragma unroll
                for (int p = 0; p < kDigits; ++p) w[p][sl >> 2] |= ((uint32_t)dg[p] & 0xffu) << (8 * (sl & 3));
            }
#pragma unroll
            for (int p = 0; p < kDigits; ++p) { yd[ks][p][0] = (int)w[p][0]; yd[ks][p][1] = (int)w[p][1]; yd[ks][p][2] = (int)w[p][2]; yd[ks][p][3] = (int)w[p][3]; }
        }
        double zrow = 0.0;
        if (tid < d) {
            const f16x8* zp = reinterpret_cast<const f16x8*>(P) + ((tid >> 5) * 8 * 2) * 64 + (tid & 31);
            for (int ks = 0; ks < 8; ++ks)
#pragma unroll
                for (int gg = 0; gg < 2; ++gg) {
                    const f16x8 h = zp[(2 * ks) * 64 + 32 * gg], l = zp[(2 * ks + 1) * 64 + 32 * gg];
#pragma unroll
                    for (int i = 0; i < 8; ++i) zrow += (double)fabsf(used16(h[i], l[i]));
                }
        }
        const double zinf = wg8_max<4>(zrow, red), zone = wg8_max<4>(zcol, red);
        double corr_l = 0.0, r2_l = 0.0;
        const double* A64 = adv(g.A64, po) + (int64_t)(4 * kg) * d + 32 * j + n;
#pragma unroll 1
        for (int rbo = 0; rbo < 4; ++rbo) {
            {
                const int ks = tid >> 6;
                const f16x8* yq = reinterpret_cast<const f16x8*>(Q) + ((rbo * 8 + 2 * ks) * 2) * 64 + lane;
                const f16x8 h0 = yq[0], l0 = yq[64], h1 = yq[128], l1 = yq[192];
                uint32_t w[kDigits][4];
#pragma unroll
                for (int p = 0; p < kDigits; ++p) { w[p][0] = 0u; w[p][1] = 0u; w[p][2] = 0u; w[p][3] = 0u; }
#pragma unroll
                for (int sl = 0; sl < 16; ++sl) {
                    int dg[kDigits];
                    digits_of<float>(sl < 8 ? used16(h0[sl & 7], l0[sl & 7]) : used16(h1[sl & 7], l1[sl & 7]), dg);
#pragma unroll
                    for (int p = 0; p < kDigits; ++p) w[p][sl >> 2] |= ((uint32_t)dg[p] & 0xffu) << (8 * (sl & 3));
                }
#pragma unroll
                for (int p = 0; p < kDigits; ++p)
                    *reinterpret_cast<uint4*>(DG + ((ks * kDigits + p) * 64 + lane) * 16) = make_uint4(w[p][0], w[p][1], w[p][2], w[p][3]);
            }
            __syncthreads();
            i32x16 acc[kGroups];
#pragma unroll
            for (int u = 0; u < kGroups; ++u)
#pragma unroll
                for (int q = 0; q < 16; ++q) acc[u][q] = 0;
#pragma unroll
            for (int ks = 0; ks < 4; ++ks) {
                i32x4 a[kDigits];
#pragma unroll
                for (int p = 0; p < kDigits; ++p) a[p] = *reinterpret_cast<const i32x4*>(DG + ((ks * kDigits + p) * 64 + lane) * 16);
#pragma unroll
                for (int p = kDigits - 1; p >= 0; --p)
#pragma unroll
                    for (int q = kDigits - 1; q >= 0; --q)
                        if (p + q >= kUminG) acc[p + q - kUminG] = __builtin_amdgcn_mfma_i32_32x32x32_i8(a[p], yd[ks][q], acc[p + q - kUminG], 0, 0, 0);
            }
#pragma unroll
            for (int q = 0; q < 16; ++q) {
                double G = 0.0;
#pragma unroll
                for (int u = 0; u < kGroups; ++u) G = __builtin_fma((double)acc[u][q], __builtin_ldexp(1.0, 7 * (u + kUminG) - 80), G);
                const double R = A64[(int64_t)(32 * rbo + rowc(q)) * d] * inv_c - G;
                r2_l += R * R;
                const int o = res_lds_off(32 * j + n, 32 * rbo + rowc(q) + 4 * kg);
                const double z = (double)used16(*reinterpret_cast<const _Float16*>(P + o), *reinterpret_cast<const _Float16*>(P + o + 1024));
                corr_l += z * R;
            }
            __syncthreads();
        }
        double v3[3] = {corr_l, r2_l, try_l};
        wg8_sum<3, 4>(v3, red);
        if (tid == 0) {
            double* stats = adv(g.stats, ho);
            for (int q = 0; q < (kTileStats + 2) * nb * nb; ++q) stats[q] = 0.0;
            stats[0] = v3[0]; stats[1] = v3[1]; stats[2] = v3[2];
            stats[kTileStats * nb * nb] = zinf; stats[kTileStats * nb * nb + 1] = zone;
            snapshot(false, false);
        }
        return;
    }

    const int par = final_iter & 1;
    const SplitMat Yo = adv(g.Y[par], po), Zo = adv(g.Z[par], po);
    for (int t = tid; t < 4 * 8 * 64; t += 256) {
        const int ln = t & 63, ks = (t >> 6) & 7, rb = t >> 9;
        const int m = ln & 31, g2 = ln >> 5;
        f16x8 yh, yl, yth, ytl, zth, ztl;
#pragma unroll
        for (int i = 0; i < 8; ++i) {
            const int row = 32 * rb + m, k = 16 * ks + 8 * g2 + i;
            const int o = res_lds_off(row, k), ot = res_lds_off(k, row);
            yh[i] = *reinterpret_cast<const _Float16*>(Q + o); yl[i] = *reinterpret_cast<const _Float16*>(Q + o + 1024);
            yth[i] = *reinterpret_cast<const _Float16*>(Q + ot); ytl[i] = *reinterpret_cast<const _Float16*>(Q + ot + 1024);
            zth[i] = *reinterpret_cast<const _Float16*>(P + ot); ztl[i] = *reinterpret_cast<const _Float16*>(P + ot + 1024);
        }
        uint4 u;
        __builtin_memcpy(&u, &yh, 16); Yo.a[fa_idx(rb, ks, 0, ln, d)] = u;
        __builtin_memcpy(&u, &yl, 16); Yo.a[fa_idx(rb, ks, 1, ln, d)] = u;
        __builtin_memcpy(&u, &yth, 16); Yo.at[fa_idx(rb, ks, 0, ln, d)] = u;
        __builtin_memcpy(&u, &ytl, 16); Yo.at[fa_idx(rb, ks, 1, ln, d)] = u;
        __builtin_memcpy(&u, &zth, 16); Zo.at[fa_idx(rb, ks, 0, ln, d)] = u;
        __builtin_memcpy(&u, &ztl, 16); Zo.at[fa_idx(rb, ks, 1, ln, d)] = u;
    }
}

}
}
```

Before: 11920.

## Use 5-plane 8-bit digit format for batched int8 MFMA Frechet products

Adds a parameterized digit-plane format and switches the batched and resident Frechet paths from six signed 7-bit planes to five 8-bit two's-complement planes. Fewer planes cut the number of int8 MFMA cross products and the digit storage and load traffic per tile. The digit split now goes through a 64-bit integer path and uses different truncation thresholds, so the accuracy margins and int32 accumulation headroom change. It also moves the small-path digit generation for Y out of the split kernel into the common digit pass.

```diff
diff --git a/fadtk_amd/csrc/frechet.hip b/fadtk_amd/csrc/frechet.hip
--- a/fadtk_amd/csrc/frechet.hip
+++ b/fadtk_amd/csrc/frechet.hip
@@ -321,17 +321,17 @@
     else hipLaunchKernelGGL((nsf::nsf_i8_big<nsf::I8_G>), dim3(grid), dim3(512), nsf::kI8BigLds, st, g, (int)B);
     return FAD_OK;
 }
-template <int NS8> static void fast_launch_i8(int mode, unsigned t, unsigned B, const nsf::I8Args& g, hipStream_t st) {
-    if (mode == nsf::I8_A) hipLaunchKernelGGL((nsf::nsf_i8<NS8, nsf::I8_A>), dim3(t, t, B), dim3(512), 0, st, g);
-    else hipLaunchKernelGGL((nsf::nsf_i8<NS8, nsf::I8_G>), dim3(t, t, B), dim3(512), 0, st, g);
-}
-static void fast_i8(int d, int mode, const nsf::I8Args& g, hipStream_t st, unsigned B = 1) {
+template <int NS8, class PL> static void fast_launch_i8(int mode, unsigned t, unsigned B, const nsf::I8Args& g, hipStream_t st) {
+    if (mode == nsf::I8_A) hipLaunchKernelGGL((nsf::nsf_i8<NS8, nsf::I8_A, PL>), dim3(t, t, B), dim3(512), 0, st, g);
+    else hipLaunchKernelGGL((nsf::nsf_i8<NS8, nsf::I8_G, PL>), dim3(t, t, B), dim3(512), 0, st, g);
+}
+template <class PL = nsf::Planes128> static void fast_i8(int d, int mode, const nsf::I8Args& g, hipStream_t st, unsigned B = 1) {
     const unsigned t = (unsigned)(d / 32);
     switch (d) {
-        case 128: case 256: fast_launch_i8<1>(mode, t, B, g, st); break;
-        case 384: case 512: fast_launch_i8<2>(mode, t, B, g, st); break;
-        case 768: fast_launch_i8<3>(mode, t, B, g, st); break;
-        default: fast_launch_i8<4>(mode, t, B, g, st); break;
+        case 128: case 256: fast_launch_i8<1, PL>(mode, t, B, g, st); break;
+        case 384: case 512: fast_launch_i8<2, PL>(mode, t, B, g, st); break;
+        case 768: fast_launch_i8<3, PL>(mode, t, B, g, st); break;
+        default: fast_launch_i8<4, PL>(mode, t, B, g, st); break;
     }
 }
 
@@ -548,7 +548,7 @@
     pa.dig[0] = dig_b; pa.dig[1] = reinterpret_cast<uint4*>(at(L.digS));
     pa.st = reinterpret_cast<NsState*>(at(L.st)); pa.hdr[0] = hdr_b; pa.hdr[1] = reinterpret_cast<nsf::MatHdr*>(at(L.hdr));
     pa.batch = 1; pa.pstride = (int64_t)L.stride;
-    hipLaunchKernelGGL(nsf::nsf_prepare, dim3((unsigned)(dd / 2048), (unsigned)(1 + B)), dim3(512), 0, st, pa);
+    hipLaunchKernelGGL(nsf::nsf_prepare_batch, dim3((unsigned)(dd / 2048), (unsigned)(1 + B)), dim3(512), 0, st, pa);
 
     NsState* st0 = reinterpret_cast<NsState*>(at(L.st));
     Ns32State* s32_0 = reinterpret_cast<Ns32State*>(at(L.s32));
@@ -573,7 +573,7 @@
         a.hB = reinterpret_cast<nsf::MatHdr*>(at(L.hdr)); a.pstride = (int64_t)L.stride; a.stats = stats; a.A64 = A64; a.P = P; a.st = st0;
         if (res_full) {  }
         else if (big && d >= 256) FAD_TRY(fast_i8_big(d, nsf::I8_A, a, st, (unsigned)B, device));
-        else fast_i8(d, nsf::I8_A, a, st, (unsigned)B);
+        else fast_i8<nsf::Planes256>(d, nsf::I8_A, a, st, (unsigned)B);
         if (resident) {
             static std::atomic<unsigned> ready{0};
             if (device >= 0 && device < 32 && !(ready.load(std::memory_order_acquire) & (1u << device))) {
@@ -637,7 +637,7 @@
             a.Y[0] = Y[0]; a.Y[1] = Y[1]; a.Z[0] = Z[0]; a.Z[1] = Z[1]; a.s32 = s32_0; a.host_words = h_words; a.host_vals = h_vals;
             for (int64_t b = 0; b < B; ++b) reinterpret_cast<int*>(reinterpret_cast<char*>(h_words) + b * hs)[12] = 0;
             if (big && d >= 256) FAD_TRY(fast_i8_big(d, nsf::I8_G, a, st, (unsigned)B, device));
-            else fast_i8(d, nsf::I8_G, a, st, (unsigned)B);
+            else fast_i8<nsf::Planes256>(d, nsf::I8_G, a, st, (unsigned)B);
         }
         FAD_HIP_TRY(hipGetLastError());
         FAD_HIP_TRY(hipStreamSynchronize(st));
@@ -770,7 +770,7 @@
     pa.st = st0; pa.hdr[0] = hA; pa.hdr[1] = hB;
     pa.batch = 2; pa.pstride = (int64_t)L.stride; pa.no_covs = 1;
     pa.per = ((dd / 2048) % 4 == 0) ? 4 : 2;
-    hipLaunchKernelGGL(nsf::nsf_prepare, dim3((unsigned)(dd / 2048 / pa.per + 1), (unsigned)(2 * B)), dim3(512), 0, st, pa);
+    hipLaunchKernelGGL(nsf::nsf_prepare_batch, dim3((unsigned)(dd / 2048 / pa.per + 1), (unsigned)(2 * B)), dim3(512), 0, st, pa);
 
     auto split_args = [&]() {
         nsf::SplitArgs g;
@@ -786,11 +786,11 @@
         a.Adig = reinterpret_cast<uint4*>(at(L.digA)); a.Bdig = reinterpret_cast<uint4*>(at(L.digB)); a.d = d; a.gen = gen; a.hA = hA; a.hB = hB;
         a.pstride = (int64_t)L.stride; a.astride = (int64_t)L.stride; a.stats = stats; a.A64 = A64; a.P = P; a.st = st0;
         if (big) FAD_TRY(fast_i8_big(d, nsf::I8_A, a, st, (unsigned)B, device));
-        else fast_i8(d, nsf::I8_A, a, st, (unsigned)B);
+        else fast_i8<nsf::Planes256>(d, nsf::I8_A, a, st, (unsigned)B);
         nsf::SplitArgs g = split_args();
         g.A[0] = P; g.B[0] = P; g.C[0] = Y[1]; g.C[1] = Z[1]; g.A64 = A64; g.statsA = stats;
         if (big) FAD_TRY(fast_split_big(d, nsf::SP_FIRST, g, st, (unsigned)B, device));
-        else { g.Cdig[0] = digY[1]; g.Cdig_t[0] = digYt[1]; fast_split(d, nsf::SP_FIRST, g, st, (unsigned)B); }
+        else fast_split(d, nsf::SP_FIRST, g, st, (unsigned)B);
     }
     int want = ws.pool ? ws.pool->lp_iters : 5;
     if (want < 2) want = 2;
@@ -804,13 +804,12 @@
         else fast_split(d, nsf::SP_T, g, st, (unsigned)B);
         g = split_args();
         g.A[0] = Y[cur]; g.B[0] = T; g.C[0] = Y[cur ^ 1]; g.A[1] = T; g.B[1] = Z[cur]; g.C[1] = Z[cur ^ 1];
-        if (!big) { g.Cdig[0] = digY[cur ^ 1]; g.Cdig_t[0] = digYt[cur ^ 1]; }
         g.skip = &s32_0->upd_skip[k & 1];
         g.k = k; g.max_low = max_low; g.nslots = big ? fast_big_t_slots(d, (unsigned)B) : nb * nb; g.chk_partials = partials; g.thr_pred = pred_threshold(ws.pool, d);
         if (big) FAD_TRY(fast_split_big(d, nsf::SP_U, g, st, (unsigned)B, device));
         else fast_split(d, nsf::SP_U, g, st, (unsigned)B);
     }
-    if (big) {
+    {
         nsf::DigArgs dg;
         memset(&dg, 0, sizeof(dg));
         dg.d = d; dg.gen = gen; dg.hA = hA; dg.hB = hB; dg.pstride = (int64_t)L.stride; dg.astride = (int64_t)L.stride; dg.s32 = s32_0;
@@ -827,7 +826,7 @@
         if (wide) { a.Rv = mat(L.Rv); a.scaled = 1; }
         for (int b = 0; b < B; ++b) { int* w = reinterpret_cast<int*>(reinterpret_cast<char*>(h_words) + (size_t)b * hs); w[12] = 0; w[13] = 0; }
         if (big) FAD_TRY(fast_i8_big(d, nsf::I8_G, a, st, (unsigned)B, device));
-        else fast_i8(d, nsf::I8_G, a, st, (unsigned)B);
+        else fast_i8<nsf::Planes256>(d, nsf::I8_G, a, st, (unsigned)B);
     }
     FAD_HIP_TRY(hipGetLastError());
     if (!ws.done_ev) FAD_HIP_TRY(hipEventCreateWithFlags(&ws.done_ev, hipEventDisableTiming));
diff --git a/fadtk_amd/csrc/ns_digits.h b/fadtk_amd/csrc/ns_digits.h
--- /dev/null
+++ b/fadtk_amd/csrc/ns_digits.h
@@ -0,0 +1,56 @@
+#pragma once
+#include <stddef.h>
+#include <stdint.h>
+
+namespace fad {
+namespace nsf {
+
+enum { I8_A = 0, I8_G = 1 };
+
+template <int BITS, int PLANES, int FRAC, int UMIN_A, int UMIN_G> struct DigitPlanes {
+    static constexpr int kBits = BITS, kPlanes = PLANES, kFrac = FRAC;
+    static constexpr int kUminA = UMIN_A, kUminG = UMIN_G;
+    template <int MODE> static constexpr int umin() { return MODE == I8_A ? UMIN_A : UMIN_G; }
+    template <int MODE> static constexpr int groups() { return 2 * (PLANES - 1) - umin<MODE>() + 1; }
+    static constexpr int weight_exp(int s) { return BITS * s - 2 * FRAC; }
+};
+typedef DigitPlanes<7, 6, 40, 3, 4> Planes128;
+typedef DigitPlanes<8, 5, 37, 2, 3> Planes256;
+
+constexpr int kDigits = Planes128::kPlanes;
+constexpr int kUminA = Planes128::kUminA, kUminG = Planes128::kUminG;
+
+template <class P = Planes128>
+__device__ __host__ __forceinline__ size_t dg_idx(int rb, int ks, int p, int lane, int d) {
+    return (((size_t)rb * (size_t)(d >> 5) + (size_t)ks) * P::kPlanes + (size_t)p) * 64 + (size_t)lane;
+}
+template <class P = Planes128>
+__device__ __host__ __forceinline__ size_t dg_elem(int row, int k, int p, int d, int& byte) {
+    byte = k & 15;
+    return dg_idx<P>(row >> 5, k >> 5, p, 32 * ((k >> 4) & 1) + (row & 31), d);
+}
+
+template <class P, typename F> __device__ __host__ __forceinline__ void digits_of(F v, int (&dg)[P::kPlanes]) {
+    static_assert(P::kBits == 7 || P::kBits == 8, "formats: Planes128, Planes256");
+    if constexpr (P::kBits == 7) {
+        F t = v * (F)32;
+#pragma unroll
+        for (int p = P::kPlanes - 1; p >= 0; --p) {
+            const F r = (sizeof(F) == 4) ? (F)__builtin_rintf((float)t) : (F)__builtin_rint((double)t);
+            dg[p] = (int)r;
+            t = (t - r) * (F)128;
+        }
+    } else {
+        int64_t V = (int64_t)__builtin_rint(__builtin_ldexp((double)v, P::kFrac));
+#pragma unroll
+        for (int p = 0; p < P::kPlanes - 1; ++p) {
+            const int b = (int)(int8_t)(uint8_t)(V & 0xff);
+            dg[p] = b;
+            V = (V - b) >> 8;
+        }
+        dg[P::kPlanes - 1] = (int)V;
+    }
+}
+
+}
+}
diff --git a/fadtk_amd/csrc/ns_fast.h b/fadtk_amd/csrc/ns_fast.h
--- a/fadtk_amd/csrc/ns_fast.h
+++ b/fadtk_amd/csrc/ns_fast.h
@@ -1,6 +1,7 @@
 #pragma once
 #include "fad_common.h"
 #include "ns_check.h"
+#include "ns_digits.h"
 #include "ns32.h"
 #include "ns_mean.h"
 
@@ -12,34 +13,15 @@
 typedef _Float16 f16x8 __attribute__((ext_vector_type(8)));
 typedef _Float16 f16x2 __attribute__((ext_vector_type(2)));
 
-constexpr int kDigits = 6;
-constexpr int kUminA = 3, kUminG = 4;
 constexpr float kLoScale = 2048.f, kLoInv = 1.f / 2048.f;
 constexpr int kTileStats = 4;
 
 __device__ __host__ __forceinline__ size_t fa_idx(int rb, int ks, int plane, int lane, int d) {
     return (((size_t)rb * (size_t)(d >> 4) + (size_t)ks) * 2 + (size_t)plane) * 64 + (size_t)lane;
-}
-__device__ __host__ __forceinline__ size_t dg_idx(int rb, int ks, int p, int lane, int d) {
-    return (((size_t)rb * (size_t)(d >> 5) + (size_t)ks) * kDigits + (size_t)p) * 64 + (size_t)lane;
 }
 __device__ __host__ __forceinline__ size_t fa_elem(int row, int k, int plane, int d, int& half) {
     half = k & 7;
     return fa_idx(row >> 5, k >> 4, plane, 32 * ((k >> 3) & 1) + (row & 31), d);
-}
-__device__ __host__ __forceinline__ size_t dg_elem(int row, int k, int p, int d, int& byte) {
-    byte = k & 15;
-    return dg_idx(row >> 5, k >> 5, p, 32 * ((k >> 4) & 1) + (row & 31), d);
-}
-
-template <typename F> __device__ __forceinline__ void digits_of(F v, int (&dg)[kDigits]) {
-    F t = v * (F)32;
-#pragma unroll
-    for (int p = kDigits - 1; p >= 0; --p) {
-        const F r = (sizeof(F) == 4) ? (F)__builtin_rintf((float)t) : (F)__builtin_rint((double)t);
-        dg[p] = (int)r;
-        t = (t - r) * (F)128;
-    }
 }
 
 __device__ __forceinline__ void split16(float v, _Float16& hi, _Float16& lo) {
@@ -129,7 +111,7 @@
 
 __device__ __forceinline__ double prep_cov(double m, double sr, double sk, double inv_n, double inv_nd) { return (m - (sr * sk) * inv_n) * inv_nd; }
 
-__global__ __launch_bounds__(512) void nsf_prepare(PrepArgs a) {
+template <class PL> __device__ __forceinline__ void prepare_body(const PrepArgs& a) {
     __shared__ double red[8 * 2];
     __shared__ double mu_lds[2 * 1024];
     __shared__ float gaps[1024];
@@ -212,9 +194,9 @@
             row = 32 * rb + r; k0 = 32 * ks + 16 * g + 4 * qd;
             fetch();
         }
-        uint32_t w[kDigits];
-#pragma unroll
-        for (int p = 0; p < kDigits; ++p) w[p] = 0u;
+        uint32_t w[PL::kPlanes];
+#pragma unroll
+        for (int p = 0; p < PL::kPlanes; ++p) w[p] = 0u;
         double* cov_out = acc ? adv(a.covs, po) + (int64_t)set * d * d + (int64_t)row * d + k0 : nullptr;
 #pragma unroll
         for (int q = 0; q < 4; ++q) {
@@ -223,16 +205,18 @@
             const double v = c0 * s;
             const bool fits = fabs(v) <= 1.9375;
             off_grid = off_grid || !fits;
-            int dg[kDigits];
-            digits_of<double>((bad || !fits) ? 0.0 : v, dg);
-#pragma unroll
-            for (int p = 0; p < kDigits; ++p) w[p] |= ((uint32_t)dg[p] & 0xffu) << (8 * q);
-        }
-#pragma unroll
-        for (int p = 0; p < kDigits; ++p) reinterpret_cast<uint32_t*>(out + dg_idx(rb, ks, p, 32 * g + r, d))[qd] = w[p];
+            int dg[PL::kPlanes];
+            digits_of<PL, double>((bad || !fits) ? 0.0 : v, dg);
+#pragma unroll
+            for (int p = 0; p < PL::kPlanes; ++p) w[p] |= ((uint32_t)dg[p] & 0xffu) << (8 * q);
+        }
+#pragma unroll
+        for (int p = 0; p < PL::kPlanes; ++p) reinterpret_cast<uint32_t*>(out + dg_idx<PL>(rb, ks, p, 32 * g + r, d))[qd] = w[p];
     }
     if (off_grid) hdr->flag_gen = a.gen;
 }
+__global__ __launch_bounds__(512) void nsf_prepare(PrepArgs a) { prepare_body<Planes128>(a); }
+__global__ __launch_bounds__(512) void nsf_prepare_batch(PrepArgs a) { prepare_body<Planes256>(a); }
 
 __global__ __launch_bounds__(512) void nsf_pairs_covs(PrepArgs a) {
     const int d = a.d, set = (int)(blockIdx.y & 1);
@@ -271,23 +255,23 @@
     {
         const bool tr = tid < 256;
         const int u = tid & 255, ln = u & 31, q = u >> 5;
-        uint32_t w[kDigits];
-#pragma unroll
-        for (int p = 0; p < kDigits; ++p) w[p] = 0u;
+        uint32_t w[Planes128::kPlanes];
+#pragma unroll
+        for (int p = 0; p < Planes128::kPlanes; ++p) w[p] = 0u;
 #pragma unroll
         for (int j = 0; j < 4; ++j) {
             const float v = tr ? fin[(4 * q + j) * 33 + ln] : fin[ln * 33 + 4 * q + j];
             _Float16 h, l; split16(v, h, l);
-            int dg[kDigits];
-            digits_of<float>(used16(h, l), dg);
-#pragma unroll
-            for (int p = 0; p < kDigits; ++p) w[p] |= ((uint32_t)dg[p] & 0xffu) << (8 * j);
+            int dg[Planes128::kPlanes];
+            digits_of<Planes128, float>(used16(h, l), dg);
+#pragma unroll
+            for (int p = 0; p < Planes128::kPlanes; ++p) w[p] |= ((uint32_t)dg[p] & 0xffu) << (8 * j);
         }
         uint4* base = tr ? dig_t : dig;
         const int rb = tr ? tx : ty, ks = tr ? ty : tx, lane = 32 * (q >> 2) + ln;
 #pragma unroll
-        for (int p = 0; p < kDigits; ++p)
-            reinterpret_cast<uint32_t*>(base + dg_idx(rb, ks, p, lane, d))[q & 3] = w[p];
+        for (int p = 0; p < Planes128::kPlanes; ++p)
+            reinterpret_cast<uint32_t*>(base + dg_idx<Planes128>(rb, ks, p, lane, d))[q & 3] = w[p];
     }
 }
 __device__ __forceinline__ void store_tile(const float* fin, const SplitMat& X, uint4* dig, uint4* dig_t, int ty, int tx, int d, int tid) {
@@ -296,7 +280,6 @@
 }
 
 
-enum { I8_A = 0, I8_G = 1 };
 constexpr int kHostWords = 16, kHostVals = 24;
 struct I8Args {
     const uint4* Adig; const uint4* Bdig;
@@ -320,14 +303,13 @@
 constexpr float kVerScale = 4096.f;
 constexpr int kVerStats = 4;
 
-template <int NS8, int MODE>
+template <int NS8, int MODE, class PL = Planes128>
 __global__ __launch_bounds__(512) void nsf_i8(I8Args g) {
     __shared__ __attribute__((aligned(16))) double part[2 * 32 * 33];
     __shared__ float fin[32 * 33];
     __shared__ float finR[(MODE == I8_G) ? 32 * 33 : 1];
     __shared__ double red[8 * 4];
-    constexpr int kUmin = (MODE == I8_A) ? kUminA : kUminG;
-    constexpr int kGroups = 2 * (kDigits - 1) - kUmin + 1;
+    constexpr int kUmin = PL::template umin<MODE>(), kGroups = PL::template groups<MODE>(), kPl = PL::kPlanes;
     const int d = g.d, tid = threadIdx.x, lane = tid & 63;
     const int64_t po = (int64_t)blockIdx.z * g.pstride, ho = (int64_t)blockIdx.z * g.hstride;
     const MatHdr* hB = adv(g.hB, po);
@@ -360,12 +342,12 @@
     const bool idle = wave * NS8 >= (d >> 5);
 
     constexpr int NBUF = (NS8 <= 2) ? NS8 : 2;
-    i32x4 a[NBUF][kDigits], b[NBUF][kDigits];
+    i32x4 a[NBUF][kPl], b[NBUF][kPl];
     auto fetch = [&](int buf, int s) {
-        const i32x4* pa = reinterpret_cast<const i32x4*>(Ad + dg_idx(ty, wave * NS8 + s, 0, lane, d));
-        const i32x4* pb = reinterpret_cast<const i32x4*>(Bd + dg_idx(tx, wave * NS8 + s, 0, lane, d));
-#pragma unroll
-        for (int m = kDigits - 1; m >= 0; --m) { a[buf][m] = pa[64 * m]; b[buf][m] = pb[64 * m]; }
+        const i32x4* pa = reinterpret_cast<const i32x4*>(Ad + dg_idx<PL>(ty, wave * NS8 + s, 0, lane, d));
+        const i32x4* pb = reinterpret_cast<const i32x4*>(Bd + dg_idx<PL>(tx, wave * NS8 + s, 0, lane, d));
+#pragma unroll
+        for (int m = kPl - 1; m >= 0; --m) { a[buf][m] = pa[64 * m]; b[buf][m] = pb[64 * m]; }
     };
     i32x16 acc[kGroups];
 #pragma unroll
@@ -374,12 +356,12 @@
         for (int q = 0; q < 16; ++q) acc[u][q] = 0;
     auto mma = [&](int buf) {
 #pragma unroll
-        for (int m = kDigits - 1; m >= 0; --m) {
-#pragma unroll
-            for (int q = kDigits - 1; q >= m; --q)
+        for (int m = kPl - 1; m >= 0; --m) {
+#pragma unroll
+            for (int q = kPl - 1; q >= m; --q)
                 if (m + q >= kUmin) acc[m + q - kUmin] = __builtin_amdgcn_mfma_i32_32x32x32_i8(a[buf][m], b[buf][q], acc[m + q - kUmin], 0, 0, 0);
 #pragma unroll
-            for (int p = kDigits - 1; p > m; --p)
+            for (int p = kPl - 1; p > m; --p)
                 if (p + m >= kUmin) acc[p + m - kUmin] = __builtin_amdgcn_mfma_i32_32x32x32_i8(a[buf][p], b[buf][m], acc[p + m - kUmin], 0, 0, 0);
         }
     };
@@ -402,7 +384,7 @@
     for (int q = 0; q < 16; ++q) gp[q] = 0.0;
 #pragma unroll
     for (int u = 0; u < kGroups; ++u) {
-        const double wgt = __builtin_ldexp(1.0, 7 * (u + kUmin) - 80);
+        const double wgt = __builtin_ldexp(1.0, PL::weight_exp(u + kUmin));
 #pragma unroll
         for (int q = 0; q < 16; ++q) gp[q] = __builtin_fma((double)acc[u][q], wgt, gp[q]);
     }
@@ -760,24 +742,25 @@
     uint4* dst = adv(blockIdx.y ? g.dig_t[par] : g.dig[par], po);
     const int lane = t & 63, ksrb = t >> 6, ks = ksrb % (d >> 5), rb = ksrb / (d >> 5);
     const int m = lane & 31, g2 = lane >> 5;
-    uint32_t w[kDigits][4];
-#pragma unroll
-    for (int p = 0; p < kDigits; ++p) { w[p][0] = 0u; w[p][1] = 0u; w[p][2] = 0u; w[p][3] = 0u; }
+    typedef Planes256 PL;
+    uint32_t w[PL::kPlanes][4];
+#pragma unroll
+    for (int p = 0; p < PL::kPlanes; ++p) { w[p][0] = 0u; w[p][1] = 0u; w[p][2] = 0u; w[p][3] = 0u; }
 #pragma unroll
     for (int h = 0; h < 2; ++h) {
         const uint4 uh = src[fa_idx(rb, 2 * ks + g2, 0, 32 * h + m, d)], ul = src[fa_idx(rb, 2 * ks + g2, 1, 32 * h + m, d)];
         f16x8 hi, lo; __builtin_memcpy(&hi, &uh, 16); __builtin_memcpy(&lo, &ul, 16);
 #pragma unroll
         for (int j = 0; j < 8; ++j) {
-            int dg[kDigits];
-            digits_of<float>(used16(hi[j], lo[j]), dg);
+            int dg[PL::kPlanes];
+            digits_of<PL, float>(used16(hi[j], lo[j]), dg);
             const int byte = 8 * h + j;
 #pragma unroll
-            for (int p = 0; p < kDigits; ++p) w[p][byte >> 2] |= ((uint32_t)dg[p] & 0xffu) << (8 * (byte & 3));
-        }
-    }
-#pragma unroll
-    for (int p = 0; p < kDigits; ++p) dst[dg_idx(rb, ks, p, lane, d)] = make_uint4(w[p][0], w[p][1], w[p][2], w[p][3]);
+            for (int p = 0; p < PL::kPlanes; ++p) w[p][byte >> 2] |= ((uint32_t)dg[p] & 0xffu) << (8 * (byte & 3));
+        }
+    }
+#pragma unroll
+    for (int p = 0; p < PL::kPlanes; ++p) dst[dg_idx<PL>(rb, ks, p, lane, d)] = make_uint4(w[p][0], w[p][1], w[p][2], w[p][3]);
 }
 
 __global__ void nsf_rearm(Ns32State* s32) {
diff --git a/fadtk_amd/csrc/ns_fast_big.h b/fadtk_amd/csrc/ns_fast_big.h
--- a/fadtk_amd/csrc/ns_fast_big.h
+++ b/fadtk_amd/csrc/ns_fast_big.h
@@ -245,7 +245,9 @@
     }
 }
 
-constexpr int kI8BigStage = 36 * 64;
+typedef Planes256 BigPL;
+constexpr int kI8BigPieces = 6 * BigPL::kPlanes;
+constexpr int kI8BigStage = kI8BigPieces * 64;
 #ifndef FAD_I8_BIG_STAGES
 #define FAD_I8_BIG_STAGES 2
 #endif
@@ -256,8 +258,8 @@
 __global__ __launch_bounds__(512) void nsf_i8_big(I8Args g, int nprob) {
     extern __shared__ __attribute__((aligned(16))) uint4 ring[];
     double* red = reinterpret_cast<double*>(ring + kI8BigStages * kI8BigStage);
-    constexpr int kUmin = (MODE == I8_A) ? kUminA : kUminG;
-    constexpr int kGroups = 2 * (kDigits - 1) - kUmin + 1;
+    typedef BigPL PL;
+    constexpr int kUmin = PL::template umin<MODE>(), kGroups = PL::template groups<MODE>(), kPl = PL::kPlanes;
     const int d = g.d, tid = threadIdx.x, lane = tid & 63;
     const int tr_ = d >> 7, tc_ = d >> 6, tt = tr_ * tc_;
     const BigSlot slot = big_slot(blockIdx.x, nprob, tt);
@@ -296,16 +298,18 @@
     const int nks = d >> 5;
 #endif
 
+    constexpr int kPieces = kI8BigPieces, kSideA = 4 * kPl;
+    constexpr int kPerWave = (kPieces + 7) / 8, kFull = (kPieces % 8) ? (kPieces % 8) : 8;
     const uint32_t voff = (uint32_t)lane * 16u;
     const uint32_t ring_lds = (uint32_t)(size_t)(__attribute__((address_space(3))) void*)ring;
     auto issue = [&](int ks) {
 #pragma unroll
-        for (int i = 0; i < 5; ++i) {
+        for (int i = 0; i < kPerWave; ++i) {
             const int q = wave + 8 * i;
-            if (q < 36) {
-                const bool bs = q >= 24;
-                const int blk = bs ? (q - 24) / 6 : q / 6, p = bs ? (q - 24) % 6 : q % 6;
-                const uint64_t sb = (uint64_t)((bs ? Bd : Ad) + dg_idx((bs ? 2 * TX : 4 * TY) + blk, ks, p, 0, d));
+            if (q < kPieces) {
+                const bool bs = q >= kSideA;
+                const int blk = bs ? (q - kSideA) / kPl : q / kPl, p = bs ? (q - kSideA) % kPl : q % kPl;
+                const uint64_t sb = (uint64_t)((bs ? Bd : Ad) + dg_idx<PL>((bs ? 2 * TX : 4 * TY) + blk, ks, p, 0, d));
                 const uint32_t lo = __builtin_amdgcn_readfirstlane((uint32_t)sb);
                 const uint32_t hi = __builtin_amdgcn_readfirstlane((uint32_t)(sb >> 32));
                 const uint64_t ub = ((uint64_t)hi << 32) | lo;
@@ -321,28 +325,29 @@
         for (int q = 0; q < 16; ++q) acc[u][q] = 0;
     static_assert(kI8BigStages >= 2 && kI8BigStages <= 4, "the counted waits below cover two younger stages at most");
     for (int ks = 0; ks < kI8BigStages - 1 && ks < nks; ++ks) issue(ks);
-    const bool five = wave < 4;
+    static_assert(kPieces == 30 && kPerWave == 4 && kFull == 6, "the counted waits below: four pieces per stage on waves 0..5, three on 6, 7");
+    const bool four = wave < kFull;
     for (int ks = 0; ks < nks; ++ks) {
         const int ahead = (nks - 1 - ks < kI8BigStages - 2) ? (nks - 1 - ks) : (kI8BigStages - 2);
-        if (ahead == 2) { if (five) asm volatile("s_waitcnt vmcnt(10)" ::: "memory"); else asm volatile("s_waitcnt vmcnt(8)" ::: "memory"); }
-        else if (ahead == 1) { if (five) asm volatile("s_waitcnt vmcnt(5)" ::: "memory"); else asm volatile("s_waitcnt vmcnt(4)" ::: "memory"); }
+        if (ahead == 2) { if (four) asm volatile("s_waitcnt vmcnt(8)" ::: "memory"); else asm volatile("s_waitcnt vmcnt(6)" ::: "memory"); }
+        else if (ahead == 1) { if (four) asm volatile("s_waitcnt vmcnt(4)" ::: "memory"); else asm volatile("s_waitcnt vmcnt(3)" ::: "memory"); }
         else asm volatile("s_waitcnt vmcnt(0)" ::: "memory");
         __builtin_amdgcn_s_barrier();
 #ifndef FAD_I8_ABL_NODMA
         if (ks + kI8BigStages - 1 < nks) issue(ks + kI8BigStages - 1);
 #endif
         const i32x4* st = reinterpret_cast<const i32x4*>(ring + (ks % kI8BigStages) * kI8BigStage) + lane;
-        i32x4 a[kDigits], b[kDigits];
-#pragma unroll
-        for (int p = 0; p < kDigits; ++p) { a[p] = st[(wr * 6 + p) * 64]; b[p] = st[(24 + wc * 6 + p) * 64]; }
+        i32x4 a[kPl], b[kPl];
+#pragma unroll
+        for (int p = 0; p < kPl; ++p) { a[p] = st[(wr * kPl + p) * 64]; b[p] = st[(kSideA + wc * kPl + p) * 64]; }
 #ifdef FAD_I8_ABL_NOMMA
 #pragma unroll
-        for (int p = 0; p < kDigits; ++p) { acc[0][p] += a[p][0] ^ b[p][1]; acc[1][p] += a[p][2] ^ b[p][3]; }
+        for (int p = 0; p < kPl; ++p) { acc[0][p] += a[p][0] ^ b[p][1]; acc[1][p] += a[p][2] ^ b[p][3]; }
 #else
 #pragma unroll
-        for (int p = kDigits - 1; p >= 0; --p)
-#pragma unroll
-            for (int q = kDigits - 1; q >= 0; --q)
+        for (int p = kPl - 1; p >= 0; --p)
+#pragma unroll
+            for (int q = kPl - 1; q >= 0; --q)
                 if (p + q >= kUmin) acc[p + q - kUmin] = __builtin_amdgcn_mfma_i32_32x32x32_i8(a[p], b[q], acc[p + q - kUmin], 0, 0, 0);
 #endif
     }
@@ -352,7 +357,7 @@
     for (int q = 0; q < 16; ++q) gp[q] = 0.0;
 #pragma unroll
     for (int u = 0; u < kGroups; ++u) {
-        const double wgt = __builtin_ldexp(1.0, 7 * (u + kUmin) - 80);
+        const double wgt = __builtin_ldexp(1.0, PL::weight_exp(u + kUmin));
 #pragma unroll
         for (int q = 0; q < 16; ++q) gp[q] = __builtin_fma((double)acc[u][q], wgt, gp[q]);
     }
diff --git a/fadtk_amd/csrc/ns_fast_res.h b/fadtk_amd/csrc/ns_fast_res.h
--- a/fadtk_amd/csrc/ns_fast_res.h
+++ b/fadtk_amd/csrc/ns_fast_res.h
@@ -4,8 +4,9 @@
 namespace fad {
 namespace nsf {
 
+typedef Planes256 ResPL;
 constexpr size_t kResLds = 2 * 65536 + 1024;
-constexpr size_t kResLdsFull = kResLds + 6 * 4 * 1024;
+constexpr size_t kResLdsFull = kResLds + ResPL::kPlanes * 4 * 1024;
 
 struct ResArgs {
     int gen, max_low;
@@ -54,14 +55,15 @@
 
     double fro2_l = 0.0, tr_l = 0.0, colsum_max = 0.0;
     if constexpr (FULL) {
-        constexpr int kGroups = 2 * (kDigits - 1) - kUminA + 1;
-        i32x4 bd[4][kDigits];
+        typedef ResPL PL;
+        constexpr int kPl = PL::kPlanes, kUmin = PL::kUminA, kGroups = PL::template groups<I8_A>();
+        i32x4 bd[4][kPl];
         {
-            const i32x4* pb = reinterpret_cast<const i32x4*>(adv(g.Bdig, po) + dg_idx(j, 0, 0, lane, d));
+            const i32x4* pb = reinterpret_cast<const i32x4*>(adv(g.Bdig, po) + dg_idx<PL>(j, 0, 0, lane, d));
 #pragma unroll
             for (int ks = 0; ks < 4; ++ks)
 #pragma unroll
-                for (int p = 0; p < kDigits; ++p) bd[ks][p] = pb[(ks * kDigits + p) * 64];
+                for (int p = 0; p < kPl; ++p) bd[ks][p] = pb[(ks * kPl + p) * 64];
         }
         const double inv12 = hdr_inv_s12(g.hA, hB);
         double* A64 = adv(g.A64, po) + (int64_t)(4 * kg) * d + 32 * j + n;
@@ -73,23 +75,23 @@
             for (int u = 0; u < kGroups; ++u)
 #pragma unroll
                 for (int q = 0; q < 16; ++q) acc[u][q] = 0;
-            const i32x4* pa = reinterpret_cast<const i32x4*>(g.Adig + dg_idx(rbo, 0, 0, lane, d));
+            const i32x4* pa = reinterpret_cast<const i32x4*>(g.Adig + dg_idx<PL>(rbo, 0, 0, lane, d));
 #pragma unroll
             for (int ks = 0; ks < 4; ++ks) {
-                i32x4 a[kDigits];
-#pragma unroll
-                for (int p = 0; p < kDigits; ++p) a[p] = pa[(ks * kDigits + p) * 64];
-#pragma unroll
-                for (int p = kDigits - 1; p >= 0; --p)
-#pragma unroll
-                    for (int q = kDigits - 1; q >= 0; --q)
-                        if (p + q >= kUminA) acc[p + q - kUminA] = __builtin_amdgcn_mfma_i32_32x32x32_i8(a[p], bd[ks][q], acc[p + q - kUminA], 0, 0, 0);
+                i32x4 a[kPl];
+#pragma unroll
+                for (int p = 0; p < kPl; ++p) a[p] = pa[(ks * kPl + p) * 64];
+#pragma unroll
+                for (int p = kPl - 1; p >= 0; --p)
+#pragma unroll
+                    for (int q = kPl - 1; q >= 0; --q)
+                        if (p + q >= kUmin) acc[p + q - kUmin] = __builtin_amdgcn_mfma_i32_32x32x32_i8(a[p], bd[ks][q], acc[p + q - kUmin], 0, 0, 0);
             }
 #pragma unroll
             for (int q = 0; q < 16; ++q) {
                 double v = 0.0;
 #pragma unroll
-                for (int u = 0; u < kGroups; ++u) v = __builtin_fma((double)acc[u][q], __builtin_ldexp(1.0, 7 * (u + kUminA) - 80), v);
+                for (int u = 0; u < kGroups; ++u) v = __builtin_fma((double)acc[u][q], __builtin_ldexp(1.0, PL::weight_exp(u + kUmin)), v);
                 A64[(int64_t)(32 * rbo + rowc(q)) * d] = v * inv12;
                 fro2_l += v * v; cs += fabs(v);
                 if (rbo == j && rowc(q) + 4 * kg == n) tr_l += v;
@@ -285,7 +287,8 @@
 
     if constexpr (FULL) {
         char* const DG = lds + 131072 + 1024;
-        constexpr int kGroups = 2 * (kDigits - 1) - kUminG + 1;
+        typedef ResPL PL;
+        constexpr int kPl = PL::kPlanes, kUmin = PL::kUminG, kGroups = PL::template groups<I8_G>();
         double try_l = 0.0, zcol = 0.0;
 #pragma unroll
         for (int ks = 0; ks < 8; ++ks)
@@ -297,21 +300,21 @@
 #pragma unroll
             for (int reg = 0; reg < 16; ++reg)
                 if (rbo == j && rowc(reg) + 4 * kg == n) try_l += (double)used16(Yh[2 * rbo + (reg >> 3)][reg & 7], Yl[2 * rbo + (reg >> 3)][reg & 7]);
-        i32x4 yd[4][kDigits];
+        i32x4 yd[4][kPl];
 #pragma unroll
         for (int ks = 0; ks < 4; ++ks) {
-            uint32_t w[kDigits][4];
-#pragma unroll
-            for (int p = 0; p < kDigits; ++p) { w[p][0] = 0u; w[p][1] = 0u; w[p][2] = 0u; w[p][3] = 0u; }
+            uint32_t w[kPl][4];
+#pragma unroll
+            for (int p = 0; p < kPl; ++p) { w[p][0] = 0u; w[p][1] = 0u; w[p][2] = 0u; w[p][3] = 0u; }
 #pragma unroll
             for (int sl = 0; sl < 16; ++sl) {
-                int dg[kDigits];
-                digits_of<float>(used16(Yh[2 * ks + (sl >> 3)][sl & 7], Yl[2 * ks + (sl >> 3)][sl & 7]), dg);
-#pragma unroll
-                for (int p = 0; p < kDigits; ++p) w[p][sl >> 2] |= ((uint32_t)dg[p] & 0xffu) << (8 * (sl & 3));
-            }
-#pragma unroll
-            for (int p = 0; p < kDigits; ++p) { yd[ks][p][0] = (int)w[p][0]; yd[ks][p][1] = (int)w[p][1]; yd[ks][p][2] = (int)w[p][2]; yd[ks][p][3] = (int)w[p][3]; }
+                int dg[kPl];
+                digits_of<PL, float>(used16(Yh[2 * ks + (sl >> 3)][sl & 7], Yl[2 * ks + (sl >> 3)][sl & 7]), dg);
+#pragma unroll
+                for (int p = 0; p < kPl; ++p) w[p][sl >> 2] |= ((uint32_t)dg[p] & 0xffu) << (8 * (sl & 3));
+            }
+#pragma unroll
+            for (int p = 0; p < kPl; ++p) { yd[ks][p][0] = (int)w[p][0]; yd[ks][p][1] = (int)w[p][1]; yd[ks][p][2] = (int)w[p][2]; yd[ks][p][3] = (int)w[p][3]; }
         }
         double zrow = 0.0;
         if (tid < d) {
@@ -333,19 +336,19 @@
                 const int ks = tid >> 6;
                 const f16x8* yq = reinterpret_cast<const f16x8*>(Q) + ((rbo * 8 + 2 * ks) * 2) * 64 + lane;
                 const f16x8 h0 = yq[0], l0 = yq[64], h1 = yq[128], l1 = yq[192];
-                uint32_t w[kDigits][4];
-#pragma unroll
-                for (int p = 0; p < kDigits; ++p) { w[p][0] = 0u; w[p][1] = 0u; w[p][2] = 0u; w[p][3] = 0u; }
+                uint32_t w[kPl][4];
+#pragma unroll
+                for (int p = 0; p < kPl; ++p) { w[p][0] = 0u; w[p][1] = 0u; w[p][2] = 0u; w[p][3] = 0u; }
 #pragma unroll
                 for (int sl = 0; sl < 16; ++sl) {
-                    int dg[kDigits];
-                    digits_of<float>(sl < 8 ? used16(h0[sl & 7], l0[sl & 7]) : used16(h1[sl & 7], l1[sl & 7]), dg);
-#pragma unroll
-                    for (int p = 0; p < kDigits; ++p) w[p][sl >> 2] |= ((uint32_t)dg[p] & 0xffu) << (8 * (sl & 3));
+                    int dg[kPl];
+                    digits_of<PL, float>(sl < 8 ? used16(h0[sl & 7], l0[sl & 7]) : used16(h1[sl & 7], l1[sl & 7]), dg);
+#pragma unroll
+                    for (int p = 0; p < kPl; ++p) w[p][sl >> 2] |= ((uint32_t)dg[p] & 0xffu) << (8 * (sl & 3));
                 }
 #pragma unroll
-                for (int p = 0; p < kDigits; ++p)
-                    *reinterpret_cast<uint4*>(DG + ((ks * kDigits + p) * 64 + lane) * 16) = make_uint4(w[p][0], w[p][1], w[p][2], w[p][3]);
+                for (int p = 0; p < kPl; ++p)
+                    *reinterpret_cast<uint4*>(DG + ((ks * kPl + p) * 64 + lane) * 16) = make_uint4(w[p][0], w[p][1], w[p][2], w[p][3]);
             }
             __syncthreads();
             i32x16 acc[kGroups];
@@ -355,20 +358,20 @@
                 for (int q = 0; q < 16; ++q) acc[u][q] = 0;
 #pragma unroll
             for (int ks = 0; ks < 4; ++ks) {
-                i32x4 a[kDigits];
-#pragma unroll
-                for (int p = 0; p < kDigits; ++p) a[p] = *reinterpret_cast<const i32x4*>(DG + ((ks * kDigits + p) * 64 + lane) * 16);
-#pragma unroll
-                for (int p = kDigits - 1; p >= 0; --p)
-#pragma unroll
-                    for (int q = kDigits - 1; q >= 0; --q)
-                        if (p + q >= kUminG) acc[p + q - kUminG] = __builtin_amdgcn_mfma_i32_32x32x32_i8(a[p], yd[ks][q], acc[p + q - kUminG], 0, 0, 0);
+                i32x4 a[kPl];
+#pragma unroll
+                for (int p = 0; p < kPl; ++p) a[p] = *reinterpret_cast<const i32x4*>(DG + ((ks * kPl + p) * 64 + lane) * 16);
+#pragma unroll
+                for (int p = kPl - 1; p >= 0; --p)
+#pragma unroll
+                    for (int q = kPl - 1; q >= 0; --q)
+                        if (p + q >= kUmin) acc[p + q - kUmin] = __builtin_amdgcn_mfma_i32_32x32x32_i8(a[p], yd[ks][q], acc[p + q - kUmin], 0, 0, 0);
             }
 #pragma unroll
             for (int q = 0; q < 16; ++q) {
                 double G = 0.0;
 #pragma unroll
-                for (int u = 0; u < kGroups; ++u) G = __builtin_fma((double)acc[u][q], __builtin_ldexp(1.0, 7 * (u + kUminG) - 80), G);
+                for (int u = 0; u < kGroups; ++u) G = __builtin_fma((double)acc[u][q], __builtin_ldexp(1.0, PL::weight_exp(u + kUmin)), G);
                 const double R = A64[(int64_t)(32 * rbo + rowc(q)) * d] * inv_c - G;
                 r2_l += R * R;
                 const int o = res_lds_off(32 * j + n, 32 * rbo + rowc(q) + 4 * kg);
```

New measurement: 12230 (median of 6 runs). 1.03x the previous value.
